# millecker/hadoop-1.0.3-gpu

Measured on AMD Instinct MI355X. Metric: K-Means job makespan + map-tasks/sec (whole node) at 1/2/4/8 MI355X, higher is better.
Workload: dtype fp32

## Files before the change

### hbmr/models/kmeans.py

```python
from __future__ import annotations

import base64
import logging
import math
import os
import threading
import time

import numpy as np
import torch

from ..gpu.splitjob import SplitJob, SplitSpec
from ..mapred import counters as C

log = logging.getLogger("hbmr.kmeans")

K_KEY = "hbmr.kmeans.k"
D_KEY = "hbmr.kmeans.dims"
INPUT_KEY = "hbmr.kmeans.input"
SPLIT_PTS_KEY = "hbmr.split.points"
CIN_KEY = "hbmr.kmeans.centroids.in"
COUT_KEY = "hbmr.kmeans.centroids.out"
INIT_KEY = "hbmr.kmeans.centroids.init"
NCENTERS_KEY = "hbmr.kmeans.synthetic.centers"
RETURN_KEY = "hbmr.kmeans.return.centroids"
CDIR_KEY = "hbmr.kmeans.centroids.dir"
EXACT_KEY = "hbmr.kmeans.exact"
EXACT_MFMA_KEY = "hbmr.kmeans.exact.mfma"
COMBINER_KEY = "hbmr.kmeans.combiner"
BOUNDS_KEY = "hbmr.kmeans.exact.bounds"

_M32 = 0xFFFFFFFF


def _mix32(x: torch.Tensor) -> torch.Tensor:
    x = x & _M32
    x = ((x ^ (x >> 16)) * 0x45D9F3B) & _M32
    x = ((x ^ (x >> 16)) * 0x45D9F3B) & _M32
    return x ^ (x >> 16)


def _uniform(c: torch.Tensor) -> torch.Tensor:
    return (_mix32(c).to(torch.float64) + 0.5) * (1.0 / 4294967296.0)


def _gauss(c1: torch.Tensor, c2: torch.Tensor) -> torch.Tensor:
    u1 = _uniform(c1)
    u2 = _uniform(c2)
    return torch.sqrt(-2.0 * torch.log(u1)) * torch.cos(2.0 * math.pi * u2)


def synthetic_points(seed: int, start: int, n: int, d: int, centers: int, device,
                     chunk: int = 1 << 18) -> torch.Tensor:
    dev = torch.device(device)
    out = torch.empty(n, d, dtype=torch.float32, device=dev)
    j = torch.arange(d, dtype=torch.int64, device=dev)
    cidx = torch.arange(centers, dtype=torch.int64, device=dev)
    s = (seed * 0x9E3779B1) & _M32
    cc = (cidx[:, None] * 131071 + j[None, :] + s * 7) & _M32
    cen = 10.0 * _gauss(cc * 2 + 1, cc * 2 + 2)
    for a in range(0, n, chunk):
        b = min(n, a + chunk)
        p = torch.arange(start + a, start + b, dtype=torch.int64, device=dev)
        lab = _mix32(p * 3 + s) % centers
        base = ((p[:, None] & 0xFFFFFF) * 1024 + j[None, :] + (s << 7)) & _M32
        noise = _gauss(base * 2 + 11, base * 2 + 12 + (p[:, None] >> 24))
        out[a:b] = (cen[lab] + noise).to(torch.float32)
    return out


def encode_centroids(c: torch.Tensor) -> str:
    a = c.detach().to("cpu", torch.float32).contiguous().numpy()
    return f"{a.shape[0]}x{a.shape[1]}:" + base64.b64encode(a.tobytes()).decode()


def decode_centroids(s: str) -> torch.Tensor:
    shp, b = s.split(":", 1)
    k, d = map(int, shp.split("x"))
    return torch.from_numpy(np.frombuffer(base64.b64decode(b), dtype=np.float32).copy()
                            ).reshape(k, d)


class CentroidStore:

    def __init__(self):
        self.lock = threading.Lock()
        self.host: dict[str, torch.Tensor] = {}
        self.images: dict[tuple, object] = {}
        self.order: list[str] = []
        self.keep = 4

    def put_host(self, key, cen):
        with self.lock:
            self.host[key] = cen
            for k in [k for k in self.images if k[0] == key]:
                self.images.pop(k)
            self._touch(key)

    def put_image(self, key, device, img):
        with self.lock:
            self.host.pop(key, None)
            self.images[(key, str(device))] = img
            self._touch(key)

    def _touch(self, key):
        if key in self.order:
            self.order.remove(key)
        self.order.append(key)
        while len(self.order) > self.keep:
            old = self.order.pop(0)
            self.host.pop(old, None)
            for k in [k for k in self.images if k[0] == old]:
                self.images.pop(k)

    def host_centroids(self, key):
        with self.lock:
            c = self.host.get(key)
            if c is not None:
                return c
            for (k, _dev), img in self.images.items():
                if k == key:
                    ready = getattr(img, "ready", None)
                    if ready is not None:
                        ready.synchronize()
                    c = img.cen.detach().to("cpu")
                    self.host[key] = c
                    return c
        return None

    def image(self, key, device):
        from ..ops import kmeans as km
        with self.lock:
            img = self.images.get((key, str(device)))
        if img is not None:
            return img
        cen = self.host_centroids(key)
        if cen is None:
            raise KeyError(f"centroids {key!r} not resident on this tracker")
        img = km.CentroidImage(cen, device)
        if img.cen.is_cuda:
            img.ready = torch.cuda.Event()
            img.ready.record()
        self.put_image(key, device, img)
        return img


STORE = CentroidStore()


def _centroid_file(cdir, key):
    return os.path.join(cdir, key.replace("/", "_").replace(":", "_") + ".npy")


def _save_centroids(cdir, key, cen):
    host = cen.detach().to("cpu", torch.float32).numpy()
    os.makedirs(cdir, exist_ok=True)
    path = _centroid_file(cdir, key)
    tmp = path + ".tmp.npy"
    np.save(tmp, host)
    os.replace(tmp, path)
    old = _SAVED.setdefault(cdir, [])
    old.append(path)
    while len(old) > 3:
        try:
            os.remove(old.pop(0))
        except OSError:
            pass


_SAVED: dict = {}
_PINNED_INFLIGHT: list = []


def _sum_slabs(outs):
    groups: dict = {}
    loose = []
    for s, c in outs:
        bs, bc = s._base, c._base
        if bs is not None and bc is not None and bs.dim() == 3 and bc.dim() == 2 and \
                tuple(s.shape) == tuple(bs.shape[1:]) and tuple(c.shape) == tuple(bc.shape[1:]):
            g = groups.setdefault(id(bs), [bs, bc, 0, []])
            g[2] += 1
            g[3].append((s, c))
        else:
            loose.append((s, c))
    parts_s, parts_c = [], []
    for bs, bc, n, members in groups.values():
        if n == bs.shape[0] and len({m[0].data_ptr() for m in members}) == n:
            parts_s.append(bs.sum(0))
            parts_c.append(bc.sum(0))
        else:
            loose.extend(members)
    if loose:
        parts_s.append(torch.stack([s for s, _ in loose]).sum(0))
        parts_c.append(torch.stack([c for _, c in loose]).sum(0))
    sums, counts = parts_s[0], parts_c[0]
    for s, c in zip(parts_s[1:], parts_c[1:]):
        sums = sums + s
        counts = counts + c
    return sums, counts


_EXACT_STATS: dict = {}
_EXACT_SKIPPED: dict = {}
_EXACT_LOCK = threading.Lock()

_BASELINES: "dict" = {}
_BASE_LOCK = threading.Lock()
_BASE_MAX = 4096


def _baseline_plan(ctxs, datas, k, dp, fx, exact, enabled):
    have, new, plain = [], [], []
    bases, keys = [], []
    seen = set()
    dev = str(ctxs[0].device)
    with _BASE_LOCK:
        for i, (c, d) in enumerate(zip(ctxs, datas)):
            sp = c.spec.split
            sk = sp.get("key") if enabled and isinstance(sp, dict) else None
            key = None if sk is None else (sk, dev, k, dp, fx, exact)
            keys.append(key)
            if key is None or key in seen:
                plain.append(i)
                bases.append(None)
                continue
            seen.add(key)
            b = _BASELINES.get(key)
            x = d.xb if exact else d
            if b is not None and b.data_ptr == x.data_ptr() and b.n == x.shape[0]:
                have.append(i)
                bases.append(b)
            else:
                new.append(i)
                bases.append(None)
    return have, new, plain, bases, keys


def _baseline_bytes(b) -> int:
    return sum(t.numel() * t.element_size() for t in (b.g, b.S0, b.N0, getattr(b, "gap", None))
               if t is not None)


def _drop_baselines(split_key, device):
    dev = f"cuda:{device}" if isinstance(device, int) else str(device)
    with _BASE_LOCK:
        for key in [kk for kk in _BASELINES if kk[0] == split_key and kk[1] == dev]:
            _BASELINES.pop(key)


def _install_baselines(entries, stream, cache=None, grown=None):
    ev = torch.cuda.Event()
    ev.record(stream)
    charge = []
    with _BASE_LOCK:
        for key, b in entries:
            b.event, b.stream = ev, stream
            old = _BASELINES.pop(key, None)
            _BASELINES[key] = b
            if old is not b:
                charge.append((key, b, _baseline_bytes(b)))
            elif grown and grown.get(id(b)):
                charge.append((key, b, grown[id(b)]))
        while len(_BASELINES) > _BASE_MAX:
            _BASELINES.pop(next(iter(_BASELINES)))
    if cache is not None and charge:
        cache.add_listener(_drop_baselines)
        idx = stream.device.index if stream is not None else 0
        for key, b, nbytes in charge:
            if not cache.charge(key[0], idx, nbytes):
                with _BASE_LOCK:
                    if _BASELINES.get(key) is b:
                        _BASELINES.pop(key)


def _exact_stats(cin, device):
    key = (cin, str(device))
    with _EXACT_LOCK:
        t = _EXACT_STATS.get(key)
        if t is None:
            t = _EXACT_STATS[key] = torch.zeros(3, dtype=torch.int64, device=device)
        return t


def _exact_skipped(cin, device):
    key = (cin, str(device))
    with _EXACT_LOCK:
        t = _EXACT_SKIPPED.get(key)
        if t is None:
            t = _EXACT_SKIPPED[key] = torch.zeros(1, dtype=torch.int64, device=device)
        return t


class KMeansSplitJob(SplitJob):
    collective_reduce = True
    needs_reduce = True

    def configure(self, conf):
        self.conf = conf
        self.k = conf.get_int(K_KEY, 64)
        self.d = conf.get_int(D_KEY, 128)
        self.input = conf.get(INPUT_KEY, "synthetic:100000:1")
        self.split_points = conf.get_int(SPLIT_PTS_KEY, 500_000)
        self.cin = conf.get(CIN_KEY)
        self.cout = conf.get(COUT_KEY)
        self.centers = conf.get_int(NCENTERS_KEY, self.k)
        self.fx_shift = conf.get_int("hbmr.kmeans.fx.shift", 24)
        self.cdir = conf.get(CDIR_KEY)
        self.exact = conf.get_boolean(EXACT_KEY, False)
        self.exact_dtype = torch.bfloat16 if (conf.get(EXACT_MFMA_KEY) or "f16").lower() in (
            "bf16", "bfloat16") else torch.float16
        self.bounds = conf.get_boolean(BOUNDS_KEY, True)
        self.combiner = (conf.get(COMBINER_KEY) or "delta").lower()
        if self.combiner not in ("delta", "sorted"):
            raise ValueError(f"{COMBINER_KEY} must be delta or sorted, not {self.combiner!r}")
        init = conf.get(INIT_KEY)
        if init and self.cin and STORE.host_centroids(self.cin) is None:
            STORE.put_host(self.cin, decode_centroids(init))
        if self.cin and self.cdir and STORE.host_centroids(self.cin) is None:
            path = _centroid_file(self.cdir, self.cin)
            if os.path.exists(path):
                STORE.put_host(self.cin, torch.from_numpy(np.load(path)))

    _split_memo: dict = {}

    def get_splits(self, conf, trackers):
        if self.input.startswith("synthetic:"):
            mk = (self.input, self.split_points, self.d, self.centers, tuple(trackers),
                  self.exact)
            got = KMeansSplitJob._split_memo.get(mk)
            if got is not None:
                return got
            if len(KMeansSplitJob._split_memo) > 16:
                KMeansSplitJob._split_memo.clear()
            out = KMeansSplitJob._split_memo[mk] = self._synthetic_splits(trackers)
            return out
        return self._file_splits(conf, trackers)

    def _synthetic_splits(self, trackers):
        _, n, seed = self.input.split(":")
        n, seed = int(n), int(seed)
        per = self.split_points
        nsplits = max(1, math.ceil(n / per))
        out = []
        for i in range(nsplits):
            a = i * per
            m = min(per, n - a)
            key = f"kmeans-syn:{seed}:{self.d}:{self.centers}:{a}:{m}" + \
                (":exact" if self.exact else "")
            loc = [trackers[i * len(trackers) // nsplits]] if trackers else []
            out.append(SplitSpec(i, key, "synthetic",
                                 {"seed": seed, "start": a, "n": m}, loc, m * self.d * 2))
        return out

    def _file_splits(self, conf, trackers):
        from ..mapred.formats import FileInputFormat, SequenceFileInputFormat
        from ..mapred.jobconf import JobConf
        jc = JobConf(conf)
        FileInputFormat.setInputPaths(jc, self.input)
        fmt = SequenceFileInputFormat()
        nmaps = max(1, conf.get_int("mapred.map.tasks", 1))
        if conf.get_long("mapred.min.split.size", 0) <= 1 and "://" not in self.input:
            total = sum(f.length for f in fmt.list_status(jc))
            jc.set_long("mapred.min.split.size", max(1, -(-total // nmaps)))
        splits = fmt.getSplits(jc, nmaps)
        out = []
        for i, s in enumerate(splits):
            key = f"kmeans-file:{s.path}:{s.start}:{s.length}" + (":exact" if self.exact else "")
            loc = [trackers[i % len(trackers)]] if trackers else []
            out.append(SplitSpec(i, key, "file", {"path": s.path, "start": s.start,
                                                  "length": s.length}, loc, s.length))
        return out

    def _load_raw(self, spec: SplitSpec, device):
        if spec.kind == "synthetic":
            p = spec.params
            return synthetic_points(p["seed"], p["start"], p["n"], self.d, self.centers, device)
        return self._load_file_split(spec.params, device)

    def _load_fp32(self, spec: SplitSpec, device):
        return self._load_raw(spec, device).to(torch.bfloat16)

    def split_nbytes(self, data) -> int:
        nb = getattr(data, "nbytes", None)
        if callable(nb):
            return int(nb())
        return super().split_nbytes(data)

    def load_split_host(self, spec: SplitSpec):
        if spec.kind != "file":
            return None
        from ..io import nativeio
        p = spec.params
        n = p["length"] // (20 + 4 * self.d) + 2
        host = torch.empty(n, self.d, dtype=torch.float32,
                           pin_memory=torch.cuda.is_available())
        got = nativeio.read_points_into(p["path"], p["start"], p["length"], host.data_ptr(),
                                        self.d, n)
        return host[:got]

    def load_split_from_host(self, spec: SplitSpec, host, device):
        from ..ops import kmeans as km
        x = host.to(device, non_blocking=True)
        ev = torch.cuda.Event()
        ev.record()
        _PINNED_INFLIGHT.append((ev, host))
        while _PINNED_INFLIGHT and _PINNED_INFLIGHT[0][0].query():
            _PINNED_INFLIGHT.pop(0)
        if self.exact:
            return km.ExactSplit(x, km.padded_dim(self.d), self.exact_dtype)
        xb = x.to(torch.bfloat16)
        dp = km.padded_dim(self.d)
        if dp == self.d:
            return xb.contiguous()
        out = torch.zeros(xb.shape[0], dp, dtype=torch.bfloat16, device=device)
        out[:, :self.d] = xb
        return out

    def _load_file_split(self, p, device):
        from ..io import nativeio
        n = p["length"] // (20 + 4 * self.d) + 2
        dev = torch.device(device)
        host = torch.empty(n, self.d, dtype=torch.float32, pin_memory=dev.type == "cuda")
        got = nativeio.read_points_into(p["path"], p["start"], p["length"], host.data_ptr(),
                                        self.d, n)
        host = host[:got]
        if dev.type != "cuda":
            return host
        x = host.to(dev, non_blocking=True)
        ev = torch.cuda.Event()
        ev.record()
        _PINNED_INFLIGHT.append((ev, host))
        while _PINNED_INFLIGHT and _PINNED_INFLIGHT[0][0].query():
            _PINNED_INFLIGHT.pop(0)
        return x

    def load_split_sample(self, spec: SplitSpec, device, fraction: float):
        if spec.kind == "synthetic":
            p = dict(spec.params)
            p["n"] = max(1, int(p["n"] * fraction))
            spec = SplitSpec(spec.index, spec.key + f":sample{fraction}", spec.kind, p,
                             spec.locations, spec.length)
            return self.load_split(spec, device)
        return super().load_split_sample(spec, device, fraction)

    def load_split(self, spec: SplitSpec, device):
        from ..ops import kmeans as km
        if self.exact:
            x = self._load_raw(spec, device)
            if str(device) == "cpu":
                return x.contiguous()
            return km.ExactSplit(x, km.padded_dim(self.d), self.exact_dtype)
        xb = self._load_fp32(spec, device)
        if str(device) == "cpu":
            return xb.to(torch.float32)
        dp = km.padded_dim(self.d)
        if dp == self.d:
            return xb.contiguous()
        out = torch.zeros(xb.shape[0], dp, dtype=torch.bfloat16, device=device)
        out[:, :self.d] = xb
        return out

    @staticmethod
    def _scratch(ctx, ns, k):
        from ..ops import kmeans as km
        key = ("kmeans-scratch", str(ctx.device), id(ctx.stream))
        store = ctx.tracker.__dict__.setdefault("_scratch", {})
        ws, labels = store.get(key, (None, None))
        need_lab, need_ws = km.batch_scratch_sizes(ns, k)
        need_ws = max(need_ws, km.delta_workspace_bytes(int(sum(ns)), len(ns), k))
        if ws is None or ws.numel() < need_ws:
            ws = torch.empty(max(need_ws, 1 << 20), dtype=torch.uint8, device=ctx.device)
        if labels is None or labels.numel() < need_lab:
            labels = torch.empty(max(need_lab, 1), dtype=torch.int32, device=ctx.device)
        store[key] = (ws, labels)
        return ws, labels

    def map_gpu(self, ctx, points):
        return self.map_gpu_batch([ctx], [points])[0]

    def map_gpu_batch(self, ctxs, datas):
        st = ctxs[0].stream
        if st is None:
            return self._map_gpu_batch(ctxs, datas)
        with torch.cuda.stream(st):
            return self._map_gpu_batch(ctxs, datas)

    def _map_gpu_batch(self, ctxs, datas):
        from ..ops import kmeans as km
        ctx = ctxs[0]
        img = STORE.image(self.cin, ctx.device)
        ready = getattr(img, "ready", None)
        if ready is not None:
            torch.cuda.current_stream().wait_event(ready)
        for t in (img.cbf, img.chalf):
            t.record_stream(torch.cuda.current_stream())
        B = len(datas)
        if self.exact:
            return self._map_exact(ctxs, datas, img)
        have, new, plain, bases, keys = _baseline_plan(
            ctxs, datas, self.k, img.dp, img.fx_shift, False, self.combiner == "delta")
        ws, labels = self._scratch(ctx, [d.shape[0] for d in datas], self.k)
        sums = torch.empty(B, self.k, img.dp, dtype=torch.int64, device=ctx.device)
        counts = torch.empty(B, self.k, dtype=torch.int64, device=ctx.device)
        order = have + new + plain
        H = len(have)
        S, N = sums.unbind(0), counts.unbind(0)
        out = [None] * B
        for j, i in enumerate(order):
            out[i] = (S[j], N[j])
        installed = []
        if have:
            hb = [bases[i] for i in have]
            km.map_batch_delta([datas[i] for i in have], img, sums[:H], counts[:H], labels, ws,
                               hb, stream=ctx.stream)
            for i, b in zip(have, hb):
                b.S0, b.N0 = out[i]
                installed.append((keys[i], b))
        rest = new + plain
        if rest:
            km.map_batch_gpu([datas[i] for i in rest], img, sums[H:], counts[H:], labels, ws,
                             stream=ctx.stream, zero_outputs=True)
            if new:
                total = sum(datas[i].shape[0] for i in rest)
                gall = labels[:total].clone()
                off = 0
                newset = set(new)
                for i in rest:
                    n = datas[i].shape[0]
                    if keys[i] is not None and i in newset:
                        installed.append((keys[i], km.Baseline(gall[off:off + n], *out[i],
                                                                datas[i].data_ptr(), n)))
                    off += n
        if installed:
            _install_baselines(installed, ctx.stream, getattr(ctx, "split_cache", None))
        for c, d in zip(ctxs, datas):
            c.reporter.incrCounter(C.TASK_GROUP, C.MAP_INPUT_RECORDS, d.shape[0])
        return out

    def _map_exact(self, ctxs, datas, img):
        from ..ops import kmeans as km
        from ..utils.trace import TRACE
        if TRACE.on:
            TRACE.instant("kmeans.map_exact", n=len(datas))
        ctx = ctxs[0]
        store = ctx.tracker.__dict__.setdefault("_scratch", {})
        scratch = store.setdefault(("kmeans-exact", str(ctx.device), id(ctx.stream)), {})
        stats = _exact_stats(self.cin, ctx.device)
        have, new, plain, bases, keys = _baseline_plan(
            ctxs, datas, self.k, img.dp, img.fx_shift, True, self.combiner == "delta")
        B = len(datas)
        sums = torch.empty(B, self.k, img.dp, dtype=torch.int64, device=ctx.device)
        counts = torch.empty(B, self.k, dtype=torch.int64, device=ctx.device)
        order = have + new + plain
        pos = {i: j for j, i in enumerate(order)}
        H = len(have)
        installed = []
        grown = None
        if have:
            ns = [datas[i].shape[0] for i in have]
            total = sum(ns)
            lab = scratch.get("labcat")
            if lab is None or lab.numel() < total:
                lab = scratch["labcat"] = torch.empty(total, dtype=torch.int32, device=ctx.device)
            need = km.delta_workspace_bytes(total, H, self.k)
            if scratch.get("dws") is None or scratch["dws"].numel() < need:
                scratch["dws"] = torch.empty(need, dtype=torch.uint8, device=ctx.device)
            hb = [bases[i] for i in have]
            bounded = self.bounds and self.combiner == "delta" and km.bounds_supported(img)
            if bounded:
                nogap = [b for b in hb if b.gap is None]
                km.assign_exact_batch([datas[i] for i in have], img, stats, lab, scratch,
                                      stream=ctx.stream, bounds=hb,
                                      skipped=_exact_skipped(self.cin, ctx.device))
                grown = {id(b): b.gap.numel() * b.gap.element_size() for b in nogap}
            else:
                km.assign_exact_batch([datas[i] for i in have], img, stats, lab, scratch,
                                      stream=ctx.stream)
            km.delta_combine([datas[i].x32 for i in have], lab, self.k, sums[:H], counts[:H],
                             scratch["dws"], hb, fx_shift=img.fx_shift, stream=ctx.stream,
                             keep_bounds=bounded)
            for i, b in zip(have, hb):
                b.S0, b.N0 = sums[pos[i]], counts[pos[i]]
                installed.append((keys[i], b))
        for i in new + plain:
            d = datas[i]
            s, c = sums[pos[i]], counts[pos[i]]
            s.zero_()
            c.zero_()
            lab = km.assign_exact(d, img, stats, scratch, stream=ctx.stream)
            need = km.workspace_bytes(d.shape[0], img.k)
            if scratch.get("ws") is None or scratch["ws"].numel() < need:
                scratch["ws"] = torch.empty(max(need, 1 << 20), dtype=torch.uint8,
                                            device=ctx.device)
            km.accumulate(d.x32, lab, img.k, s, c, fx_shift=img.fx_shift, stream=ctx.stream,
                          workspace=scratch["ws"])
            if keys[i] is not None and i in new:
                b = km.Baseline(lab.clone(), s, c, d.xb.data_ptr(), d.shape[0])
                installed.append((keys[i], b))
        if installed:
            _install_baselines(installed, ctx.stream, getattr(ctx, "split_cache", None), grown)
        for c, d in zip(ctxs, datas):
            c.reporter.incrCounter(C.TASK_GROUP, C.MAP_INPUT_RECORDS, d.shape[0])
        return [(sums[pos[i]], counts[pos[i]]) for i in range(B)]

    def map_cpu(self, ctx, points):
        from ..ops import kmeans as km
        cen = STORE.host_centroids(self.cin)
        if cen is None:
            raise KeyError(f"centroids {self.cin!r} not resident")
        sums, counts = km.new_partials(self.k, self.d, "cpu")
        st = [0]
        km.map_split_cpu(points, cen, sums, counts, nthreads=ctx.cpu_threads,
                         fx_shift=self.fx_shift, exact=self.exact, stats=st)
        if self.exact:
            ctx.reporter.incrCounter("KMEANS", "EXACT_FLAGGED_POINTS", st[0])
        ctx.reporter.incrCounter(C.TASK_GROUP, C.MAP_INPUT_RECORDS, points.shape[0])
        return sums, counts

    def map_sim(self, ctx, points):
        if points is None:
            ctx.reporter.incrCounter(C.TASK_GROUP, C.MAP_INPUT_RECORDS, 0)
            return None
        return self.map_cpu(ctx, points)

    def combine(self, ctx, outputs):
        from ..ops import kmeans as km
        dev = ctx.device if ctx.device is not None else torch.device("cpu")
        dp = km.padded_dim(self.d) if dev.type == "cuda" else self.d
        outputs = [o for o in outputs if o is not None]
        if dev.type == "cuda":
            cur = torch.cuda.current_stream()
            for s, c in outputs:
                if s.is_cuda:
                    s.record_stream(cur)
                    c.record_stream(cur)
        from ..utils.trace import TRACE
        if TRACE.on:
            TRACE.instant("kmeans.combine.recorded", n=len(outputs))
        same = [(s, c) for s, c in outputs if s.device == dev and s.shape[1] == dp]
        other = [(s, c) for s, c in outputs if not (s.device == dev and s.shape[1] == dp)]
        if same:
            sums, counts = _sum_slabs(same)
        else:
            sums = torch.zeros(self.k, dp, dtype=torch.int64, device=dev)
            counts = torch.zeros(self.k, dtype=torch.int64, device=dev)
        for s, c in other:
            sums[:, :s.shape[1]] += s.to(dev, non_blocking=True)
            counts += c.to(dev, non_blocking=True)
        return sums, counts

    def reduce(self, ctx, combined):
        from ..ops import kmeans as km
        from ..utils.trace import TRACE
        sums, counts = combined
        k, dp = sums.shape
        packed = torch.cat([sums.reshape(-1), counts])
        sim = getattr(ctx, "simulated_collective_s", None)
        with TRACE.span("kmeans.allreduce", nbytes=packed.numel() * 8):
            if sim is None:
                ctx.comm.all_reduce(packed)
            else:
                ctx.sim_ready = max(time.time(), getattr(ctx, "sim_base", 0.0)) + sim
        sums = packed[:k * dp].view(k, dp)
        counts = packed[k * dp:]
        est = _EXACT_STATS.pop((self.cin, str(sums.device)), None) \
            if self.exact and sums.device.type == "cuda" else None
        esk = _EXACT_SKIPPED.pop((self.cin, str(sums.device)), None) \
            if self.exact and sums.device.type == "cuda" else None
        killed = getattr(ctx, "killed", None)
        if killed is not None and killed():
            raise RuntimeError("reduce killed (collective restart): result not published")
        if sums.device.type == "cuda":
            old = STORE.image(self.cin, sums.device)
            ready = getattr(old, "ready", None)
            if ready is not None:
                torch.cuda.current_stream().wait_event(ready)
            img = km.CentroidImage.__new__(km.CentroidImage)
            img.__dict__.update(old.__dict__)
            img.cen = old.cen.clone()
            img.cbf = old.cbf.clone()
            img.chalf = old.chalf.clone()
            img.shift2 = torch.zeros_like(old.shift2)
            img.refresh(sums, counts)
            if self.exact:
                img.image16(self.exact_dtype)
                img.neighbors()
            img.ready = torch.cuda.Event()
            img.ready.record()
            host_cen = cen_ev = None
            if ctx.rank == 0 and (self.cdir or self.conf.get_boolean(RETURN_KEY, False)):
                host_cen = torch.empty(tuple(img.cen.shape), dtype=torch.float32,
                                       pin_memory=True)
                host_cen.copy_(img.cen, non_blocking=True)
                cen_ev = torch.cuda.Event()
                cen_ev.record()
            if TRACE.on:
                TRACE.instant("kmeans.refresh_launched")
            STORE.put_image(self.cout, sums.device, img)
            rel = getattr(ctx, "release_dependents", None)
            if rel is not None:
                rel()
            vals = [img.shift2.max().double().sqrt(), counts.sum().double()]
            if est is not None:
                vals += list(est.double().unbind(0))
            if esk is not None:
                vals.append(esk[0].double())
            got = torch.stack(vals).tolist()
            shift, npts = got[0], got[1]
            if esk is not None:
                ctx.reporter.incrCounter("KMEANS", "EXACT_BOUND_SKIPPED_POINTS", int(got[-1]))
            if est is not None:
                for name, v in zip(("EXACT_FLAGGED_POINTS", "EXACT_RELABELLED_POINTS",
                                    "EXACT_NEIGHBOUR_SCANS"), got[2:5]):
                    ctx.reporter.incrCounter("KMEANS", name, int(v))
            if TRACE.on:
                TRACE.instant("kmeans.shift_synced")
            new_cen = None
        else:
            host_cen = cen_ev = None
            old = STORE.host_centroids(self.cin)
            if sim is not None:
                new_cen, shift, npts = old, 0.0, 0
            else:
                cnt = counts.to(torch.float64)[:, None]
                s = sums[:, :self.d].to(torch.float64) / float(1 << self.fx_shift)
                new_cen = torch.where(cnt > 0, s / cnt.clamp(min=1),
                                      old.to(torch.float64)).to(torch.float32)
                shift = float((new_cen - old).norm(dim=1).max()) if self.k else 0.0
                npts = int(counts.sum().item())
            STORE.put_host(self.cout, new_cen)
            rel = getattr(ctx, "release_dependents", None)
            if rel is not None:
                rel()
            if sim is not None:
                delay = ctx.sim_ready - time.time()
                if delay > 0:
                    time.sleep(delay)
        self._write_output(ctx, counts, new_cen)
        if TRACE.on:
            TRACE.instant("kmeans.output_written")
        res = {"shift": shift, "points": int(npts), "centroids_key": self.cout}
        if host_cen is not None:
            cen_ev.synchronize()
        if ctx.rank == 0 and self.cdir:
            cen = new_cen if new_cen is not None else host_cen
            _save_centroids(self.cdir, self.cout, cen[:, :self.d])
        if ctx.rank == 0 and self.conf.get_boolean(RETURN_KEY, False):
            cen = new_cen if new_cen is not None else host_cen
            res["centroids"] = encode_centroids(cen[:, :self.d])
        if TRACE.on:
            TRACE.instant("kmeans.reduce_return")
        return res

    def poison_result(self, ctx):
        with STORE.lock:
            host = STORE.host.get(self.cout)
            if host is not None:
                STORE.host[self.cout] = host + 1.0
            for key, img in list(STORE.images.items()):
                if key[0] == self.cout:
                    STORE.images.pop(key)
                    STORE.host[self.cout] = img.cen.detach().to("cpu")[:, :self.d] + 1.0

    def _write_output(self, ctx, counts, new_cen):
        out = self.conf.get("mapred.output.dir")
        if not out:
            return
        import os

        from ..io import sequencefile as seqf
        from ..io.writable import FloatVectorWritable, IntWritable
        cen = new_cen if new_cen is not None else STORE.host_centroids(self.cout)
        W = ctx.world_size
        per = math.ceil(self.k / W)
        lo, hi = ctx.rank * per, min(self.k, (ctx.rank + 1) * per)
        os.makedirs(out, exist_ok=True)
        with seqf.Writer(os.path.join(out, f"part-{ctx.rank:05d}"), IntWritable,
                         FloatVectorWritable) as w:
            for j in range(lo, hi):
                w.append(IntWritable(j), FloatVectorWritable(cen[j].numpy()))


def make_iteration_conf(base, k, d, inp, split_points, cin, cout, init=None,
                        return_centroids=False):
    from ..mapred.jobconf import JobConf
    job = JobConf(base)
    job.set_job_name(f"kmeans {cin}->{cout}")
    job.set("hbmr.splitjob.class", "hbmr.models.kmeans:KMeansSplitJob")
    job.set("hbmr.gpu.mapper.class", "hbmr.models.kmeans:KMeansSplitJob")
    job.set_int(K_KEY, k)
    job.set_int(D_KEY, d)
    job.set(INPUT_KEY, inp)
    job.set_int(SPLIT_PTS_KEY, split_points)
    job.set(CIN_KEY, cin)
    job.set(COUT_KEY, cout)
    job.set("hbmr.job.signature", f"kmeans|{inp}|{k}|{d}|{split_points}")
    if init is not None:
        job.set(INIT_KEY, encode_centroids(init))
    if return_centroids:
        job.set_boolean(RETURN_KEY, True)
    return job


def initial_centroids(inp, k, d, centers=None, exact=False):
    def rnd(x):
        return x if exact else x.to(torch.bfloat16).to(torch.float32)
    if inp.startswith("synthetic:"):
        _, _n, seed = inp.split(":")
        x = synthetic_points(int(seed), 0, k, d, centers or k, "cpu")
        return rnd(x)
    from ..io import sequencefile as seqf
    import os
    path = inp
    if os.path.isdir(path):
        path = os.path.join(path, sorted(f for f in os.listdir(path) if not f.startswith(("_", ".")))[0])
    rows = []
    with seqf.Reader(path) as r:
        while len(rows) < k:
            raw = r.next_raw()
            if raw is None:
                break
            rows.append(np.frombuffer(raw[1][4:], dtype=">f4").astype(np.float32))
    return rnd(torch.from_numpy(np.stack(rows)))


class KMeansDriver:

    MANIFEST = "driver.json"

    def __init__(self, submit, result_of, conf=None, k=64, d=128, inp="synthetic:100000:1",
                 split_points=500_000, run_id=None, return_centroids=None, checkpoint_dir=None):
        self.submit = submit
        self.result_of = result_of
        self.base = conf
        self.k, self.d, self.inp, self.split_points = k, d, inp, split_points
        self.run_id = run_id or f"km{int(time.time() * 1e3) & 0xFFFFFF:x}"
        self.iteration = 0
        self.history = []
        self.return_centroids = (k * d <= 65536) if return_centroids is None else return_centroids
        base_dir = (conf.get("mapred.local.dir") if conf is not None else None) or "/tmp/hbmr-local"
        self.centroid_dir = checkpoint_dir or os.path.join(base_dir, "kmeans-centroids",
                                                           self.run_id)
        self._manifest_written = False
        self.prefetch_delay = 0.005
        self._ahead: list = []

    def _write_manifest(self):
        import json
        os.makedirs(self.centroid_dir, exist_ok=True)
        path = os.path.join(self.centroid_dir, self.MANIFEST)
        with open(path + ".tmp", "w") as f:
            json.dump({"run_id": self.run_id, "k": self.k, "d": self.d, "input": self.inp,
                       "split_points": self.split_points}, f)
        os.replace(path + ".tmp", path)
        self._manifest_written = True

    @classmethod
    def resume(cls, submit, result_of, checkpoint_dir, conf=None, **kw):
        import json
        import re
        with open(os.path.join(checkpoint_dir, cls.MANIFEST)) as f:
            m = json.load(f)
        drv = cls(submit, result_of, conf=conf, k=m["k"], d=m["d"], inp=m["input"],
# ... 119 lines not shown
```

### hbmr/ops/_lib.py

```python
from __future__ import annotations

import ctypes
import os
import threading
from pathlib import Path

import torch

_LIB_PATH = Path(__file__).resolve().parent.parent / "lib" / "libhbmr.so"
_lock = threading.Lock()
_lib = None

c_void_p = ctypes.c_void_p
c_long = ctypes.c_long
c_int = ctypes.c_int
c_uint = ctypes.c_uint
c_uint64 = ctypes.c_uint64
c_double_p = ctypes.POINTER(ctypes.c_double)

_SIGS = {
    "hbmr_kmeans_assign_bf16": (c_int, [c_void_p, c_long, c_int, c_void_p, c_void_p, c_int,
                                        c_void_p, c_void_p, c_void_p]),
    "hbmr_kmeans_accum_bf16": (c_int, [c_void_p, c_long, c_int, c_void_p, c_int, c_void_p,
                                       c_void_p, c_int, c_void_p, c_long, c_int, c_void_p]),
    "hbmr_kmeans_accum_f32": (c_int, [c_void_p, c_long, c_int, c_void_p, c_int, c_void_p,
                                      c_void_p, c_int, c_void_p, c_long, c_int, c_void_p]),
    "hbmr_kmeans_assign_top3_bf16": (c_int, [c_void_p, c_long, c_int, c_void_p, c_void_p, c_int,
                                             c_void_p, c_void_p, c_void_p, c_void_p, c_void_p]),
    "hbmr_kmeans_assign_top3_f16": (c_int, [c_void_p, c_long, c_int, c_void_p, c_void_p, c_int,
                                            c_void_p, c_void_p, c_void_p, c_void_p, c_void_p]),
    "hbmr_kmeans_exact_prep": (c_int, [c_void_p, c_long, c_int, c_int, c_int, c_int, c_void_p,
                                       c_void_p, c_void_p, c_void_p, c_void_p]),
    "hbmr_kmeans_assign_top3_q1_grouped": (c_int, [c_int, c_void_p, c_void_p, c_int, c_int,
                                                   c_void_p, c_void_p, c_void_p, c_int, c_void_p,
                                                   c_void_p, c_void_p, c_void_p, c_int, c_int,
                                                   c_void_p, c_void_p, c_void_p, c_void_p,
                                                   c_void_p, c_long, c_void_p, c_void_p]),
    "hbmr_kmeans_bound_workspace_bytes": (c_long, [c_long, c_int, c_int]),
    "hbmr_kmeans_assign_top3_q1_bounded": (c_int, [c_int, c_void_p, c_void_p, c_int, c_int,
                                                   c_void_p, c_void_p, c_int, c_void_p,
                                                   c_void_p, c_void_p, c_void_p, c_int, c_int,
                                                   c_void_p, c_void_p, c_void_p, c_void_p,
                                                   c_void_p, c_long, c_void_p,
                                                   c_void_p, c_void_p, c_void_p, c_void_p,
                                                   c_void_p, c_long, c_void_p, c_void_p]),
    "hbmr_kmeans_centroid_nbr": (c_int, [c_void_p, c_int, c_int, c_int, c_void_p, c_void_p,
                                         c_void_p, c_void_p]),
    "hbmr_kmeans_image16": (c_int, [c_void_p, c_int, c_int, c_int, c_int, c_int, c_void_p,
                                    c_void_p, c_void_p, c_void_p, c_void_p, c_void_p]),
    "hbmr_kmeans_image16_tiled": (c_int, [c_void_p, c_int, c_int, c_void_p, c_void_p]),
    "hbmr_kmeans_set_exact_kernel": (c_int, [c_int]),
    "hbmr_kmeans_get_exact_kernel": (c_int, []),
    "hbmr_kmeans_refine_f32": (c_int, [c_void_p, c_long, c_int, c_int, c_void_p, c_void_p,
                                       c_void_p, c_void_p, c_int, c_int, c_void_p, c_void_p,
                                       c_void_p, c_void_p, c_void_p, c_void_p, c_int, c_void_p,
                                       c_void_p, c_void_p, c_void_p, c_void_p, c_int,
                                       c_void_p]),
    "hbmr_kmeans_refine_batch_bytes": (c_long, [c_int, c_void_p]),
    "hbmr_kmeans_assign_top3_grouped": (c_int, [c_int, c_void_p, c_void_p, c_int, c_int,
                                                c_void_p, c_void_p, c_int, c_void_p, c_void_p,
                                                c_void_p, c_void_p, c_void_p]),
    "hbmr_kmeans_refine_batch_q1g": (c_int, [c_int, c_void_p, c_int, c_int, c_int, c_void_p,
                                             c_void_p, c_void_p, c_void_p, c_void_p, c_void_p,
                                             c_void_p, c_void_p, c_void_p, c_void_p, c_void_p,
                                             c_void_p, c_long, c_void_p, c_void_p]),
    "hbmr_kmeans_refine_batch_q1": (c_int, [c_int, c_void_p, c_int, c_int, c_int, c_int,
                                            c_void_p, c_void_p, c_void_p, c_void_p, c_void_p,
                                            c_void_p, c_void_p, c_void_p, c_void_p, c_void_p,
                                            c_void_p, c_void_p, c_void_p, c_long, c_int,
                                            c_void_p, c_void_p]),
    "hbmr_kmeans_refine_batch_finish": (c_int, [c_int, c_void_p, c_void_p, c_void_p, c_int,
                                                c_int, c_void_p, c_int, c_int, c_void_p,
                                                c_void_p, c_void_p, c_void_p, c_int, c_void_p,
                                                c_int, c_void_p, c_long, c_void_p]),
    "hbmr_kmeans_accum_workspace_bytes": (c_long, [c_long, c_int]),
    "hbmr_kmeans_batch_workspace_bytes": (c_long, [c_long, c_int, c_int]),
    "hbmr_kmeans_map_batch": (c_int, [c_int, c_void_p, c_void_p, c_int, c_void_p, c_void_p, c_int,
                                      c_int, c_void_p, c_void_p, c_long, c_void_p, c_void_p,
                                      c_int, c_int, c_void_p]),
    "hbmr_kmeans_delta_workspace_bytes": (c_long, [c_long, c_int, c_int]),
    "hbmr_kmeans_delta_combine": (c_int, [c_int, c_void_p, c_void_p, c_int, c_int, c_int,
                                          c_void_p, c_void_p, c_long, c_void_p, c_void_p, c_int,
                                          c_void_p, c_void_p, c_void_p, c_void_p]),
    "hbmr_kmeans_map_batch_delta": (c_int, [c_int, c_void_p, c_void_p, c_int, c_void_p, c_void_p,
                                            c_int, c_int, c_void_p, c_void_p, c_long, c_void_p,
                                            c_void_p, c_int, c_void_p, c_void_p, c_void_p,
                                            c_void_p]),
    "hbmr_kmeans_update": (c_int, [c_void_p, c_void_p, c_int, c_int, c_int, c_int, c_int,
                                   c_void_p, c_void_p, c_void_p, c_void_p, c_void_p]),
    "hbmr_kmeans_padded_k": (c_int, [c_int]),
    "hbmr_kmeans_map_cpu_f32": (c_int, [c_void_p, c_long, c_int, c_void_p, c_int, c_void_p,
                                        c_void_p, c_void_p, c_double_p, c_int, c_int]),
    "hbmr_kmeans_map_cpu_f32_ex": (c_int, [c_void_p, c_long, c_int, c_void_p, c_int, c_void_p,
                                           c_void_p, c_void_p, c_double_p, c_int, c_int, c_int,
                                           c_void_p]),
    "hbmr_kmeans_padded_dim": (c_int, [c_int]),
    "hbmr_f32_to_bf16_pad": (c_int, [c_void_p, c_long, c_int, c_int, c_void_p, c_void_p]),
    "hbmr_radix_sort_workspace_bytes": (c_long, [c_long]),
    "hbmr_radix_onesweep_workspace_bytes": (c_long, [c_long]),
    "hbmr_radix_onesweep_status_bytes": (c_long, [c_long]),
    "hbmr_radix_sort_keys_u64": (c_int, [c_void_p, c_void_p, c_long, c_int, c_int, c_void_p,
                                         c_long, c_void_p, c_long, c_void_p, c_void_p, c_int,
                                         c_void_p]),
    "hbmr_radix_sort_pairs_u64": (c_int, [c_void_p, c_void_p, c_void_p, c_void_p, c_long, c_int,
                                          c_int, c_void_p, c_long, c_void_p]),
    "hbmr_teragen": (c_int, [c_long, c_long, c_void_p, c_void_p]),
    "hbmr_tera_keys": (c_int, [c_void_p, c_long, c_int, c_void_p, c_void_p, c_void_p]),
    "hbmr_gather_u64": (c_int, [c_void_p, c_void_p, c_long, c_void_p, c_void_p]),
    "hbmr_gather_records": (c_int, [c_void_p, c_void_p, c_long, c_int, c_void_p, c_void_p]),
    "hbmr_split_offsets": (c_int, [c_void_p, c_void_p, c_long, c_void_p, c_void_p, c_int,
                                   c_void_p, c_void_p]),
    "hbmr_check_sorted": (c_int, [c_void_p, c_void_p, c_long, c_void_p, c_void_p]),
    "hbmr_tera_collect": (c_int, [c_void_p, c_void_p, c_void_p, c_void_p, c_void_p, c_int, c_long,
                                  c_void_p, c_void_p, c_void_p, c_void_p, c_void_p]),
    "hbmr_tera_collect_slots": (c_int, [c_void_p, c_void_p, c_void_p, c_int, c_int, c_long,
                                        c_void_p, c_void_p, c_void_p]),
    "hbmr_gather_records_multi": (c_int, [c_void_p, c_void_p, c_void_p, c_void_p, c_long, c_int,
                                          c_void_p, c_void_p]),
    "hbmr_tera_partition_workspace_bytes": (c_long, [c_long, c_int]),
    "hbmr_tera_collect_gid": (c_int, [c_void_p, c_void_p, c_void_p, c_void_p, c_int, c_long,
                                      c_int, c_uint64, c_uint, c_uint, c_int, c_void_p, c_void_p,
                                      c_void_p]),
    "hbmr_gather_records_gid": (c_int, [c_void_p, c_void_p, c_void_p, c_long, c_int, c_void_p,
                                        c_void_p, c_void_p, c_void_p, c_void_p]),
    "hbmr_tera_group_stats": (c_int, [c_void_p, c_void_p, c_long, c_void_p, c_void_p, c_void_p,
                                      c_void_p]),
    "hbmr_radix_set_onesweep_waves": (c_int, [c_int]),
    "hbmr_gather_set_unroll": (c_int, [c_int]),
    "hbmr_tera_tie_fix_scratch_bytes": (c_long, [c_long, c_int]),
    "hbmr_tera_tie_fix_records": (c_int, [c_void_p, c_void_p, c_void_p, c_long, c_int, c_uint64,
                                          c_uint, c_uint, c_int, c_void_p, c_void_p, c_void_p,
                                          c_long, c_void_p]),
    "hbmr_merge_path": (c_int, [c_void_p, c_void_p, c_void_p, c_long, c_void_p, c_void_p, c_void_p,
                                c_long, c_void_p, c_void_p, c_void_p, c_void_p]),
    "hbmr_tera_tie_fix": (c_int, [c_void_p, c_void_p, c_void_p, c_long, c_void_p, c_void_p]),
    "hbmr_tera_partition": (c_int, [c_void_p, c_long, c_int, c_void_p, c_void_p, c_int, c_void_p,
                                    c_void_p, c_void_p, c_void_p, c_void_p, c_void_p, c_long,
                                    c_void_p]),
    "hbmr_wc_tiles": (c_long, [c_long]),
    "hbmr_wc_tokenize_count": (c_int, [c_void_p, c_long, c_void_p, c_void_p]),
    "hbmr_wc_tokenize_write": (c_int, [c_void_p, c_long, c_void_p, c_void_p, c_void_p, c_void_p]),
    "hbmr_wc_insert": (c_int, [c_void_p, c_long, c_void_p, c_void_p, c_void_p, c_long, c_void_p,
                               c_void_p, c_long, c_void_p, c_void_p]),
    "hbmr_wc_compact": (c_int, [c_void_p, c_long, c_void_p, c_void_p, c_long, c_int, c_void_p,
                                c_void_p, c_void_p, c_void_p, c_void_p, c_void_p]),
    "hbmr_wc_pack": (c_int, [c_void_p, c_void_p, c_void_p, c_void_p, c_long, c_void_p, c_void_p,
                             c_void_p]),
    "hbmr_grep_cand_count": (c_int, [c_void_p, c_long, c_void_p, c_void_p, c_int, c_int, c_int,
                                     c_int, c_void_p, c_void_p, c_void_p]),
    "hbmr_grep_cand_write": (c_int, [c_void_p, c_long, c_void_p, c_void_p, c_int, c_int, c_int,
                                     c_int, c_void_p, c_void_p, c_void_p, c_void_p, c_void_p]),
    "hbmr_grep_select_blocks": (c_long, [c_long]),
    "hbmr_grep_block_max": (c_int, [c_void_p, c_long, c_void_p, c_void_p]),
    "hbmr_grep_prefix_max": (c_int, [c_void_p, c_long, c_void_p, c_void_p, c_void_p]),
    "hbmr_grep_select_count": (c_int, [c_void_p, c_void_p, c_void_p, c_long, c_void_p, c_void_p]),
    "hbmr_grep_select_write": (c_int, [c_void_p, c_void_p, c_void_p, c_long, c_void_p, c_void_p,
                                       c_void_p, c_void_p]),
    "hbmr_span_insert": (c_int, [c_void_p, c_long, c_void_p, c_void_p, c_void_p, c_long, c_void_p,
                                 c_void_p, c_long, c_void_p, c_void_p]),
    "hbmr_span_compact": (c_int, [c_void_p, c_void_p, c_void_p, c_void_p, c_void_p, c_long, c_int,
                                  c_void_p, c_void_p, c_void_p, c_void_p, c_void_p, c_void_p]),
    "hbmr_lines_count": (c_int, [c_void_p, c_long, c_void_p, c_void_p]),
    "hbmr_lines_write": (c_int, [c_void_p, c_long, c_void_p, c_void_p, c_void_p, c_void_p]),
    "hbmr_recsort_hash_partition": (c_int, [c_void_p, c_void_p, c_void_p, c_long, c_int, c_void_p,
                                            c_void_p]),
    "hbmr_recsort_round_keys": (c_int, [c_void_p, c_void_p, c_void_p, c_void_p, c_long, c_int,
                                        c_void_p, c_void_p, c_void_p]),
    "hbmr_recsort_round_workspace_bytes": (c_long, [c_long]),
    "hbmr_recsort_round": (c_int, [c_void_p, c_void_p, c_void_p, c_int, c_long, c_int, c_void_p,
                                   c_void_p, c_void_p, c_void_p, c_void_p, c_void_p, c_void_p,
                                   c_void_p, c_void_p, c_long, c_void_p]),
    "hbmr_recsort_cuts": (c_int, [c_void_p, c_void_p, c_void_p, c_void_p, c_long, c_void_p,
                                  c_void_p, c_void_p, c_int, c_void_p, c_void_p]),
    "hbmr_recsort_chunk_bytes": (c_int, []),
    "hbmr_recsort_set_chunk_lanes": (c_int, [c_int]),
    "hbmr_recsort_gather": (c_int, [c_void_p, c_void_p, c_void_p, c_void_p, c_void_p, c_void_p,
                                    c_void_p, c_long, c_long, c_void_p, c_void_p]),
    "hbmr_pi_halton": (c_int, [ctypes.c_longlong, ctypes.c_longlong, c_void_p, c_void_p]),
    "hbmr_gemm_bf16_tn": (c_int, [c_void_p, c_void_p, c_void_p, c_long, c_long, c_long,
                                  ctypes.c_float, c_int, c_void_p]),
    "hbmr_gemm_set_kernel": (c_int, [c_int]),
    "hbmr_gemm_bf16_tn_ex": (c_int, [c_void_p, c_void_p, c_void_p, c_long, c_long, c_long,
                                     ctypes.c_float, c_int, c_void_p, c_void_p]),
}


class NativeLibraryError(RuntimeError):
    pass


def lib_path() -> Path:
    return _LIB_PATH


def available() -> bool:
    try:
        load()
        return True
# ... 45 lines not shown
```

### hbmr/ops/kmeans.py

```python
from __future__ import annotations

import ctypes
import os
import threading

import torch

from . import _lib
from ..utils.trace import TRACE

SUPPORTED_DP = (64, 128, 256)


def _nullctx():
    import contextlib
    return contextlib.nullcontext()
FX_SHIFT = 24
NBR_L = 256


def padded_dim(d: int) -> int:
    for dp in SUPPORTED_DP:
        if d <= dp:
            return dp
# ... 172 lines not shown
    ws = max(int(lib.hbmr_kmeans_batch_workspace_bytes(total, len(ns), k)),
             int(lib.hbmr_kmeans_accum_workspace_bytes(max(ns), k)))
    return total, ws


def accum_workspace(n: int, k: int, device) -> torch.Tensor:
    lib = _lib.load()
    need = int(lib.hbmr_kmeans_accum_workspace_bytes(n, k))
    key = torch.device(device)
    ws = _workspaces.get(key)
    if ws is None or ws.numel() < need:
        ws = torch.empty(max(need, 1 << 20), dtype=torch.uint8, device=key)
        _workspaces[key] = ws
    return ws


def accumulate(points: torch.Tensor, labels: torch.Tensor, k: int, sums: torch.Tensor,
               counts: torch.Tensor, fx_shift: int = FX_SHIFT, stream=None,
               workspace: torch.Tensor | None = None, mode: int = ACCUM_AUTO) -> None:
    n, dp = points.shape
    if sums.shape != (k, dp) or sums.dtype != torch.int64:
        raise ValueError(f"sums must be int64 [{k}, {dp}]")
    if counts.shape != (k,) or counts.dtype != torch.int64:
        raise ValueError(f"counts must be int64 [{k}]")
    if points.dtype not in (torch.bfloat16, torch.float32) or not points.is_contiguous() or \
            dp not in SUPPORTED_DP or labels.numel() < n:
        raise ValueError("points must be contiguous bf16/fp32 [n, dp] with n labels")
    lib = _lib.load()
    if workspace is None and mode != ACCUM_LDS:
        workspace = accum_workspace(n, k, points.device)
    fn, name = ((lib.hbmr_kmeans_accum_f32, "hbmr_kmeans_accum_f32")
                if points.dtype == torch.float32 else
                (lib.hbmr_kmeans_accum_bf16, "hbmr_kmeans_accum_bf16"))
    rc = fn(_ptr(points), n, dp, _ptr(labels), k, _ptr(sums), _ptr(counts), fx_shift,
            _ptr(workspace), 0 if workspace is None else workspace.numel(), mode,
            _lib.stream_handle(stream))
    _lib.check(rc, name)


def _f32_up(v: torch.Tensor) -> torch.Tensor:
    f = v.float()
    return torch.where(f.double() < v, torch.nextafter(f, torch.full_like(f, float("inf"))), f)


class ExactSplit:
    __slots__ = ("xb", "x32", "xnorm", "xbn2", "xerr", "d")

    def __init__(self, x32: torch.Tensor, dp: int, dtype=torch.float16):
        n, d = x32.shape
        self.d = d
        dev = x32.device
        if dp == d:
            self.x32 = x32.contiguous()
        else:
            self.x32 = torch.zeros(n, dp, dtype=torch.float32, device=dev)
            self.x32[:, :d] = x32
        if dev.type == "cuda":
            self.xb = torch.empty(n, dp, dtype=dtype, device=dev)
            self.xnorm = torch.empty(n, dtype=torch.float32, device=dev)
            self.xbn2 = torch.empty(n, dtype=torch.float32, device=dev)
            self.xerr = torch.empty(n, dtype=torch.float32, device=dev)
            rc = _lib.load().hbmr_kmeans_exact_prep(
                _ptr(self.x32), n, dp, dp, dp, int(dtype == torch.float16), _ptr(self.xb),
                _ptr(self.xnorm), _ptr(self.xbn2), _ptr(self.xerr), _lib.stream_handle(None))
            _lib.check(rc, "hbmr_kmeans_exact_prep")
            return
        x64 = self.x32.double()
        self.xnorm = x64.norm(dim=1).float()
        lim = 65504.0 if dtype == torch.float16 else float("inf")
        xb = self.x32.clamp(-lim, lim).to(dtype)
        xb64 = xb.double()
        self.xbn2 = xb64.pow(2).sum(1).float()
        self.xerr = _f32_up((x64 - xb64).norm(dim=1))
        self.xb = xb.contiguous()

    @property
    def shape(self):
        return self.xb.shape

    def nbytes(self) -> int:
        return sum(t.numel() * t.element_size() for t in (self.xb, self.x32, self.xnorm,
                                                          self.xbn2, self.xerr))


def assign_top3(points: torch.Tensor, img: CentroidImage, labels, cand, scores, margin,
                stream=None) -> None:
    n, dp = points.shape
    if points.dtype not in (torch.bfloat16, torch.float16) or dp != img.dp or \
            not points.is_contiguous():
        raise ValueError("points must be contiguous bf16/fp16 [n, dp] matching the image")
    for t, dt, m in ((labels, torch.int32, 1), (cand, torch.int32, 2), (scores, torch.float32, 1),
                     (margin, torch.float32, 2)):
        if t.numel() != m * n or t.dtype != dt or not t.is_contiguous():
            raise ValueError("top-3 outputs: labels/scores [n], cand/margin [2n]")
    f16 = points.dtype == torch.float16
    with torch.cuda.stream(stream) if stream is not None else _nullctx():
        c16, ch = img.image16(points.dtype)[:2]
    fn = "hbmr_kmeans_assign_top3_f16" if f16 else "hbmr_kmeans_assign_top3_bf16"
    rc = getattr(_lib.load(), fn)(
        _ptr(points), n, dp, _ptr(c16), _ptr(ch), img.k_pad, _ptr(labels),
        _ptr(cand), _ptr(scores), _ptr(margin), _lib.stream_handle(stream))
    _lib.check(rc, fn)


REFINE_VERSION = int(os.environ.get("HBMR_REFINE", "3"))
MAX_REFINE_BATCH = 64


def _check_refine_dim(img: "CentroidImage") -> None:
    if REFINE_VERSION >= 3 and img.d % 8:
        raise ValueError(f"refine v3 needs d % 8 == 0 (d = {img.d}): HBMR_REFINE=2 takes any d")


def _refine_ws(ns: list, device, scratch: dict | None):
    arr = (ctypes.c_long * len(ns))(*ns)
    need = int(_lib.load().hbmr_kmeans_refine_batch_bytes(len(ns), arr))
    if need < 0:
        raise ValueError("refine batch of 1..64 splits expected")
    ws = None if scratch is None else scratch.get("refine_ws")
    if ws is None or ws.numel() < need:
        ws = torch.empty(need, dtype=torch.uint8, device=device)
        if scratch is not None:
            scratch["refine_ws"] = ws
    return arr, ws


class _RefineBatch:

    def __init__(self, splits: list, img: "CentroidImage", stats, scratch, stream):
        _check_refine_dim(img)
        self.splits, self.img, self.stats, self.stream = splits, img, stats, stream
        self.dt = splits[0].xb.dtype
        self.ns, self.ws = _refine_ws([sp.shape[0] for sp in splits], splits[0].x32.device,
                                      scratch)
        with torch.cuda.stream(stream) if stream is not None else _nullctx():
            self.norms = img.norms(self.dt)
            self.nbr = img.neighbors()
            self.pd = img.pair_dist()
        self.labels = [None] * len(splits)
        self.lib = _lib.load()
        self.st = _lib.stream_handle(stream)

    def q1(self, i, labels_ptr, cand, scores, margin):
        sp, img = self.splits[i], self.img
        cn, cmax, ce, cemax = self.norms
        self.labels[i] = labels_ptr
        rc = self.lib.hbmr_kmeans_refine_batch_q1(
            len(self.splits), self.ns, i, img.d, img.k, img.k_pad, _ptr(sp.xnorm),
            _ptr(sp.xbn2), _ptr(sp.xerr), _ptr(cn), _ptr(cmax), _ptr(ce), _ptr(cemax),
            labels_ptr, _ptr(cand), _ptr(scores), _ptr(margin), _ptr(self.stats),
            _ptr(self.ws), self.ws.numel(), int(i == 0), _ptr(self.pd), self.st)
        _lib.check(rc, "hbmr_kmeans_refine_batch_q1")

    def finish(self):
        B = len(self.splits)
        img = self.img
        _, cmax, _, cemax = self.norms
        ni, nd, L = self.nbr
        xs = (ctypes.c_void_p * B)(*[sp.x32.data_ptr() for sp in self.splits])
        ls = (ctypes.c_void_p * B)(*[(lp.value if isinstance(lp, ctypes.c_void_p) else lp)
                                     for lp in self.labels])
        rc = self.lib.hbmr_kmeans_refine_batch_finish(
            B, self.ns, xs, ls, img.d, self.splits[0].x32.shape[1], _ptr(img.cen), img.k,
            img.k_pad, _ptr(cmax), _ptr(cemax), _ptr(ni), _ptr(nd), L, _ptr(self.stats),
            self.stats.numel(), _ptr(self.ws), self.ws.numel(), self.st)
        _lib.check(rc, "hbmr_kmeans_refine_batch_finish")


def refine_f32(split: ExactSplit, img: CentroidImage, labels, cand, scores, margin,
               stats: torch.Tensor, stream=None, scratch: dict | None = None) -> None:
    n = split.shape[0]
    if stats.dtype != torch.int64 or stats.numel() < 3:
        raise ValueError("stats must be int64 [3]")
    if labels.numel() != n or cand.numel() != 2 * n or margin.numel() != 2 * n:
        raise ValueError("labels [n], cand/margin [2n] from assign_top3 expected")
    if REFINE_VERSION >= 3:
        rb = _RefineBatch([split], img, stats, scratch, stream)
        rb.q1(0, labels.data_ptr(), cand, scores, margin)
        rb.finish()
        return
    with torch.cuda.stream(stream) if stream is not None else _nullctx():
        cn, cmax, ce, cemax = img.norms(split.xb.dtype)
        ni, nd, L = img.neighbors()
    rc = _lib.load().hbmr_kmeans_refine_f32(
        _ptr(split.x32), n, img.d, split.x32.shape[1], _ptr(split.xnorm), _ptr(split.xbn2),
        _ptr(split.xerr), _ptr(img.cen), img.k, img.k_pad, _ptr(cn), _ptr(cmax), _ptr(ce),
        _ptr(cemax), _ptr(ni), _ptr(nd), L,
        _ptr(labels), _ptr(cand), _ptr(scores), _ptr(margin), _ptr(stats), stats.numel(),
        _lib.stream_handle(stream))
    _lib.check(rc, "hbmr_kmeans_refine_f32")


def assign_exact(split: ExactSplit, img: CentroidImage, stats: torch.Tensor,
                 scratch: dict | None = None, stream=None) -> torch.Tensor:
    _check_refine_dim(img)
    n = split.shape[0]
    dev = split.xb.device
    scratch = {} if scratch is None else scratch
    key = ("exact", n)
    bufs = scratch.get(key)
    if bufs is None:
        bufs = scratch[key] = (torch.empty(n, dtype=torch.int32, device=dev),
                               torch.empty(2 * n, dtype=torch.int32, device=dev),
                               torch.empty(n, dtype=torch.float32, device=dev),
                               torch.empty(2 * n, dtype=torch.float32, device=dev))
    lab, cand, sc, mg = bufs
    assign_top3(split.xb, img, lab, cand, sc, mg, stream=stream)
    refine_f32(split, img, lab, cand, sc, mg, stats, stream=stream, scratch=scratch)
    return lab


def bounds_supported(img: CentroidImage) -> bool:
    return REFINE_VERSION >= 3 and img.dp <= 128 and GROUPED_EXACT and FUSED_Q1 and \
        img.cen.is_cuda and _lib.load().hbmr_kmeans_get_exact_kernel() == 3


def assign_exact_batch(splits: list, img: CentroidImage, stats: torch.Tensor, out: torch.Tensor,
                       scratch: dict | None = None, stream=None, bounds: list | None = None,
                       skipped: torch.Tensor | None = None) -> None:
    if not splits:
        return
    _check_refine_dim(img)
    if bounds is not None and (len(bounds) != len(splits) or not bounds_supported(img)):
        raise ValueError("bounds: one baseline per split, grouped fused v3 assign (dp <= 128)")
    dev = splits[0].xb.device
    total = sum(sp.shape[0] for sp in splits)
    if out.dtype != torch.int32 or out.numel() < total or not out.is_contiguous():
        raise ValueError("out must be contiguous int32 with room for every split's labels")
    if stats.dtype != torch.int64 or stats.numel() < 3:
        raise ValueError("stats must be int64 [3]")
    dt = splits[0].xb.dtype
    for sp in splits:
        if sp.xb.dtype != dt or dt not in (torch.bfloat16, torch.float16) or \
                sp.xb.shape[1] != img.dp or not sp.xb.is_contiguous() or \
                not sp.x32.is_contiguous():
            raise ValueError("exact splits must hold contiguous [n, dp] rows of one 16-bit type")
    nmax = max(sp.shape[0] for sp in splits)
    scratch = {} if scratch is None else scratch
    key = ("exact-batch", nmax)
    bufs = scratch.get(key)
    if bufs is None:
        for kk in [kk for kk in scratch if isinstance(kk, tuple) and kk[0] == "exact-batch"]:
            del scratch[kk]
        bufs = scratch[key] = (torch.empty(2 * nmax, dtype=torch.int32, device=dev),
                               torch.empty(nmax, dtype=torch.float32, device=dev),
                               torch.empty(2 * nmax, dtype=torch.float32, device=dev))
    cand, sc, mg = bufs
    grouped = REFINE_VERSION >= 3 and img.dp <= 128 and GROUPED_EXACT
    with torch.cuda.stream(stream) if stream is not None else _nullctx():
        c16, ch, cn, cmax, ce, cemax = img.image16(dt)
        ni, nd, L = (None, None, 0) if grouped else img.neighbors()
        newref = None
        if bounds is not None:
            img.cen.record_stream(torch.cuda.current_stream())
            newref = img.cen.clone()
    lib = _lib.load()
    top3 = lib.hbmr_kmeans_assign_top3_f16 if dt == torch.float16 else \
        lib.hbmr_kmeans_assign_top3_bf16
    st = _lib.stream_handle(stream)
    pc, ps, pm, pst = _ptr(cand), _ptr(sc), _ptr(mg), _ptr(stats)
    pcn, pcmax, pce, pcemax, pni, pnd = (_ptr(t) for t in (cn, cmax, ce, cemax, ni, nd))
    base, off = out.data_ptr(), 0
    for g0 in range(0, len(splits), MAX_REFINE_BATCH):
        group = splits[g0:g0 + MAX_REFINE_BATCH]
        if grouped:
            off += _exact_group(group, img, stats, base + 4 * off, c16, ch, (cn, cmax, ce, cemax),
                                dt, scratch, stream, lib, st,
                                None if bounds is None else bounds[g0:g0 + MAX_REFINE_BATCH],
                                skipped, newref)
            continue
        rb = _RefineBatch(group, img, stats, scratch, stream) if REFINE_VERSION >= 3 else None
        for i, sp in enumerate(group):
            n = sp.shape[0]
            pl = ctypes.c_void_p(base + 4 * off)
            rc = top3(_ptr(sp.xb), n, img.dp, _ptr(c16), _ptr(ch), img.k_pad, pl, pc, ps, pm, st)
            _lib.check(rc, "hbmr_kmeans_assign_top3")
            if rb is not None:
                rb.q1(i, pl, cand, sc, mg)
            else:
                rc = lib.hbmr_kmeans_refine_f32(
                    _ptr(sp.x32), n, img.d, sp.x32.shape[1], _ptr(sp.xnorm), _ptr(sp.xbn2),
                    _ptr(sp.xerr), _ptr(img.cen), img.k, img.k_pad, pcn, pcmax, pce, pcemax,
                    pni, pnd, L, pl, pc, ps, pm, pst, stats.numel(), st)
                _lib.check(rc, "hbmr_kmeans_refine_f32")
            off += n
        if rb is not None:
            rb.finish()


PAIR_DIST_MAX_K = int(os.environ.get("HBMR_PAIR_DIST_MAX_K", "8192"))
NBR_NATIVE_MAX_K = int(os.environ.get("HBMR_NBR_NATIVE_MAX_K", "8192"))
GROUPED_EXACT = os.environ.get("HBMR_EXACT_GROUPED", "1") != "0"
FUSED_Q1 = os.environ.get("HBMR_EXACT_FUSED_Q1", "1") != "0"


def _bounded_group(group, bases, img, labels_ptr, ch, norms, dt, scratch, stream, lib, st, rb,
                   skipped, newref):
    B = len(group)
    ns = [sp.shape[0] for sp in group]
    N = sum(ns)
    dev = group[0].xb.device
    cur = torch.cuda.current_stream() if stream is None else stream
    with torch.cuda.stream(cur):
        events, blocks = {}, {}
        for b in bases:
            if b.event is not None and b.stream is not None and b.stream != cur:
                events[id(b.event)] = b.event
        for ev in events.values():
            cur.wait_event(ev)
        for b in bases:
            if b.gap is None:
                b.gap, b.ref = torch.empty(b.g.numel(), dtype=torch.float32, device=dev), None
        for b, n in zip(bases, ns):
            if b.g.numel() != n or b.gap.numel() != n or \
                    (b.ref is not None and (tuple(b.ref.shape) != tuple(img.cen.shape) or
                                            not b.ref.is_contiguous())):
                raise ValueError("bounds: baseline does not match its split / the centroids")
            for t in (b.g, b.gap, b.ref):
                if t is not None:
                    base = t._base if t._base is not None else t
                    blocks[id(base)] = base
        for t in blocks.values():
            t.record_stream(cur)
        need = int(lib.hbmr_kmeans_bound_workspace_bytes(N, B, img.k))
        bws = scratch.get("bound_ws")
        if bws is None or bws.numel() < need:
            bws = scratch["bound_ws"] = torch.empty(need, dtype=torch.uint8, device=dev)
    P = ctypes.c_void_p * B
    cn, cmax, ce, cemax = norms
    refs = [b.ref for b in bases]
    for b in bases:
        b.ref = b.pending = None
    rc = lib.hbmr_kmeans_assign_top3_q1_bounded(
        B, P(*[sp.xb.data_ptr() for sp in group]), (ctypes.c_long * B)(*ns), img.dp,
        int(dt == torch.float16), _ptr(img.image16_tiled(dt)), _ptr(ch), img.k_pad, labels_ptr,
        P(*[sp.xnorm.data_ptr() for sp in group]), P(*[sp.xbn2.data_ptr() for sp in group]),
        P(*[sp.xerr.data_ptr() for sp in group]), img.d, img.k, _ptr(cn), _ptr(cmax), _ptr(ce),
        _ptr(cemax), _ptr(rb.ws), rb.ws.numel(), _ptr(rb.pd),
        P(*[b.g.data_ptr() for b in bases]), P(*[b.gap.data_ptr() for b in bases]),
        P(*[None if r is None else r.data_ptr() for r in refs]), _ptr(img.cen),
        _ptr(bws), bws.numel(), _ptr(skipped), st)
    _lib.check(rc, "hbmr_kmeans_assign_top3_q1_bounded")
    for b in bases:
        b.pending = newref


def _exact_group(group, img, stats, labels_ptr, c16, ch, norms, dt, scratch, stream, lib, st,
                 bases=None, skipped=None, newref=None):
    B = len(group)
    ns = [sp.shape[0] for sp in group]
    N = sum(ns)
    dev = group[0].xb.device
    P = ctypes.c_void_p * B
    xs = P(*[sp.xb.data_ptr() for sp in group])
    nsa = (ctypes.c_long * B)(*ns)
    if bases is not None:
        rb = _RefineBatch(group, img, stats, scratch, stream)
        if TRACE.on:
            TRACE.instant("kmeans.top3_launch", n=B)
        _bounded_group(group, bases, img, labels_ptr, ch, norms, dt, scratch, stream, lib, st, rb,
                       skipped, newref)
        o = 0
        for i in range(B):
            rb.labels[i] = labels_ptr + 4 * o
            o += ns[i]
        rb.finish()
        return N
    if FUSED_Q1 and img.dp <= 128:
        rb = _RefineBatch(group, img, stats, scratch, stream)
        if TRACE.on:
            TRACE.instant("kmeans.top3_launch", n=B)
        cn, cmax, ce, cemax = norms
        rc = lib.hbmr_kmeans_assign_top3_q1_grouped(
            B, xs, nsa, img.dp, int(dt == torch.float16), _ptr(c16),
            _ptr(img.image16_tiled(dt)), _ptr(ch), img.k_pad,
            labels_ptr, P(*[sp.xnorm.data_ptr() for sp in group]),
            P(*[sp.xbn2.data_ptr() for sp in group]), P(*[sp.xerr.data_ptr() for sp in group]),
            img.d, img.k, _ptr(cn), _ptr(cmax), _ptr(ce), _ptr(cemax), _ptr(rb.ws),
            rb.ws.numel(), _ptr(rb.pd), st)
        _lib.check(rc, "hbmr_kmeans_assign_top3_q1_grouped")
        o = 0
        for i in range(B):
            rb.labels[i] = labels_ptr + 4 * o
            o += ns[i]
        rb.finish()
        return N
    key = ("exact-group", N)
    bufs = scratch.get(key)
    if bufs is None:
        for kk in [kk for kk in scratch if isinstance(kk, tuple) and kk[0] == "exact-group"]:
            del scratch[kk]
        bufs = scratch[key] = (torch.empty(2 * N, dtype=torch.int32, device=dev),
                               torch.empty(N, dtype=torch.float32, device=dev),
                               torch.empty(2 * N, dtype=torch.float32, device=dev))
    cand, sc, mg = bufs
    rc = lib.hbmr_kmeans_assign_top3_grouped(B, xs, nsa, img.dp, int(dt == torch.float16),
                                             _ptr(c16), _ptr(ch), img.k_pad, labels_ptr,
                                             _ptr(cand), _ptr(sc), _ptr(mg), st)
    _lib.check(rc, "hbmr_kmeans_assign_top3_grouped")
    rb = _RefineBatch(group, img, stats, scratch, stream)
    cn, cmax, ce, cemax = norms
    rc = lib.hbmr_kmeans_refine_batch_q1g(
        B, nsa, img.d, img.k, img.k_pad, P(*[sp.xnorm.data_ptr() for sp in group]),
        P(*[sp.xbn2.data_ptr() for sp in group]), P(*[sp.xerr.data_ptr() for sp in group]),
        _ptr(cn), _ptr(cmax), _ptr(ce), _ptr(cemax), labels_ptr, _ptr(cand), _ptr(sc), _ptr(mg),
        _ptr(rb.ws), rb.ws.numel(), _ptr(rb.pd), st)
    _lib.check(rc, "hbmr_kmeans_refine_batch_q1g")
    o = 0
    for i in range(B):
        rb.labels[i] = labels_ptr + 4 * o
        o += ns[i]
    rb.finish()
    return N


def map_split_exact(split: ExactSplit, img: CentroidImage, sums, counts, scratch: dict,
                    stats: torch.Tensor, stream=None) -> None:
    n = split.shape[0]
    lab = assign_exact(split, img, stats, scratch, stream=stream)
    need = workspace_bytes(n, img.k)
    if scratch.get("ws") is None or scratch["ws"].numel() < need:
        scratch["ws"] = torch.empty(max(need, 1 << 20), dtype=torch.uint8, device=split.xb.device)
    accumulate(split.x32, lab, img.k, sums, counts, fx_shift=img.fx_shift, stream=stream,
               workspace=scratch["ws"])


def map_batch_gpu(splits: list, img: CentroidImage, sums: torch.Tensor, counts: torch.Tensor,
                  labels: torch.Tensor, workspace: torch.Tensor, stream=None,
                  zero_outputs: bool = True) -> None:
    B = len(splits)
    if B == 0:
        return
    for s in splits:
        if s.dtype != torch.bfloat16 or s.shape[1] != img.dp or not s.is_contiguous():
            raise ValueError("splits must be contiguous bf16 [n, dp]")
    if sums.shape != (B, img.k, img.dp) or counts.shape != (B, img.k):
        raise ValueError("batch output shape mismatch")
    need_lab, need_ws = batch_scratch_sizes([s.shape[0] for s in splits], img.k)
    if labels.numel() < need_lab:
        raise ValueError("labels scratch too small")
    lib = _lib.load()
    if workspace.numel() < need_ws:
        raise ValueError("workspace too small")
    ptrs = (ctypes.c_void_p * B)(*[s.data_ptr() for s in splits])
    ns = (ctypes.c_long * B)(*[s.shape[0] for s in splits])
    rc = lib.hbmr_kmeans_map_batch(B, ptrs, ns, img.dp, _ptr(img.cbf), _ptr(img.chalf), img.k_pad,
                                   img.k, _ptr(labels), _ptr(workspace), workspace.numel(),
                                   _ptr(sums), _ptr(counts), img.fx_shift, int(zero_outputs),
                                   _lib.stream_handle(stream))
    _lib.check(rc, "hbmr_kmeans_map_batch")


class Baseline:
    __slots__ = ("g", "S0", "N0", "event", "stream", "data_ptr", "n", "gap", "ref", "pending")

    def __init__(self, g, S0, N0, data_ptr, n):
        self.g, self.S0, self.N0 = g, S0, N0
        self.gap = self.ref = self.pending = None
        self.event = None
        self.stream = None
        self.data_ptr, self.n = data_ptr, n

    def labels_advanced(self, bounded: bool = False) -> None:
        self.ref = self.pending if bounded else None
        self.pending = None


def delta_workspace_bytes(total: int, ntasks: int, k: int) -> int:
    return int(_lib.load().hbmr_kmeans_delta_workspace_bytes(total, ntasks, k))


def _delta_args(xs, bases, stream):
    B = len(xs)
    st = torch.cuda.current_stream() if stream is None else stream
    events, blocks = {}, {}
    for b in bases:
        if b.event is not None and b.stream is not None and b.stream != st:
            events[id(b.event)] = b.event
        for t in (b.g, b.S0, b.N0):
            base = t._base if t._base is not None else t
            blocks[id(base)] = base
    for ev in events.values():
        st.wait_event(ev)
    for t in blocks.values():
        t.record_stream(st)
    ptrs = (ctypes.c_void_p * B)(*[x.data_ptr() for x in xs])
    ns = (ctypes.c_long * B)(*[x.shape[0] for x in xs])
    gs = (ctypes.c_void_p * B)(*[b.g.data_ptr() for b in bases])
    s0 = (ctypes.c_void_p * B)(*[b.S0.data_ptr() for b in bases])
    n0 = (ctypes.c_void_p * B)(*[b.N0.data_ptr() for b in bases])
    return ptrs, ns, gs, s0, n0


def map_batch_delta(splits: list, img: CentroidImage, sums: torch.Tensor, counts: torch.Tensor,
                    labels: torch.Tensor, workspace: torch.Tensor, bases: list,
                    stream=None) -> None:
    B = len(splits)
    if B == 0:
        return
    if B > 64 or len(bases) != B:
        raise ValueError("at most 64 splits per delta batch, one baseline each")
    for s, b in zip(splits, bases):
        if s.dtype != torch.bfloat16 or s.shape[1] != img.dp or not s.is_contiguous():
            raise ValueError("splits must be contiguous bf16 [n, dp]")
        if b.g.numel() != s.shape[0] or tuple(b.S0.shape) != (img.k, img.dp) or \
                b.N0.numel() != img.k:
            raise ValueError("baseline does not match its split")
    if sums.shape != (B, img.k, img.dp) or counts.shape != (B, img.k) or \
            not sums.is_contiguous() or not counts.is_contiguous():
        raise ValueError("batch output shape mismatch")
    total = sum(s.shape[0] for s in splits)
    if labels.numel() < total:
        raise ValueError("labels scratch too small")
    need = delta_workspace_bytes(total, B, img.k)
    if workspace.numel() < need:
        raise ValueError("workspace too small")
    ptrs, ns, gs, s0, n0 = _delta_args(splits, bases, stream)
    for b in bases:
        b.labels_advanced()
    rc = _lib.load().hbmr_kmeans_map_batch_delta(
        B, ptrs, ns, img.dp, _ptr(img.cbf), _ptr(img.chalf), img.k_pad, img.k, _ptr(labels),
        _ptr(workspace), workspace.numel(), _ptr(sums), _ptr(counts), img.fx_shift, gs, s0, n0,
        _lib.stream_handle(stream))
    _lib.check(rc, "hbmr_kmeans_map_batch_delta")


def delta_combine(xs: list, labels: torch.Tensor, k: int, sums: torch.Tensor,
                  counts: torch.Tensor, workspace: torch.Tensor, bases: list,
                  fx_shift: int = FX_SHIFT, stream=None, keep_bounds: bool = False) -> None:
    B = len(xs)
    if B == 0:
        return
    pend = [b.pending for b in bases]
    for b in bases:
        b.labels_advanced()
    dp = xs[0].shape[1]
    f32 = xs[0].dtype == torch.float32
    for x, b in zip(xs, bases):
        if x.dtype != xs[0].dtype or x.shape[1] != dp or not x.is_contiguous() or \
                b.g.numel() != x.shape[0]:
            raise ValueError("delta_combine: rows/baselines mismatch")
    if B > 64 or dp not in SUPPORTED_DP or sums.shape != (B, k, dp) or counts.shape != (B, k):
        raise ValueError("delta_combine: shape mismatch")
    total = sum(x.shape[0] for x in xs)
    need = delta_workspace_bytes(total, B, k)
    if workspace.numel() < need or labels.numel() < total:
        raise ValueError("delta_combine: scratch too small")
    ptrs, ns, gs, s0, n0 = _delta_args(xs, bases, stream)
    rc = _lib.load().hbmr_kmeans_delta_combine(
        B, ptrs, ns, dp, int(f32), k, _ptr(labels), _ptr(workspace), workspace.numel(),
        _ptr(sums), _ptr(counts), fx_shift, gs, s0, n0, _lib.stream_handle(stream))
    _lib.check(rc, "hbmr_kmeans_delta_combine")
    if keep_bounds:
        for b, p in zip(bases, pend):
            b.ref = p


def map_split_gpu(points, img: CentroidImage, sums, counts, labels=None, stream=None):
    labels = assign(points, img, labels=labels, stream=stream)
    accumulate(points, labels, img.k, sums, counts, fx_shift=img.fx_shift, stream=stream)
    return labels


def map_split_cpu(points: torch.Tensor, centroids: torch.Tensor, sums: torch.Tensor,
                  counts: torch.Tensor, nthreads: int = 1, labels: torch.Tensor | None = None,
                  fx_shift: int = FX_SHIFT, exact: bool = False, stats: list | None = None):
    x = points.detach().to(torch.float32).contiguous()
    c = centroids.detach().to(torch.float32).contiguous()
    n, d = x.shape
    k = c.shape[0]
    if counts.shape != (k,) or counts.dtype != torch.int64 or sums.dtype != torch.int64:
        raise ValueError("sums/counts must be int64")
    target = sums
    if sums.shape != (k, d):
        target = torch.zeros(k, d, dtype=torch.int64)
    cost = ctypes.c_double(0.0)
    lib = _lib.load()
    res = ctypes.c_long(0)
    rc = lib.hbmr_kmeans_map_cpu_f32_ex(_ptr(x), n, d, _ptr(c), k, _ptr(labels), _ptr(target),
                                        _ptr(counts), ctypes.byref(cost), fx_shift, int(nthreads),
                                        int(exact), ctypes.byref(res))
    _lib.check(rc, "hbmr_kmeans_map_cpu_f32_ex")
    if stats is not None:
        stats[0] += res.value
    if target is not sums:
        sums[:, :d] += target
    return cost.value
```

### native/include/hbmr/hbmr.h

```cpp
#pragma once
#include <stddef.h>
#include <stdint.h>

#ifdef __cplusplus
extern "C" {
#endif

typedef struct ihipStream_t* hbmr_stream_t;

#ifndef HBMR_NO_HIP_DECLS
#include <hip/hip_runtime_api.h>
int hbmr_kmeans_assign_bf16(const void* X, long n, int dp, const void* C, const float* chalf,
                            int k_pad, int32_t* labels, float* scores, hipStream_t st);
int hbmr_kmeans_accum_bf16(const void* X, long n, int dp, const int32_t* labels, int k,
                           long long* sums, long long* counts, int fx_shift, void* ws,
                           long ws_bytes, int mode, hipStream_t st);
int hbmr_kmeans_accum_f32(const float* X, long n, int dp, const int32_t* labels, int k,
                          long long* sums, long long* counts, int fx_shift, void* ws,
                          long ws_bytes, int mode, hipStream_t st);
int hbmr_kmeans_assign_top3_bf16(const void* X, long n, int dp, const void* C, const float* chalf,
                                 int k_pad, int32_t* labels, int32_t* cand, float* scores,
                                 float* margin, hipStream_t st);
int hbmr_kmeans_assign_top3_f16(const void* X, long n, int dp, const void* C, const float* chalf,
                                int k_pad, int32_t* labels, int32_t* cand, float* scores,
                                float* margin, hipStream_t st);
int hbmr_kmeans_exact_prep(const float* x, long n, int d, int ldx, int dp, int f16, void* x16,
                           float* xnorm, float* xn2, float* xerr, hipStream_t st);
int hbmr_kmeans_centroid_nbr(const float* cen, int k, int d, int L, int32_t* di, float* dv,
                             float* pd, hipStream_t st);
int hbmr_kmeans_image16(const float* cen, int k, int d, int dp, int k_pad, int f16, void* c16,
                        float* chalf, float* cnorm, float* cerr, float* maxima, hipStream_t st);
int hbmr_kmeans_image16_tiled(const void* c16, int k_pad, int dp, void* c16t, hipStream_t st);
int hbmr_kmeans_set_stamps(void* p);
int hbmr_kmeans_refine_f32(const float* X32, long n, int d, int ldx, const float* xnorm,
                           const float* xbn2, const float* xerr, const float* C32, int k,
                           int k_pad, const float* cnorm, const float* cmax, const float* cerr,
                           const float* cerrmax, const int32_t* nbr_idx,
                           const float* nbr_dist, int L, int32_t* labels, const int32_t* cand,
                           const float* scores, const float* margin, unsigned long long* stats,
                           int nstats, hipStream_t st);
int hbmr_kmeans_assign_top3_q1_grouped(int nsplit, const void* const* X, const long* n, int dp,
                                       int f16, const void* C, const void* Ct,
                                       const float* chalf, int k_pad,
                                       int32_t* labels, const float* const* xnorm,
                                       const float* const* xbn2, const float* const* xerr,
                                       int d, int k, const float* cnorm, const float* cmax,
                                       const float* cerr, const float* cerrmax, void* ws,
                                       long ws_bytes, const float* dcc, hipStream_t st);
long hbmr_kmeans_bound_workspace_bytes(long total, int nsplit, int k);
int hbmr_kmeans_assign_top3_q1_bounded(int nsplit, const void* const* X, const long* n, int dp,
                                       int f16, const void* Ct, const float* chalf, int k_pad,
                                       int32_t* labels, const float* const* xnorm,
                                       const float* const* xbn2, const float* const* xerr,
                                       int d, int k, const float* cnorm, const float* cmax,
                                       const float* cerr, const float* cerrmax, void* ws,
                                       long ws_bytes, const float* dcc,
                                       const int32_t* const* g, float* const* gap,
                                       const float* const* ref, const float* cen, void* bws,
                                       long bws_bytes, unsigned long long* skipped,
                                       hipStream_t st);
int hbmr_kmeans_assign_top3_grouped(int nsplit, const void* const* X, const long* n, int dp,
                                    int f16, const void* C, const float* chalf, int k_pad,
                                    int32_t* labels, int32_t* cand, float* scores, float* margin,
                                    hipStream_t st);
int hbmr_kmeans_refine_batch_q1g(int nsplit, const long* ns, int d, int k, int k_pad,
                                 const float* const* xnorm, const float* const* xbn2,
                                 const float* const* xerr, const float* cnorm, const float* cmax,
                                 const float* cerr, const float* cerrmax, const int32_t* labels,
                                 const int32_t* cand, const float* scores, const float* margin,
                                 void* ws, long ws_bytes, const float* dcc, hipStream_t st);
long hbmr_kmeans_refine_batch_bytes(int nsplit, const long* ns);
int hbmr_kmeans_refine_batch_q1(int nsplit, const long* ns, int s, int d, int k, int k_pad,
                                const float* xnorm, const float* xbn2, const float* xerr,
                                const float* cnorm, const float* cmax, const float* cerr,
                                const float* cerrmax, const int32_t* labels, const int32_t* cand,
                                const float* scores, const float* margin,
                                unsigned long long* stats, void* ws, long ws_bytes, int reset,
                                const float* dcc, hipStream_t st);
int hbmr_kmeans_refine_batch_finish(int nsplit, const long* ns, const float* const* x32,
                                    int32_t* const* labels, int d, int ldx, const float* C32,
                                    int k, int k_pad, const float* cmax, const float* cerrmax,
                                    const int32_t* nbr_idx, const float* nbr_dist, int L,
                                    unsigned long long* stats, int nstats, void* ws,
                                    long ws_bytes, hipStream_t st);
int hbmr_kmeans_update(const long long* sums, const long long* counts, int fx_shift, int k, int d,
                       int dp, int k_pad, float* cen, void* cbf, float* chalf, float* shift2,
                       hipStream_t st);
int hbmr_kmeans_map_batch(int ntasks, const void* const* X, const long* n, int dp,
                          const void* C, const float* chalf, int k_pad, int k, int32_t* labels,
                          void* ws, long ws_bytes, long long* sums, long long* counts,
                          int fx_shift, int zero_outputs, hipStream_t st);
int hbmr_f32_to_bf16_pad(const float* src, long n, int d, int dp, void* dst, hipStream_t st);
#endif
int hbmr_kmeans_padded_dim(int d);

#ifndef HBMR_NO_HIP_DECLS
int hbmr_radix_sort_pairs_u64(uint64_t* keys, uint32_t* vals, uint64_t* tkeys, uint32_t* tvals,
                              long n, int begin_bit, int end_bit, void* ws, long ws_bytes,
                              hipStream_t st);
int hbmr_teragen(long first_row, long nrows, void* out, hipStream_t st);
int hbmr_tera_keys(const void* records, long n, int stride, uint64_t* hi, uint64_t* lo,
                   hipStream_t st);
int hbmr_gather_u64(const uint64_t* src, const uint32_t* perm, long n, uint64_t* dst,
                    hipStream_t st);
int hbmr_gather_records(const void* src, const uint32_t* perm, long n, int record_bytes, void* dst,
                        hipStream_t st);
int hbmr_split_offsets(const uint64_t* hi, const uint64_t* lo, long n, const uint64_t* shi,
                       const uint64_t* slo, int nparts, long* offsets, hipStream_t st);
int hbmr_check_sorted(const uint64_t* hi, const uint64_t* lo, long n, unsigned long long* bad,
                      hipStream_t st);
int hbmr_tera_collect(const uint64_t* const* his, const uint64_t* const* los,
                      const uint32_t* const* rows, const long* starts, const long* prefix, int S,
                      long n, uint64_t* ohi, uint64_t* olo, uint32_t* osplit, uint32_t* orow,
                      hipStream_t st);
int hbmr_tera_collect_slots(const uint32_t* const* rows, const long* starts, const long* pre,
                            int S, int W, long C, uint32_t* osplit, uint32_t* orow,
                            hipStream_t st);
int hbmr_gather_records_multi(const void* const* bases, const uint32_t* split, const uint32_t* row,
                              const uint32_t* perm, long n, int record_bytes, void* dst,
                              hipStream_t st);
int hbmr_tera_collect_gid(const uint64_t* const* his, const uint32_t* const* rows,
                          const long* starts, const long* prefix, int S, long n, int pack,
                          uint64_t vlo, unsigned int m, unsigned int R, int sh, uint64_t* ohi,
                          uint32_t* ogid, hipStream_t st);
int hbmr_gather_records_gid(const void* const* bases, const uint32_t* gid, const uint64_t* packed,
                            long n, int record_bytes, void* dst, uint64_t* hi, uint64_t* lo,
                            uint32_t* win, hipStream_t st);
long hbmr_radix_onesweep_workspace_bytes(long n);
long hbmr_radix_onesweep_status_bytes(long n);
int hbmr_radix_sort_keys_u64(uint64_t* keys, uint64_t* tkeys, long n, int begin_bit, int end_bit,
                             void* ws, long ws_bytes, void* status, long status_bytes,
                             unsigned int* epoch, uint32_t* err, int copy_back, hipStream_t st);
long hbmr_tera_tie_fix_scratch_bytes(long cap, int record_bytes);
int hbmr_tera_group_stats(const uint64_t* hi, const uint64_t* lo, long n, const uint64_t* ph,
                          const uint64_t* pl, unsigned long long* acc, hipStream_t st);
int hbmr_tera_tie_fix_records(uint64_t* hi, uint64_t* lo, void* rec, long n, int record_bytes,
                              uint64_t vlo, unsigned int m, unsigned int R, int sh,
                              const uint32_t* win, unsigned int* flag, void* scratch, long cap,
                              hipStream_t st);
int hbmr_merge_path(const uint64_t* ahi, const uint64_t* alo, const uint32_t* av, long na,
                    const uint64_t* bhi, const uint64_t* blo, const uint32_t* bv, long nb,
                    uint64_t* ohi, uint64_t* olo, uint32_t* ov, hipStream_t st);
int hbmr_tera_tie_fix(const uint64_t* hi, uint64_t* lo, uint32_t* perm, long n,
                      unsigned int* flag, hipStream_t st);
int hbmr_tera_partition(const void* records, long n, int stride, const uint64_t* shi,
                        const uint64_t* slo, int nsplit, uint64_t* ohi, uint64_t* olo,
                        uint32_t* orow, long* offsets, unsigned long long* kmm, void* ws,
                        long ws_bytes, hipStream_t st);
#endif
long hbmr_radix_sort_workspace_bytes(long n);
long hbmr_tera_partition_workspace_bytes(long n, int nparts);

#ifndef HBMR_NO_HIP_DECLS
int hbmr_gemm_bf16_tn(const void* A, const void* Bt, void* C, long M, long N, long K, float alpha,
                      int out_bf16, hipStream_t st);
int hbmr_gemm_bf16_tn_ex(const void* A, const void* Bt, void* C, long M, long N, long K,
                         float alpha, int out_bf16, double* partials, hipStream_t st);
#endif
#ifndef HBMR_NO_HIP_DECLS
long hbmr_wc_tiles(long n);
int hbmr_wc_tokenize_count(const uint8_t* buf, long n, uint32_t* tile_counts, hipStream_t st);
int hbmr_wc_tokenize_write(const uint8_t* buf, long n, const long* tile_base, uint32_t* starts,
                           uint32_t* lens, hipStream_t st);
int hbmr_wc_insert(const uint8_t* buf, long n, const uint32_t* starts, const uint32_t* lens,
                   const int64_t* weights, long nwords, uint64_t* tkeys, uint64_t* tcounts,
                   long cap, int* overflow, hipStream_t st);
int hbmr_wc_compact(const uint8_t* buf, long n, const uint64_t* tkeys, const uint64_t* tcounts,
                    long cap, int R, uint32_t* ustart, uint32_t* ulen, int64_t* ucount,
                    int32_t* upart, unsigned int* counter, hipStream_t st);
int hbmr_wc_pack(const uint8_t* buf, const uint32_t* ustart, const uint32_t* ulen,
                 const int64_t* order, long nu, const int64_t* out_off, uint8_t* out,
                 hipStream_t st);
#endif
#ifndef HBMR_NO_HIP_DECLS
int hbmr_grep_cand_count(const uint8_t* buf, long n, const uint16_t* table,
                         const uint8_t* byteclass, int nstates, int nclasses, int start_bol,
                         int start_mid, uint32_t* tile_counts, int* non_ascii, hipStream_t st);
int hbmr_grep_cand_write(const uint8_t* buf, long n, const uint16_t* table,
                         const uint8_t* byteclass, int nstates, int nclasses, int start_bol,
                         int start_mid, const long* tile_base, uint32_t* pos, uint32_t* len,
                         int64_t* end, hipStream_t st);
long hbmr_grep_select_blocks(long nc);
int hbmr_grep_block_max(const int64_t* end, long nc, int64_t* block_max, hipStream_t st);
int hbmr_grep_prefix_max(const int64_t* end, long nc, const int64_t* block_prefix, int64_t* pmax,
                         hipStream_t st);
int hbmr_grep_select_count(const uint32_t* pos, const uint32_t* len, const int64_t* pmax, long nc,
                           uint32_t* block_counts, hipStream_t st);
int hbmr_grep_select_write(const uint32_t* pos, const uint32_t* len, const int64_t* pmax, long nc,
                           const long* block_base, uint32_t* spos, uint32_t* slen,
                           hipStream_t st);
int hbmr_span_insert(const uint8_t* buf, long n, const uint32_t* starts, const uint32_t* lens,
                     const int64_t* weights, long nspans, uint64_t* tkeys, uint64_t* tcounts,
                     long cap, int* overflow, hipStream_t st);
int hbmr_span_compact(const uint8_t* buf, const uint32_t* starts, const uint32_t* lens,
                      const uint64_t* tkeys, const uint64_t* tcounts, long cap, int R,
                      uint32_t* ustart, uint32_t* ulen, int64_t* ucount, int32_t* upart,
                      unsigned int* counter, hipStream_t st);
int hbmr_lines_count(const uint8_t* buf, long n, uint32_t* tile_counts, hipStream_t st);
int hbmr_lines_write(const uint8_t* buf, long n, const long* tile_base, uint32_t* starts,
                     uint32_t* lens, hipStream_t st);
int hbmr_recsort_hash_partition(const uint8_t* data, const int64_t* koff, const int64_t* klen,
                                long n, int nparts, uint32_t* part, hipStream_t st);
int hbmr_recsort_round_keys(const uint8_t* data, const int64_t* koff, const int64_t* klen,
                            const uint32_t* rec, long m, int d, uint64_t* keys, uint32_t* vals,
                            hipStream_t st);
long hbmr_recsort_round_workspace_bytes(long m);
int hbmr_recsort_round(const uint8_t* data, const int64_t* koff, const int64_t* klen, int d,
                       long m, int seg_bits, const uint32_t* act_pos, const uint32_t* act_rec,
                       const uint32_t* act_seg, uint32_t* perm, uint32_t* new_pos,
                       uint32_t* new_rec, uint32_t* new_seg, uint32_t* count, void* ws,
                       long ws_bytes, hipStream_t st);
int hbmr_recsort_cuts(const uint8_t* data, const int64_t* koff, const int64_t* klen,
                      const uint32_t* perm, long n, const uint8_t* sp, const int64_t* sp_off,
                      const int64_t* sp_len, int nsplit, int64_t* cuts, hipStream_t st);
int hbmr_recsort_chunk_bytes(void);
int hbmr_recsort_set_chunk_lanes(int lanes);
int hbmr_recsort_gather(const uint8_t* src, const uint32_t* perm, const int64_t* foff,
                        const int64_t* flen, const int64_t* dst_off, const int64_t* chunk_base,
                        const uint32_t* chunk_entry, long n, long nchunks, uint8_t* dst,
                        hipStream_t st);
#endif
int hbmr_kmeans_padded_k(int k);
long hbmr_kmeans_accum_workspace_bytes(long n, int k);
long hbmr_kmeans_batch_workspace_bytes(long total_n, int ntasks, int k);

int hbmr_kmeans_map_cpu_f32(const float* X, long n, int d, const float* C, int k,
                            int32_t* labels, long long* sums, long long* counts, double* cost,
                            int fx_shift, int nthreads);
int hbmr_kmeans_map_cpu_f32_ex(const float* X, long n, int d, const float* C, int k,
                               int32_t* labels, long long* sums, long long* counts, double* cost,
                               int fx_shift, int nthreads, int exact, long* rescored);

#ifdef __cplusplus
}
#endif
```

### native/kernels/kmeans.hip

```cpp
#include "common.h"
#include "../include/hbmr/hbmr.h"
#include <algorithm>
#include <cstdlib>
#include <cstring>
#include <type_traits>
#include "kmeans/assign.h"
#include "kmeans/grouped.h"
#include "kmeans/combine.h"
#include "kmeans/refine.h"
#include "kmeans/image.h"
#include "kmeans/refine_queue.h"
#include "kmeans/fused.h"
#include "kmeans/bounded.h"
#include "kmeans/launch.h"

extern "C" {

int hbmr_kmeans_assign_bf16(const void* X, long n, int dp, const void* C, const float* chalf,
                            int k_pad, int32_t* labels, float* scores, hipStream_t st) {
  return dispatch_dp(dp, [&](auto D) {
    return launch_assign<D()>(X, n, C, chalf, k_pad, labels, scores, st);
  });
}

// ... 55 lines not shown
  if (ntasks <= 0) return 0;
  if (zero_outputs) {
    HBMR_RETURN_IF_ERROR(hipMemsetAsync(sums, 0, (size_t)ntasks * k * dp * 8, st));
    HBMR_RETURN_IF_ERROR(hipMemsetAsync(counts, 0, (size_t)ntasks * k * 8, st));
  }
  long total = 0;
  for (int t = 0; t < ntasks; ++t) total += n[t];
  const bool small = ((size_t)k * AccCfg<128>::RS * 8 + (size_t)k * 4) <= 76 * 1024 && dp <= 128;
  if (!small && ntasks <= kMaxGroup && k <= 8192 &&
      ws_bytes >= hbmr_kmeans_batch_workspace_bytes(total, ntasks, k)) {
    set_lds_limits();
    return map_batch_grouped(ntasks, X, n, dp, C, chalf, k_pad, k, labels, ws, sums, counts,
                             fx_shift, st, cu_count());
  }
  long off = 0;
  for (int t = 0; t < ntasks; ++t) {
    int rc = hbmr_kmeans_assign_bf16(X[t], n[t], dp, C, chalf, k_pad, labels + off, nullptr, st);
    if (rc) return rc;
    rc = hbmr_kmeans_accum_bf16(X[t], n[t], dp, labels + off, k, sums + (size_t)t * k * dp,
                                counts + (size_t)t * k, fx_shift, ws, ws_bytes, 0, st);
    if (rc) return rc;
    off += n[t];
  }
  return 0;
}

long hbmr_kmeans_delta_workspace_bytes(long total_n, int ntasks, int k) {
  return (long)(2 * ws_align((size_t)ntasks * k * 4) + ws_align((size_t)ntasks * (k + 1) * 4) +
                ws_align((size_t)ntasks * 4) + 2 * ws_align((size_t)total_n * 8));
}

int hbmr_kmeans_delta_combine(int ntasks, const void* const* X, const long* n, int dp, int x_f32,
                              int k, const int32_t* labels, void* ws, long ws_bytes,
                              long long* sums, long long* counts, int fx_shift,
                              int32_t* const* g, const long long* const* S0,
                              const long long* const* N0, hipStream_t st) {
  if (ntasks <= 0) return 0;
  if (ntasks > kMaxGroup || k <= 0 || k > 8192 || (dp != 64 && dp != 128 && dp != 256))
    return (int)hipErrorInvalidValue;
  long total = 0;
  for (int i = 0; i < ntasks; ++i) {
    if (n[i] < 0 || n[i] >= (1L << 31)) return (int)hipErrorInvalidValue;
    total += n[i];
  }
  if (ws == nullptr || ws_bytes < hbmr_kmeans_delta_workspace_bytes(total, ntasks, k))
    return (int)hipErrorInvalidValue;
  set_lds_limits();
  return x_f32 ? delta_combine_impl<float>(ntasks, X, n, dp, k, labels, ws, sums, counts,
                                           fx_shift, g, S0, N0, st)
               : delta_combine_impl<__bf16>(ntasks, X, n, dp, k, labels, ws, sums, counts,
                                            fx_shift, g, S0, N0, st);
}

int hbmr_kmeans_map_batch_delta(int ntasks, const void* const* X, const long* n, int dp,
                                const void* C, const float* chalf, int k_pad, int k,
                                int32_t* labels, void* ws, long ws_bytes, long long* sums,
                                long long* counts, int fx_shift, int32_t* const* g,
                                const long long* const* S0, const long long* const* N0,
                                hipStream_t st) {
  if (ntasks <= 0) return 0;
  if (ntasks > kMaxGroup || k_pad % kCK) return (int)hipErrorInvalidValue;
  const int pts = assign_pts_of(dp);
  if (!pts) return (int)hipErrorInvalidValue;
  SplitTable t;
  make_split_table(t, ntasks, k, X, n);
  const long nb = split_blocks(t, [&](long m) { return (m + pts - 1) / pts; });
  if (nb > 0x7fffffffL) return (int)hipErrorInvalidValue;
  if (nb > 0) {
    launch_grouped_assign(dp, nb, t, C, chalf, k_pad, labels, st);
    HBMR_RETURN_IF_ERROR(hipGetLastError());
  }
  return hbmr_kmeans_delta_combine(ntasks, X, n, dp, 0, k, labels, ws, ws_bytes, sums, counts,
                                   fx_shift, g, S0, N0, st);
}

int hbmr_kmeans_assign_top3_bf16(const void* X, long n, int dp, const void* C, const float* chalf,
                                 int k_pad, int32_t* labels, int32_t* cand, float* scores,
                                 float* margin, hipStream_t st) {
  if (!labels || !cand || !scores || !margin) return (int)hipErrorInvalidValue;
  return dispatch_dp(dp, [&](auto D) {
    return launch_assign_top3<D(), false>(X, n, C, chalf, k_pad, labels, cand, scores, margin, st);
  });
}

int hbmr_kmeans_assign_top3_f16(const void* X, long n, int dp, const void* C, const float* chalf,
                                int k_pad, int32_t* labels, int32_t* cand, float* scores,
                                float* margin, hipStream_t st) {
  if (!labels || !cand || !scores || !margin) return (int)hipErrorInvalidValue;
  return dispatch_dp(dp, [&](auto D) {
    return launch_assign_top3<D(), true>(X, n, C, chalf, k_pad, labels, cand, scores, margin, st);
  });
}

int hbmr_kmeans_assign_top3_grouped(int nsplit, const void* const* X, const long* n, int dp,
                                    int f16, const void* C, const float* chalf, int k_pad,
                                    int32_t* labels, int32_t* cand, float* scores, float* margin,
                                    hipStream_t st) {
  if (!labels || !cand || !scores || !margin) return (int)hipErrorInvalidValue;
  return dispatch_dp(dp, [&](auto D) {
    return f16 ? launch_assign_top3_grouped<D(), true>(nsplit, X, n, C, chalf, k_pad, labels,
                                                       cand, scores, margin, st)
               : launch_assign_top3_grouped<D(), false>(nsplit, X, n, C, chalf, k_pad, labels,
                                                        cand, scores, margin, st);
  });
}

int hbmr_kmeans_assign_top3_q1_grouped(int nsplit, const void* const* X, const long* n, int dp,
                                       int f16, const void* C, const void* Ct,
                                       const float* chalf, int k_pad,
                                       int32_t* labels, const float* const* xnorm,
                                       const float* const* xbn2, const float* const* xerr,
                                       int d, int k, const float* cnorm, const float* cmax,
                                       const float* cerr, const float* cerrmax, void* ws,
                                       long ws_bytes, const float* dcc, hipStream_t st) {
  if (nsplit <= 0 || nsplit > kMaxGroup || k_pad % 32 || k <= 0 || k_pad < k ||
      d > kRefineMaxDp || !labels || ((uintptr_t)ws & 255) || (dp != 64 && dp != 128))
    return (int)hipErrorInvalidValue;
  TopQ1Table t;
  memset(&t, 0, sizeof(t));
  t.nsplit = nsplit;
  long total = 0, nb = 0;
  for (int i = 0; i < nsplit; ++i) {
    if (n[i] < 0 || n[i] > 0x7fffffffL) return (int)hipErrorInvalidValue;
    fill_topq1(t, i, X, xnorm, xbn2, xerr, total, nb);
    total += n[i];
    nb += ceil_div(n[i], kFusedPts);
  }
  t.off[nsplit] = total;
  t.blk[nsplit] = nb;
  const RefineLayout Ly = refine_layout(nsplit, n);
  if (ws_bytes < (long)Ly.bytes) return (int)hipErrorInvalidValue;
  char* w = static_cast<char*>(ws);
  HBMR_RETURN_IF_ERROR(hipMemsetAsync(w, 0, kHdrClear, st));
  if (nb == 0) return 0;
  if (nb > 0x7fffffffL) return (int)hipErrorInvalidValue;
  const FusedQ1Fin fin = make_fused_fin(k, d, k_pad, cnorm, cerr, dcc, cmax, cerrmax, w, Ly);
  if (exact_kernel() == 3) {
    if (!Ct) return (int)hipErrorInvalidValue;
    const auto [kern, lds] = fused_kernel(dp, f16, [](auto D, auto F) {
      return &kmeans_assign_top3_q1_v3_kernel<D(), F()>;
    });
    hipLaunchKernelGGL(kern, dim3((unsigned)nb), dim3(256), lds, st, t,
                       reinterpret_cast<const __bf16*>(Ct), chalf, k_pad / 32, labels, fin);
    return (int)hipGetLastError();
  }
  const auto [kern, lds] = fused_kernel(dp, f16, [](auto D, auto F) {
    return &kmeans_assign_top3_q1_grouped_kernel<D(), F()>;
  });
  hipLaunchKernelGGL(kern, dim3((unsigned)nb), dim3(AssignV2<64>::THREADS), lds, st, t,
                     reinterpret_cast<const __bf16*>(C), chalf, k_pad / 32, labels, fin);
  return (int)hipGetLastError();
}

long hbmr_kmeans_bound_workspace_bytes(long total, int nsplit, int k) {
  if (total < 0 || nsplit <= 0 || nsplit > kMaxGroup || k <= 0) return -1;
  const size_t sh = ((size_t)nsplit * k * sizeof(float) + 255) & ~(size_t)255;
  return (long)(kBoundHdr + sh + (size_t)total * sizeof(uint32_t));
}

int hbmr_kmeans_assign_top3_q1_bounded(int nsplit, const void* const* X, const long* n, int dp,
                                       int f16, const void* Ct, const float* chalf, int k_pad,
                                       int32_t* labels, const float* const* xnorm,
                                       const float* const* xbn2, const float* const* xerr,
                                       int d, int k, const float* cnorm, const float* cmax,
                                       const float* cerr, const float* cerrmax, void* ws,
                                       long ws_bytes, const float* dcc,
                                       const int32_t* const* g, float* const* gap,
                                       const float* const* ref, const float* cen, void* bws,
                                       long bws_bytes, unsigned long long* skipped,
                                       hipStream_t st) {
  if (nsplit <= 0 || nsplit > kMaxGroup || k_pad % 32 || k <= 0 || k_pad < k || d <= 0 ||
      d > kRefineMaxDp || !labels || ((uintptr_t)ws & 255) || (dp != 64 && dp != 128) || !Ct ||
      !g || !gap || !ref || !cen || !bws || ((uintptr_t)bws & 255))
    return (int)hipErrorInvalidValue;
  TopQ1Table t;
  SweepTable sw;
  GapTable gt;
  ShiftTable sh;
  memset(&t, 0, sizeof(t));
  memset(&sw, 0, sizeof(sw));
  memset(&gt, 0, sizeof(gt));
  memset(&sh, 0, sizeof(sh));
  t.nsplit = sw.nsplit = nsplit;
  long total = 0, nb = 0, nsb = 0;
  int nref = 0;
  for (int i = 0; i < nsplit; ++i) {
    if (n[i] < 0 || n[i] > 0x7fffffffL || (n[i] > 0 && (!gap[i] || (ref[i] && !g[i]))))
      return (int)hipErrorInvalidValue;
    fill_topq1(t, i, X, xnorm, xbn2, xerr, total, nb);
    sw.off[i] = total;
    sw.blk[i] = nsb;
    sw.n[i] = n[i];
    sw.g[i] = g[i];
    gt.gap[i] = gap[i];
    if (ref[i]) {
      int r = 0;
      while (r < nref && sh.ref[r] != ref[i]) ++r;
      if (r == nref) sh.ref[nref++] = ref[i];
      sw.rid[i] = r;
      sw.gap[i] = gap[i];
    }
    total += n[i];
    nb += ceil_div(n[i], kFusedPts);
    nsb += ceil_div(n[i], 256 * kSweepPer);
  }
  t.off[nsplit] = total;
  t.blk[nsplit] = nb;
  sw.blk[nsplit] = nsb;
  const RefineLayout Ly = refine_layout(nsplit, n);
  if (ws_bytes < (long)Ly.bytes ||
      bws_bytes < hbmr_kmeans_bound_workspace_bytes(total, nsplit, k))
    return (int)hipErrorInvalidValue;
  char* w = static_cast<char*>(ws);
  char* bw = static_cast<char*>(bws);
  HBMR_RETURN_IF_ERROR(hipMemsetAsync(w, 0, kHdrClear, st));
  if (nb == 0) return 0;
  if (nb > 0x7fffffffL) return (int)hipErrorInvalidValue;
  HBMR_RETURN_IF_ERROR(hipMemsetAsync(bw, 0, kBoundHdr, st));
  uint32_t* cnt = reinterpret_cast<uint32_t*>(bw);
  uint32_t* smax = cnt + kMaxGroup;
  float* shift = reinterpret_cast<float*>(bw + kBoundHdr);
  uint32_t* idx = reinterpret_cast<uint32_t*>(
      bw + kBoundHdr + (((size_t)nsplit * k * sizeof(float) + 255) & ~(size_t)255));
  if (nref > 0) {
    hipLaunchKernelGGL(kmeans_bound_shift_kernel, dim3((unsigned)k, (unsigned)nref), dim3(64), 0,
                       st, sh, cen, k, d, shift, smax);
    HBMR_RETURN_IF_ERROR(hipGetLastError());
  }
  hipLaunchKernelGGL(kmeans_bound_sweep_kernel, dim3((unsigned)nsb), dim3(256), 0, st, sw, k,
                     shift, reinterpret_cast<const float*>(smax), labels, cnt, idx);
  HBMR_RETURN_IF_ERROR(hipGetLastError());
  const FusedQ1Fin fin = make_fused_fin(k, d, k_pad, cnorm, cerr, dcc, cmax, cerrmax, w, Ly);
  const auto [kern, lds] = fused_kernel(dp, f16, [](auto D, auto F) {
    return &kmeans_assign_top3_q1_bounded_kernel<D(), F()>;
  });
  hipLaunchKernelGGL(kern, dim3((unsigned)nb), dim3(256), lds, st, t, gt,
                     reinterpret_cast<const __bf16*>(Ct), chalf, k_pad / 32, labels, fin,
                     (const uint32_t*)cnt, (const uint32_t*)idx, skipped);
  return (int)hipGetLastError();
}

int hbmr_kmeans_refine_f32(const float* X32, long n, int d, int ldx, const float* xnorm,
                           const float* xbn2, const float* xerr, const float* C32, int k,
                           int k_pad, const float* cnorm, const float* cmax, const float* cerr,
                           const float* cerrmax, const int32_t* nbr_idx,
                           const float* nbr_dist, int L, int32_t* labels, const int32_t* cand,
                           const float* scores, const float* margin, unsigned long long* stats,
                           int nstats, hipStream_t st) {
  if (n <= 0) return 0;
  if (d > ldx || d > kRefineMaxDp || k <= 0 || k_pad < k || L < 1 || L > k)
    return (int)hipErrorInvalidValue;
  const double pack_rel = pack_rel_of(k_pad);
  const long blocks = (n + 255) / 256;
  const bool v2_ok = d % 8 == 0 && ldx % 4 == 0 && ((uintptr_t)X32 & 15) == 0 &&
                     ((uintptr_t)C32 & 15) == 0;
  if (v2_ok) {
    auto kern = d <= 128 ? kmeans_refine_v2_kernel<1> : kmeans_refine_v2_kernel<2>;
    hipLaunchKernelGGL(kern, dim3((unsigned)blocks), dim3(256), 0, st, X32, n, d, ldx, xnorm,
                       xbn2, xerr, C32, k, cnorm, cmax, cerr, cerrmax, pack_rel, nbr_idx,
                       nbr_dist, L, labels, cand, scores, margin, stats, nstats);
    return (int)hipGetLastError();
  }
  hipLaunchKernelGGL(kmeans_refine_kernel, dim3((unsigned)blocks), dim3(256), 0, st, X32, n, d,
                     ldx, xnorm, xbn2, xerr, C32, k, cnorm, cmax, cerr, cerrmax, pack_rel,
                     nbr_idx, nbr_dist, L,
                     labels, cand, scores, margin, stats, nstats);
  return (int)hipGetLastError();
}


int hbmr_kmeans_exact_prep(const float* x, long n, int d, int ldx, int dp, int f16, void* x16,
                           float* xnorm, float* xn2, float* xerr, hipStream_t st) {
  if (n <= 0) return 0;
  if (d > ldx || d > dp || dp % 8 || !x16 || !xnorm || !xn2 || !xerr)
    return (int)hipErrorInvalidValue;
  const long blocks = (n + 15) / 16;
  if (blocks > 0x7fffffffL) return (int)hipErrorInvalidValue;
  hipLaunchKernelGGL(kmeans_exact_prep_kernel, dim3((unsigned)blocks), dim3(256), 0, st, x, n, d,
                     ldx, dp, f16, reinterpret_cast<uint16_t*>(x16), xnorm, xn2, xerr);
  return (int)hipGetLastError();
}

int hbmr_kmeans_set_exact_kernel(int v) {
  const int old = g_exact_kernel;
  g_exact_kernel = v == 2 || v == 3 ? v : -1;
  return old;
}

int hbmr_kmeans_get_exact_kernel(void) { return exact_kernel(); }

int hbmr_kmeans_image16_tiled(const void* c16, int k_pad, int dp, void* c16t, hipStream_t st) {
  if (k_pad <= 0 || k_pad % 32 || (dp != 64 && dp != 128) || !c16 || !c16t)
    return (int)hipErrorInvalidValue;
  const long pieces = (long)k_pad * dp / 8;
  hipLaunchKernelGGL(kmeans_image16_tiled_kernel, dim3((unsigned)((pieces + 255) / 256)),
                     dim3(256), 0, st, reinterpret_cast<const uint4*>(c16), k_pad, dp,
                     reinterpret_cast<uint4*>(c16t));
  return (int)hipGetLastError();
}

int hbmr_kmeans_image16(const float* cen, int k, int d, int dp, int k_pad, int f16, void* c16,
                        float* chalf, float* cnorm, float* cerr, float* maxima, hipStream_t st) {
  if (k <= 0 || k_pad < k || d > dp) return (int)hipErrorInvalidValue;
  HBMR_RETURN_IF_ERROR(hipMemsetAsync(maxima, 0, 2 * sizeof(float), st));
  hipLaunchKernelGGL(kmeans_image16_kernel, dim3((unsigned)k_pad), dim3(128), 0, st, cen, k, d,
                     dp, f16, reinterpret_cast<uint16_t*>(c16), chalf, cnorm, cerr,
                     reinterpret_cast<unsigned*>(maxima));
  return (int)hipGetLastError();
}

int hbmr_kmeans_centroid_nbr(const float* cen, int k, int d, int L, int32_t* di, float* dv,
                             float* pd, hipStream_t st) {
  if (k <= 0 || k > kNbrMaxK || d <= 0 || d > kNbrMaxD || L <= 0 || L > k)
    return (int)hipErrorInvalidValue;
  if (((uintptr_t)cen & 15) != 0) return (int)hipErrorInvalidValue;
  int kp2 = 1;
  while (kp2 < k) kp2 <<= 1;
  const size_t lds = (size_t)kp2 * sizeof(unsigned long long);
  static bool lds_set = false;
  if (!lds_set) {
    HBMR_RETURN_IF_ERROR(hipFuncSetAttribute((const void*)kmeans_centroid_nbr_kernel,
                                             hipFuncAttributeMaxDynamicSharedMemorySize,
                                             (int)(kNbrMaxK * sizeof(unsigned long long))));
    lds_set = true;
  }
  const double rel = (double)(d + 4) * 0x1p-53 * 1.01;
  hipLaunchKernelGGL(kmeans_centroid_nbr_kernel, dim3((unsigned)k), dim3(kNbrThreads), lds, st,
                     cen, k, d, L, kp2, rel, di, dv, pd);
  return (int)hipGetLastError();
}


long hbmr_kmeans_refine_batch_bytes(int nsplit, const long* ns) {
  if (nsplit <= 0 || nsplit > kMaxGroup) return -1;
  return (long)refine_layout(nsplit, ns).bytes;
}

int hbmr_kmeans_refine_batch_q1(int nsplit, const long* ns, int s, int d, int k, int k_pad,
                                const float* xnorm, const float* xbn2, const float* xerr,
                                const float* cnorm, const float* cmax, const float* cerr,
                                const float* cerrmax, const int32_t* labels, const int32_t* cand,
                                const float* scores, const float* margin,
                                unsigned long long* stats, void* ws, long ws_bytes, int reset,
                                const float* dcc, hipStream_t st) {
  if (nsplit <= 0 || nsplit > kMaxGroup || s < 0 || s >= nsplit || k <= 0 || k_pad < k ||
      d > kRefineMaxDp || ((uintptr_t)ws & 255))
    return (int)hipErrorInvalidValue;
  for (int i = 0; i < nsplit; ++i)
    if (ns[i] < 0 || ns[i] > 0x7fffffffL) return (int)hipErrorInvalidValue;
  const RefineLayout Ly = refine_layout(nsplit, ns);
  if (ws_bytes < (long)Ly.bytes) return (int)hipErrorInvalidValue;
  char* w = static_cast<char*>(ws);
  uint32_t* c1 = reinterpret_cast<uint32_t*>(w);
  if (reset) HBMR_RETURN_IF_ERROR(hipMemsetAsync(c1, 0, kHdrClear, st));
  const long n = ns[s];
  if (n == 0) return 0;
  const double pack_rel = pack_rel_of(k_pad);
  const long b1 = ceil_div(n, 256 * kQ1Per);
  hipLaunchKernelGGL(kmeans_refine_q1_kernel, dim3((unsigned)b1), dim3(256), 0, st, n, s, d, k,
                     xnorm, xbn2, xerr, cnorm, cmax, cerr, cerrmax, pack_rel, labels, cand,
                     scores, margin, c1, reinterpret_cast<ExactQ1*>(w + Ly.off1), Ly.cap1,
                     reinterpret_cast<unsigned long long*>(w + kStatsOff), dcc);
  return (int)hipGetLastError();
}

int hbmr_kmeans_refine_batch_q1g(int nsplit, const long* ns, int d, int k, int k_pad,
                                 const float* const* xnorm, const float* const* xbn2,
                                 const float* const* xerr, const float* cnorm, const float* cmax,
                                 const float* cerr, const float* cerrmax, const int32_t* labels,
                                 const int32_t* cand, const float* scores, const float* margin,
                                 void* ws, long ws_bytes, const float* dcc, hipStream_t st) {
  if (nsplit <= 0 || nsplit > kMaxGroup || k <= 0 || k_pad < k || d > kRefineMaxDp ||
      ((uintptr_t)ws & 255))
    return (int)hipErrorInvalidValue;
  Q1Table t;
  memset(&t, 0, sizeof(t));
  t.nsplit = nsplit;
  long total = 0, nb = 0;
  for (int i = 0; i < nsplit; ++i) {
    if (ns[i] < 0 || ns[i] > 0x7fffffffL) return (int)hipErrorInvalidValue;
    t.n[i] = ns[i];
    fill_topq1(t, i, nullptr, xnorm, xbn2, xerr, total, nb);
    total += ns[i];
    nb += ceil_div(ns[i], 256 * kQ1Per);
  }
  t.blk[nsplit] = nb;
  t.total = total;
  const RefineLayout Ly = refine_layout(nsplit, ns);
  if (ws_bytes < (long)Ly.bytes) return (int)hipErrorInvalidValue;
  char* w = static_cast<char*>(ws);
  uint32_t* c1 = reinterpret_cast<uint32_t*>(w);
  HBMR_RETURN_IF_ERROR(hipMemsetAsync(c1, 0, kHdrClear, st));
  if (nb == 0) return 0;
  const double pack_rel = pack_rel_of(k_pad);
  hipLaunchKernelGGL(kmeans_refine_q1_grouped_kernel, dim3((unsigned)nb), dim3(256), 0, st, t, d,
                     k, cnorm, cmax, cerr, cerrmax, pack_rel, labels, cand, scores, margin, c1,
                     reinterpret_cast<ExactQ1*>(w + Ly.off1), Ly.cap1,
                     reinterpret_cast<unsigned long long*>(w + kStatsOff), dcc);
  return (int)hipGetLastError();
}

int hbmr_kmeans_refine_batch_finish(int nsplit, const long* ns, const float* const* x32,
                                    int32_t* const* labels, int d, int ldx, const float* C32,
                                    int k, int k_pad, const float* cmax, const float* cerrmax,
                                    const int32_t* nbr_idx, const float* nbr_dist, int L,
                                    unsigned long long* stats, int nstats, void* ws,
                                    long ws_bytes, hipStream_t st) {
  if (nsplit <= 0 || nsplit > kMaxGroup || d > ldx || d > kRefineMaxDp || d % 8 || ldx % 4 ||
      k <= 0 || k_pad < k || L < 1 || L > k || nstats < 3 || ((uintptr_t)C32 & 15) ||
      ((uintptr_t)ws & 255))
    return (int)hipErrorInvalidValue;
  const RefineLayout Ly = refine_layout(nsplit, ns);
  if (ws_bytes < (long)Ly.bytes) return (int)hipErrorInvalidValue;
  RefineTable tbl;
  std::memset(&tbl, 0, sizeof(tbl));
  tbl.nsplit = nsplit;
  for (int i = 0; i < nsplit; ++i) {
    if ((uintptr_t)x32[i] & 15) return (int)hipErrorInvalidValue;
    tbl.x32[i] = x32[i];
    tbl.labels[i] = labels[i];
  }
  const double pack_rel = pack_rel_of(k_pad);
  char* w = static_cast<char*>(ws);
  uint32_t* c1 = reinterpret_cast<uint32_t*>(w);
  uint32_t* c2 = c1 + kQShards;
  const ExactQ1* q1 = reinterpret_cast<const ExactQ1*>(w + Ly.off1);
  ExactQ2* q2 = reinterpret_cast<ExactQ2*>(w + Ly.off2);
  unsigned long long* ss = reinterpret_cast<unsigned long long*>(w + kStatsOff);
  const unsigned g3 = std::max(1u, Ly.g2);
  if (d <= 128) {
    hipLaunchKernelGGL(kmeans_refine_q2_kernel<1>, dim3(Ly.g2), dim3(256), 0, st, tbl, d, ldx,
                       C32, k, cmax, cerrmax, pack_rel, c1, q1, Ly.cap1, c2, q2, Ly.cap2, ss);
    HBMR_RETURN_IF_ERROR(hipGetLastError());
    hipLaunchKernelGGL(kmeans_refine_q3_kernel<1>, dim3(g3), dim3(256), 0, st, tbl, d, ldx, C32,
                       k, nbr_idx, nbr_dist, L, c2, q2, Ly.cap2, ss, nstats);
  } else {
    hipLaunchKernelGGL(kmeans_refine_q2_kernel<2>, dim3(Ly.g2), dim3(256), 0, st, tbl, d, ldx,
                       C32, k, cmax, cerrmax, pack_rel, c1, q1, Ly.cap1, c2, q2, Ly.cap2, ss);
    HBMR_RETURN_IF_ERROR(hipGetLastError());
    hipLaunchKernelGGL(kmeans_refine_q3_kernel<2>, dim3(g3), dim3(256), 0, st, tbl, d, ldx, C32,
                       k, nbr_idx, nbr_dist, L, c2, q2, Ly.cap2, ss, nstats);
  }
  HBMR_RETURN_IF_ERROR(hipGetLastError());
  hipLaunchKernelGGL(kmeans_refine_stats_kernel, dim3(1), dim3(64), 0, st, ss, stats, nstats);
  return (int)hipGetLastError();
}

}
```

### native/kernels/kmeans/bounded.h

```cpp
#pragma once
#include "../common.h"
#include "fused.h"

namespace {

constexpr int kSweepPer = 8;
constexpr int kBoundHdr = 512;

struct ShiftTable {
  const float* ref[kMaxGroup];
};

__global__ __launch_bounds__(64) void kmeans_bound_shift_kernel(
    const ShiftTable tbl, const float* __restrict__ cen, int k, int d, float* __restrict__ shift,
    uint32_t* __restrict__ smax) {
  const int j = blockIdx.x, r = blockIdx.y;
  const float* a = cen + (size_t)j * d;
  const float* b = tbl.ref[r] + (size_t)j * d;
  double acc = 0.0;
  for (int i = threadIdx.x; i < d; i += 64) {
    const double e = (double)a[i] - (double)b[i];
    acc = fma(e, e, acc);
  }
#pragma unroll
  for (int off = 1; off < 64; off <<= 1) acc += __shfl_xor(acc, off);
  if (threadIdx.x == 0) {
    const float s = __double2float_ru(sqrt(acc) * (1.0 + 0x1p-40));
    shift[(size_t)r * k + j] = s;
    atomicMax(smax + r, __float_as_uint(s));
  }
}

__device__ __forceinline__ float sub_rd_pos(float a, float b) {
  const float t = a - b;
  if (!(t > 0x1p-100f)) return 0.f;
  const float bb = t - a;
  const float err = (a - (t - bb)) - (b + bb);
  return err < 0.f ? __uint_as_float(__float_as_uint(t) - 1u) : t;
}

struct SweepTable {
  int nsplit;
  const int32_t* g[kMaxGroup];
  float* gap[kMaxGroup];
  int rid[kMaxGroup];
  long n[kMaxGroup];
  long off[kMaxGroup];
  long blk[kMaxGroup + 1];
};

__global__ __launch_bounds__(256) void kmeans_bound_sweep_kernel(
    const SweepTable tbl, int k, const float* __restrict__ shift,
    const float* __restrict__ smax, int32_t* __restrict__ labels, uint32_t* __restrict__ cnt,
    uint32_t* __restrict__ idx) {
  const long b = blockIdx.x;
  int lo = 0, hi = tbl.nsplit;
  while (hi - lo > 1) {
    const int mid = (lo + hi) >> 1;
    if (tbl.blk[mid] <= b) lo = mid; else hi = mid;
  }
  const int s = __builtin_amdgcn_readfirstlane(lo);
  const int tid = threadIdx.x, lane = tid & 63, wave = tid >> 6;
  const long n = tbl.n[s], o = tbl.off[s];
  const int32_t* __restrict__ g = tbl.g[s];
  float* __restrict__ gap = tbl.gap[s];
  const float* __restrict__ sh = shift + (size_t)tbl.rid[s] * k;
  const float sm = gap ? smax[tbl.rid[s]] : 0.f;
  const long p0 = (b - tbl.blk[s]) * (256 * kSweepPer);
  __shared__ uint32_t wcnt[4][kSweepPer];
  __shared__ uint32_t base_s;
  bool list[kSweepPer];
  uint32_t rank[kSweepPer];
#pragma unroll
  for (int i = 0; i < kSweepPer; ++i) {
    const long p = p0 + i * 256 + tid;
    list[i] = false;
    if (p < n) {
      list[i] = true;
      if (gap) {
        const int32_t c = g[p];
        const float v =
            (uint32_t)c < (uint32_t)k ? sub_rd_pos(sub_rd_pos(gap[p], sh[c]), sm) : 0.f;
        if (v > 0.f) {
          list[i] = false;
          labels[o + p] = c;
          gap[p] = v;
        }
      }
    }
    const unsigned long long m = __ballot(list[i]);
    rank[i] = lane_rank(m);
    if (lane == 0) wcnt[wave][i] = (uint32_t)__popcll(m);
  }
  __syncthreads();
  if (tid == 0) {
    uint32_t tot = 0;
#pragma unroll
    for (int w = 0; w < 4; ++w)
#pragma unroll
      for (int i = 0; i < kSweepPer; ++i) {
        const uint32_t c = wcnt[w][i];
        wcnt[w][i] = tot;
        tot += c;
      }
    base_s = tot ? atomicAdd(cnt + s, tot) : 0u;
  }
  __syncthreads();
  uint32_t* out = idx + o + base_s;
#pragma unroll
  for (int i = 0; i < kSweepPer; ++i)
    if (list[i]) out[wcnt[wave][i] + rank[i]] = (uint32_t)(p0 + i * 256 + tid);
}

struct GapTable {
  float* gap[kMaxGroup];
};

template <int D, bool F16>
__global__ __launch_bounds__(256, kExactMinB) void kmeans_assign_top3_q1_bounded_kernel(
    const TopQ1Table tbl, const GapTable gt, const __bf16* __restrict__ Ct,
    const float* __restrict__ chalf, int ntiles, int32_t* __restrict__ labels, FusedQ1Fin fin,
    const uint32_t* __restrict__ cnt, const uint32_t* __restrict__ idx,
    unsigned long long* __restrict__ skipped) {
  extern __shared__ __attribute__((aligned(16))) char smem[];
  if (blockIdx.x == 0 && threadIdx.x == 0 && skipped != nullptr) {
    unsigned long long sk = 0;
    for (int i = 0; i < tbl.nsplit; ++i)
      sk += (unsigned long long)(tbl.off[i + 1] - tbl.off[i]) - cnt[i];
    if (sk) atomicAdd(skipped, sk);
  }
  const long b = hbmr_xcd_remap(blockIdx.x, gridDim.x);
  int lo = 0, hi = tbl.nsplit;
  while (hi - lo > 1) {
    const int mid = (lo + hi) >> 1;
    if (tbl.blk[mid] <= b) lo = mid; else hi = mid;
  }
  const int s = __builtin_amdgcn_readfirstlane(lo);
  const long nl = (long)__builtin_amdgcn_readfirstlane(cnt[s]);
  const long lb = b - tbl.blk[s];
  if (lb * 256 >= nl) return;
  const long o = tbl.off[s];
  fin.xnorm = tbl.xnorm[s];
  fin.xbn2 = tbl.xbn2[s];
  fin.xerr = tbl.xerr[s];
  fin.sidx = s;
  fin.idx = idx + o;
  fin.gap = gt.gap[s];
  assign_tile_v3<D, F16, true>(tbl.X[s], nl, Ct, chalf, ntiles, labels + o, lb, smem, fin);
}


}
```

### native/kernels/kmeans/fused.h

```cpp
#pragma once
#include "../common.h"
#include "assign.h"
#include "grouped.h"
#include "refine_queue.h"

namespace {

struct FusedQ1Fin {
  const float* xnorm;
  const float* xbn2;
  const float* xerr;
  int sidx;
  int k;
  double gam, pack_rel;
  const float* cmax_p;
  const float* cerrmax_p;
  const float* cnorm;
  const float* cerr;
  const float* dcc;
  uint32_t* qcount;
  ExactQ1* q1;
  long cap1;
  unsigned long long* stats;
  const uint32_t* idx;
  float* gap;

  template <class AM, int PB, bool BND = false>
  __device__ __forceinline__ void operator()(const AM (&am)[PB], int h, long p0, int col, long n,
                                             int32_t* __restrict__ labels) const {
    const int tid = threadIdx.x, lane = tid & 63, wave = tid >> 6;
    __shared__ uint32_t fq_cnt[4 * PB];
    __shared__ uint32_t fq_base;
    const int shard = blockIdx.x % kQShards;
    const double inflate = 1.0 + 0x1p-20;
    const double cem = (double)cerrmax_p[0] * inflate;
    const double cm = (double)cmax_p[0] * inflate + cem;
    ExactQ1 e[PB];
    bool flag[PB];
    uint32_t rank[PB];
#pragma unroll
    for (int pb = 0; pb < PB; ++pb) {
      float v[3];
      int c[3];
      am[pb].top3(v[0], v[1], v[2]);
#pragma unroll
      for (int i = 0; i < 3; ++i) c[i] = am[pb].cluster(v[i], h);
      float ov[3];
      int oc[3];
#pragma unroll
      for (int i = 0; i < 3; ++i) {
        ov[i] = __shfl_xor(v[i], 32);
        oc[i] = __shfl_xor(c[i], 32);
      }
#pragma unroll
      for (int i = 0; i < 3; ++i) insert3(v, c, ov[i], oc[i]);
      if (((c[0] ^ c[1]) & AM::TMASK) == 0) {
        v[2] = v[0];
        c[2] = c[0];
      }
      const long p = p0 + pb * 32 + col;
      flag[pb] = false;
      if (h == 0 && p < n) {
        long row = p;
        if constexpr (BND) row = idx[p];
        labels[row] = c[0];
        const float bs = am[pb].score(v[0]);
        const float m2 = bs - am[pb].score(v[1]);
        ExactQ1& q = e[pb];
        q.row = (uint32_t)row;
        q.split = (uint32_t)sidx;
        q.b = c[0];
        q.s = c[1];
        q.t = c[2];
        q.sb = bs;
        q.m3 = bs - am[pb].score(v[2]);
        q.x2 = xbn2[row];
        q.xn = xnorm[row];
        q.xe = xerr[row];
        q.pad0 = q.pad1 = 0.f;
        if constexpr (BND) {
          float gp = 0.f;
          flag[pb] = q.s < k && q1_certify<true>(q, m2, cnorm[q.b], cerr[q.b], k, gam, cm, cem,
                                                 pack_rel, cnorm, cerr, dcc, gp);
          gap[row] = gp;
        } else {
          flag[pb] = q.s < k && q1_flagged(q, m2, cnorm[q.b], cerr[q.b], k, gam, cm, cem,
                                           pack_rel, cnorm, cerr, dcc);
        }
      }
      const unsigned long long m = __ballot(flag[pb]);
      rank[pb] = lane_rank(m);
      if (lane == 0) fq_cnt[wave * PB + pb] = (uint32_t)__popcll(m);
    }
    __syncthreads();
    if (tid == 0) {
      uint32_t tot = 0;
#pragma unroll
      for (int i = 0; i < 4 * PB; ++i) {
        const uint32_t c = fq_cnt[i];
        fq_cnt[i] = tot;
        tot += c;
      }
      fq_base = tot ? atomicAdd(qcount + shard, tot) : 0u;
      if (tot) atomicAdd(stats + 4 * shard, (unsigned long long)tot);
    }
    __syncthreads();
    ExactQ1* out = q1 + (long)shard * cap1 + fq_base;
#pragma unroll
    for (int pb = 0; pb < PB; ++pb)
      if (flag[pb]) out[fq_cnt[wave * PB + pb] + rank[pb]] = e[pb];
  }
};

template <int D>
__device__ __forceinline__ void stage_tile32t(char* buf, const __bf16* __restrict__ Ct,
                                              const float* __restrict__ chalf, int tile, int wave,
                                              int lane) {
  using V = AssignV2<D>;
  const uint32_t loff = (uint32_t)lane * 16u;
#pragma unroll
  for (int i = 0; i < V::P; ++i) {
    const int base = (i * V::WAVES + wave) * HBMR_WAVE;
    const char* g = reinterpret_cast<const char*>(Ct) + (size_t)tile * V::TILE_BYTES +
                    (size_t)base * 16;
    __builtin_amdgcn_global_load_lds((const void*)(g + loff), (void*)(buf + base * 16), 16, 0, 0);
  }
  if (wave == 0 && lane < 32) {
    const char* g = reinterpret_cast<const char*>(chalf + (size_t)tile * 32);
    __builtin_amdgcn_global_load_lds((const void*)(g + loff / 4u), (void*)(buf + V::TILE_BYTES),
                                     4, 0, 0);
  }
}

__device__ __forceinline__ void tile_codes(uint32_t top, int t, uint32_t (&code)[16]) {
  const uint32_t base = top - ((uint32_t)t << 4);
#pragma unroll
  for (int r = 0; r < 16; ++r) {
    code[r] = base | (15u - r);
    asm("" : "+s"(code[r]));
  }
}

__device__ __forceinline__ void top2_insert(PackedTop2x8& am, const f32x16& acc,
                                            const uint32_t (&code)[16], uint32_t vmask) {
  constexpr int NT = PackedTop2x8::NT;
#pragma unroll
  for (int r = 0; r < 16; ++r) {
    if ((r / NT) % 2) continue;
    const float u = __uint_as_float((__float_as_uint(acc[r]) & vmask) | code[r]);
    const float v = __uint_as_float((__float_as_uint(acc[r + NT]) & vmask) | code[r + NT]);
    const float m = vmed3(am.tb[r % NT], u, v);
    am.ts[r % NT] = vmax3(m, am.ts[r % NT], am.ts[r % NT]);
    am.tb[r % NT] = vmax3(am.tb[r % NT], u, v);
  }
}

template <int D, bool F16, bool BND = false>
__device__ __forceinline__ void assign_tile_v3(const __bf16* __restrict__ X, long n,
                                               const __bf16* __restrict__ Ct,
                                               const float* __restrict__ chalf, int ntiles,
                                               int32_t* __restrict__ labels, long blk, char* smem,
                                               const FusedQ1Fin& fin) {
  static_assert(D <= 128, "v3 keeps two 32-point blocks of D <= 128 in registers");
  constexpr int PB = 2, NS = 4;
  using V = AssignV2<D, NS>;
  static_assert(V::WAVES == 4, "v3: 4 waves per workgroup");
  constexpr int KS = V::KS;
  static_assert(V::TILE_BYTES == 32 * D * 2, "tile layout");
  const int tid = threadIdx.x;
  const int wave = __builtin_amdgcn_readfirstlane(tid / HBMR_WAVE);
  const int lane = tid & (HBMR_WAVE - 1);
  const int h = lane >> 5;
  const int col = lane & 31;
  const long p0 = blk * (V::WAVES * PB * 32) + (long)wave * PB * 32;
  const int rowoff = h * 512 + col * 16;
  auto frag = [&](const char* row, int s) __attribute__((always_inline)) {
    return *reinterpret_cast<const bf16x8*>(row + s * 1024);
  };
  auto bias = [&](const char* buf, f32x16& acc) __attribute__((always_inline)) {
    const float* ch = reinterpret_cast<const float*>(buf + V::TILE_BYTES);
#pragma unroll
    for (int g = 0; g < 4; ++g) {
      const f32x4 v = *reinterpret_cast<const f32x4*>(ch + 8 * g + 4 * h);
      acc[4 * g + 0] = v[0];
      acc[4 * g + 1] = v[1];
      acc[4 * g + 2] = v[2];
      acc[4 * g + 3] = v[3];
    }
  };

#pragma unroll
  for (int i = 0; i < NS; ++i)
    if (i < ntiles) stage_tile32t<D>(smem + i * V::BUF, Ct, chalf, i, wave, lane);

  bf16x8 bfrag[PB][KS];
#pragma unroll
  for (int pb = 0; pb < PB; ++pb) {
    long p = p0 + pb * 32 + col;
    if (p >= n) p = n - 1;
    if constexpr (BND) p = fin.idx[p];
    const uint4* row = reinterpret_cast<const uint4*>(X + p * D);
#pragma unroll
    for (int s = 0; s < KS; ++s) bfrag[pb][s] = __builtin_bit_cast(bf16x8, row[2 * s + h]);
  }
  PackedTop2x8 am[PB];
#pragma unroll
  for (int pb = 0; pb < PB; ++pb) am[pb].init(ntiles);
  asm volatile("s_waitcnt vmcnt(0)" ::: "memory");
#pragma unroll
  for (int pb = 0; pb < PB; ++pb)
#pragma unroll
    for (int s = 0; s < KS; ++s) asm volatile("" : "+v"(bfrag[pb][s]));
  __syncthreads();
  const bool w0 = wave == 0;
  const uint32_t top = am[0].top;
  const uint32_t vmask = am[0].vmask;

  bf16x8 a[KS];
  f32x16 bz;
  {
    const char* row = smem + rowoff;
#pragma unroll
    for (int s = 0; s < KS; ++s) a[s] = frag(row, s);
    bias(smem, bz);
  }
  int slot = 0;
  for (int t = 0; t < ntiles; ++t) {
    wait_tile_dmas<V::P, NS - 2>(max(0, min(NS - 2, ntiles - 2 - t)), w0);
    asm volatile("s_waitcnt lgkmcnt(0)" ::: "memory");
    __syncthreads();
    char* rbuf = smem + slot * V::BUF;
    if (t + NS < ntiles) stage_tile32t<D>(rbuf, Ct, chalf, t + NS, wave, lane);
    slot = slot + 1 == NS ? 0 : slot + 1;
    const char* nbuf = smem + slot * V::BUF;
    const char* nrow = nbuf + rowoff;
    f32x16 acc[PB];
#pragma unroll
// ... 71 lines not shown
```

### native/kernels/kmeans/refine_queue.h

```cpp
#pragma once
#include "../common.h"
#include <algorithm>
#include "grouped.h"
#include "refine.h"

namespace {

struct ExactQ1 {
  uint32_t row, split;
  int32_t b, s, t;
  float sb, m3, x2, xn, xe, pad0, pad1;
};
struct ExactQ2 {
  uint32_t row, split;
  int32_t w, pad;
  double dw;
};
static_assert(sizeof(ExactQ1) == 48 && sizeof(ExactQ2) == 24, "queue entry layout");

constexpr int kQShards = 8;
constexpr int kQ1Per = 4;
constexpr int kQ2Lanes = 8;
constexpr int kQ2Per = HBMR_WAVE / kQ2Lanes;
constexpr int kRefineGrid = 2048;
constexpr int kStatsOff = 64;
constexpr int kRefineHdr = 512;
constexpr int kHdrClear = kStatsOff + kQShards * 4 * 8;

struct RefineTable {
  int nsplit;
  const float* x32[kMaxGroup];
  int32_t* labels[kMaxGroup];
};

__host__ __device__ inline long ceil_div(long a, long b) { return (a + b - 1) / b; }

struct RefineLayout {
  long cap1, cap2;
  unsigned g2;
  size_t off1, off2, bytes;
};
inline RefineLayout refine_layout(int nsplit, const long* ns) {
  RefineLayout L;
  long total = 0, cap1 = 0, nb_fused = 0;
  for (int i = 0; i < nsplit; ++i) {
    total += ns[i];
    cap1 += ceil_div(ceil_div(ns[i], 256 * kQ1Per), kQShards) * 256 * kQ1Per;
    nb_fused += ceil_div(ns[i], 256);
  }
  L.cap1 = std::max<long>(cap1, ceil_div(nb_fused, kQShards) * 256);
  L.g2 = (unsigned)std::max<long>(1, std::min<long>(kRefineGrid, ceil_div(total, 4 * kQ2Per)));
  const long per_iter = (long)L.g2 * 4 * kQ2Per;
  L.cap2 = ceil_div(L.g2, kQShards) * 4 * kQ2Per * std::max<long>(1, ceil_div(total, per_iter));
  L.off1 = kRefineHdr;
  L.off2 = L.off1 + ((kQShards * (size_t)L.cap1 * sizeof(ExactQ1) + 255) & ~(size_t)255);
  L.bytes = L.off2 + kQShards * (size_t)L.cap2 * sizeof(ExactQ2);
  return L;
}

__device__ __forceinline__ long shard_slot(const uint32_t (&c)[kQShards], long cap, uint32_t i) {
  uint32_t acc = 0;
  long slot = 0;
#pragma unroll
  for (int j = 0; j < kQShards; ++j) {
    if (i >= acc && i < acc + c[j]) slot = (long)j * cap + (i - acc);
    acc += c[j];
  }
  return slot;
}

__device__ __forceinline__ uint32_t lane_rank(unsigned long long m) {
  return __builtin_amdgcn_mbcnt_hi((uint32_t)(m >> 32), __builtin_amdgcn_mbcnt_lo((uint32_t)m, 0u));
}

template <bool GAP>
__device__ __forceinline__ bool q1_certify(const ExactQ1& e, float m2, float cnb, float ceb, int k,
                                           double gam, double cm, double cem, double pack_rel,
                                           const float* __restrict__ cnorm,
                                           const float* __restrict__ cerr,
                                           const float* __restrict__ dcc, float& gap) {
  const double inflate = 1.0 + 0x1p-20;
  const double xn = ((double)e.xn + (double)e.xe) * inflate;
  const double x2 = (double)e.x2;
  const double sb = e.sb;
  const double mm = m2;
  const double amax = ((double)e.xe + cem) * inflate;
  double eb, es, dl_b, dl_s;
  exact_bound(sb, ((double)cnb + (double)ceb) * inflate, xn, x2,
              ((double)e.xe + (double)ceb) * inflate, gam, pack_rel, eb, dl_b);
  exact_bound(sb - mm, cm, xn, x2, amax, gam, pack_rel, es, dl_s);
  bool flag = !(mm > eb + es && dl_s >= 2.0 * amax);
  double marg = mm - (eb + es);
  const int b = e.b, sc = e.s, t = e.t;
  if (flag && dcc != nullptr && t < k && t != b) {
    const double ex = (double)e.xe * inflate;
    const double ebb = (double)ceb * inflate;
    const double ess = (double)cerr[sc] * inflate;
    const double dbs = ((double)dcc[(size_t)b * k + sc] + (double)ceb + (double)cerr[sc]) *
                       inflate;
    double eap_b, rb, eap_s, rs;
    score_err(sb, ((double)cnb + (double)ceb) * inflate, xn, x2, gam, pack_rel, eap_b, rb);
    score_err(sb - mm, ((double)cnorm[sc] + (double)cerr[sc]) * inflate, xn, x2, gam,
              pack_rel, eap_s, rs);
    const double ep = dbs * ex + rs * ess + rb * ebb + 0.5 * (ex + ebb) * (ex + ebb) +
                      eap_b + eap_s;
    double et, dl_t;
    const double m3 = e.m3;
    exact_bound(sb - m3, cm, xn, x2, amax, gam, pack_rel, et, dl_t);
    if (mm > ep && m3 > eb + et && dl_t >= 2.0 * amax) {
      flag = false;
      if constexpr (GAP) marg = fmin(mm - ep, m3 - (eb + et));
    }
  }
  if constexpr (GAP) {
    gap = 0.f;
    if (!flag && marg > 0.0) {
      const double ctb = ((double)cnb + (double)ceb) * inflate;
      const double eacc = gam * (xn * ctb + 0.5 * ctb * ctb);
      const double slack = 2.0 * (eacc + fabs(sb) * pack_rel) + x2 * 0x1p-22;
      const double r = sqrt(fmax(0.0, x2 - 2.0 * sb) + slack) * (1.0 + 0x1p-40) +
                       ((double)e.xe + (double)ceb) * inflate;
      const double delta = 2.0 * marg * (1.0 - 0x1p-30);
      const double g = delta / (sqrt(r * r + delta) * (1.0 + 0x1p-40) + r) * (1.0 - 0x1p-30);
      gap = fmaxf(0.f, __double2float_rd(g));
    }
  }
  return flag;
}

__device__ __forceinline__ bool q1_flagged(const ExactQ1& e, float m2, float cnb, float ceb, int k,
                                           double gam, double cm, double cem, double pack_rel,
                                           const float* __restrict__ cnorm,
                                           const float* __restrict__ cerr,
                                           const float* __restrict__ dcc) {
  float unused;
  return q1_certify<false>(e, m2, cnb, ceb, k, gam, cm, cem, pack_rel, cnorm, cerr, dcc, unused);
}

__device__ __forceinline__ void refine_q1_block(
    long n, int sidx, long blk, int d, int k, const float* __restrict__ xnorm,
    const float* __restrict__ xbn2, const float* __restrict__ xerr,
    const float* __restrict__ cnorm, const float* __restrict__ cmax,
    const float* __restrict__ cerr, const float* __restrict__ cerrmax, double pack_rel,
    const int32_t* __restrict__ labels, const int32_t* __restrict__ cand,
    const float* __restrict__ score, const float* __restrict__ margin, long cs,
    uint32_t* __restrict__ qcount, ExactQ1* __restrict__ q1, long cap1,
    unsigned long long* __restrict__ stats, const float* __restrict__ dcc) {
  const int tid = threadIdx.x, lane = tid & 63, wave = tid >> 6;
  const int shard = blockIdx.x % kQShards;
  __shared__ uint32_t wcnt[4][kQ1Per];
  __shared__ uint32_t base_s;
  const double inflate = 1.0 + 0x1p-20;
  const double gam = (double)(d + 2) * 0x1p-23 * 1.01;
  const double cem = (double)cerrmax[0] * inflate;
  const double cm = (double)cmax[0] * inflate + cem;
  ExactQ1 e[kQ1Per];
  bool in[kQ1Per];
  float m2[kQ1Per];
#pragma unroll
  for (int i = 0; i < kQ1Per; ++i) {
    const long p = blk * (256 * kQ1Per) + i * 256 + tid;
    in[i] = p < n;
    const long q = in[i] ? p : n - 1;
    e[i].row = (uint32_t)q;
    e[i].split = (uint32_t)sidx;
    e[i].b = labels[q];
    e[i].s = cand[q];
    e[i].t = cand[cs + q];
    e[i].sb = score[q];
    m2[i] = margin[q];
    e[i].m3 = margin[cs + q];
    e[i].x2 = xbn2[q];
    e[i].xn = xnorm[q];
    e[i].xe = xerr[q];
  }
  float cnb[kQ1Per], ceb[kQ1Per];
#pragma unroll
  for (int i = 0; i < kQ1Per; ++i) {
    cnb[i] = cnorm[e[i].b];
    ceb[i] = cerr[e[i].b];
  }
  bool flag[kQ1Per];
  uint32_t rank[kQ1Per];
#pragma unroll
  for (int i = 0; i < kQ1Per; ++i) {
    flag[i] = in[i] && e[i].s < k &&
              q1_flagged(e[i], m2[i], cnb[i], ceb[i], k, gam, cm, cem, pack_rel, cnorm, cerr, dcc);
    const unsigned long long m = __ballot(flag[i]);
    rank[i] = lane_rank(m);
    if (lane == 0) wcnt[wave][i] = (uint32_t)__popcll(m);
  }
  __syncthreads();
  if (tid == 0) {
    uint32_t tot = 0;
#pragma unroll
    for (int w = 0; w < 4; ++w)
#pragma unroll
      for (int i = 0; i < kQ1Per; ++i) {
        const uint32_t c = wcnt[w][i];
        wcnt[w][i] = tot;
        tot += c;
      }
    base_s = tot ? atomicAdd(qcount + shard, tot) : 0u;
    if (tot) atomicAdd(stats + 4 * shard, (unsigned long long)tot);
  }
  __syncthreads();
  ExactQ1* out = q1 + (long)shard * cap1 + base_s;
#pragma unroll
  for (int i = 0; i < kQ1Per; ++i)
    if (flag[i]) out[wcnt[wave][i] + rank[i]] = e[i];
}

__global__ __launch_bounds__(256) void kmeans_refine_q1_kernel(
    long n, int sidx, int d, int k, const float* __restrict__ xnorm,
    const float* __restrict__ xbn2, const float* __restrict__ xerr,
    const float* __restrict__ cnorm, const float* __restrict__ cmax,
    const float* __restrict__ cerr, const float* __restrict__ cerrmax, double pack_rel,
    const int32_t* __restrict__ labels, const int32_t* __restrict__ cand,
    const float* __restrict__ score, const float* __restrict__ margin,
    uint32_t* __restrict__ qcount, ExactQ1* __restrict__ q1, long cap1,
    unsigned long long* __restrict__ stats, const float* __restrict__ dcc) {
  refine_q1_block(n, sidx, blockIdx.x, d, k, xnorm, xbn2, xerr, cnorm, cmax, cerr, cerrmax,
                  pack_rel, labels, cand, score, margin, n, qcount, q1, cap1, stats, dcc);
}

struct Q1Table {
  int nsplit;
  long total;
  long n[kMaxGroup];
  long off[kMaxGroup];
  long blk[kMaxGroup + 1];
  const float* xnorm[kMaxGroup];
  const float* xbn2[kMaxGroup];
  const float* xerr[kMaxGroup];
};

__global__ __launch_bounds__(256) void kmeans_refine_q1_grouped_kernel(
    const Q1Table tbl, int d, int k, const float* __restrict__ cnorm,
    const float* __restrict__ cmax, const float* __restrict__ cerr,
    const float* __restrict__ cerrmax, double pack_rel, const int32_t* __restrict__ labels,
    const int32_t* __restrict__ cand, const float* __restrict__ score,
    const float* __restrict__ margin, uint32_t* __restrict__ qcount, ExactQ1* __restrict__ q1,
    long cap1, unsigned long long* __restrict__ stats, const float* __restrict__ dcc) {
  const long b = blockIdx.x;
  int lo = 0, hi = tbl.nsplit;
  while (hi - lo > 1) {
    const int mid = (lo + hi) >> 1;
    if (tbl.blk[mid] <= b) lo = mid; else hi = mid;
  }
  const int s = __builtin_amdgcn_readfirstlane(lo);
  const long o = tbl.off[s];
  refine_q1_block(tbl.n[s], s, b - tbl.blk[s], d, k, tbl.xnorm[s], tbl.xbn2[s], tbl.xerr[s],
                  cnorm, cmax, cerr, cerrmax, pack_rel, labels + o, cand + o, score + o,
                  margin + o, tbl.total, qcount, q1, cap1, stats, dcc);
}

template <int NM>
__device__ __forceinline__ void load_row16(const float* __restrict__ r, int d, int sub,
                                           float (&v)[16 * NM]) {
#pragma unroll
  for (int m = 0; m < NM; ++m) {
#pragma unroll
    for (int h = 0; h < 4; ++h) {
      const int b = 128 * m + 32 * h + 4 * sub;
      const bool ok = b < d;
      const float4 a = *reinterpret_cast<const float4*>(r + (ok ? b : 0));
      float* o = v + 16 * m + 4 * h;
      o[0] = ok ? a.x : 0.f; o[1] = ok ? a.y : 0.f; o[2] = ok ? a.z : 0.f; o[3] = ok ? a.w : 0.f;
    }
  }
}

__device__ __forceinline__ float row_sum8f(float v) {
  v += __shfl_xor(v, 1);
  v += __shfl_xor(v, 2);
  v += __shfl_xor(v, 4);
  return v;
}

__device__ __forceinline__ double row_sum8(double v) {
  v += dpp_f64<0xB1>(v);
  v += dpp_f64<0x4E>(v);
  v += dpp_f64<0x141>(v);
  return v;
}

template <int NM>
__global__ __launch_bounds__(256) void kmeans_refine_q2_kernel(
    const RefineTable tbl, int d, int ldx, const float* __restrict__ C32, int k,
    const float* __restrict__ cmax, const float* __restrict__ cerrmax, double pack_rel,
    const uint32_t* __restrict__ qcount, const ExactQ1* __restrict__ q1, long cap1,
    uint32_t* __restrict__ q2count, ExactQ2* __restrict__ q2, long cap2,
    unsigned long long* __restrict__ sstats) {
  constexpr uint32_t kPerBlk = 4 * kQ2Per;
  constexpr uint32_t kBuf = 256;
  const int tid = threadIdx.x, lane = tid & 63, wave = tid >> 6;
  const int grp = lane / kQ2Lanes, sub = lane % kQ2Lanes;
  __shared__ ExactQ2 sbuf[kBuf];
  __shared__ uint32_t sn, sbase;
  __shared__ unsigned long long cnt[2];
  if (tid < 2) cnt[tid] = 0;
  if (tid == 0) sn = 0;
  __syncthreads();
  const double inflate = 1.0 + 0x1p-20;
  const double gam = (double)(d + 2) * 0x1p-23 * 1.01;
  const double cem = (double)cerrmax[0] * inflate;
  const double cm = (double)cmax[0] * inflate + cem;
  uint32_t c1[kQShards];
  uint32_t total = 0;
#pragma unroll
  for (int j = 0; j < kQShards; ++j) {
    c1[j] = qcount[j];
    total += c1[j];
  }
  const int shard = blockIdx.x % kQShards;
  const uint32_t stride = gridDim.x * kPerBlk;
  const uint32_t off = wave * kQ2Per + grp;
  auto flush = [&]() {
    if (tid == 0) {
      sbase = atomicAdd(q2count + shard, sn);
      cnt[1] += sn;
    }
    __syncthreads();
    const uint32_t m = sn;
    for (uint32_t i = tid; i < m; i += 256) q2[(long)shard * cap2 + sbase + i] = sbuf[i];
    __syncthreads();
    if (tid == 0) sn = 0;
    __syncthreads();
  };
  uint32_t bb = blockIdx.x * kPerBlk;
  ExactQ1 e;
  if (bb < total) e = q1[shard_slot(c1, cap1, min(bb + off, total - 1))];
  for (; bb < total; bb += stride) {
    const ExactQ1 q = e;
    const bool have = bb + off < total;
    const uint32_t nb = bb + stride;
    if (nb < total) e = q1[shard_slot(c1, cap1, min(nb + off, total - 1))];
    const bool t_real = q.t < k;
    const float* xr = tbl.x32[q.split] + (size_t)q.row * ldx;
    float xf[16 * NM], c0[16 * NM], c1r[16 * NM], c2[16 * NM];
    load_row16<NM>(xr, d, sub, xf);
    load_row16<NM>(C32 + (size_t)q.b * d, d, sub, c0);
    load_row16<NM>(C32 + (size_t)q.s * d, d, sub, c1r);
    load_row16<NM>(C32 + (size_t)(t_real ? q.t : q.b) * d, d, sub, c2);
    float f0 = 0.f, f1 = 0.f, f2 = 0.f;
#pragma unroll
    for (int i = 0; i < 16 * NM; ++i) {
      const float e0 = xf[i] - c0[i], e1 = xf[i] - c1r[i], e2 = xf[i] - c2[i];
      f0 = fmaf(e0, e0, f0);
      f1 = fmaf(e1, e1, f1);
      f2 = fmaf(e2, e2, f2);
    }
    f0 = row_sum8f(f0);
    f1 = row_sum8f(f1);
    f2 = row_sum8f(f2);
    const double rel = (double)(16 * NM + 8) * 0x1p-24 * 1.01, aeps = 0x1p-120;
    int w = q.b;
    double dw = f0;
    if ((double)f1 < dw || ((double)f1 == dw && q.s < w)) { w = q.s; dw = f1; }
    if (t_real && ((double)f2 < dw || ((double)f2 == dw && q.t < w))) { w = q.t; dw = f2; }
    const double whi = dw * (1.0 + rel) + aeps;
    auto beats = [&](double dj) { return dj * (1.0 - rel) - aeps > whi; };
    bool separated = isfinite(whi) &&
                     (w == q.b || beats(f0)) && (w == q.s || beats(f1)) &&
                     (!t_real || w == q.t || beats(f2));
    dw = whi;
    bool certified = !t_real && separated;
    if (t_real && separated) {
      const double xn = ((double)q.xn + (double)q.xe) * inflate;
      const double x2 = (double)q.x2;
      const double amax = ((double)q.xe + cem) * inflate;
      const double st = (double)q.sb - (double)q.m3;
      double et, dl_t;
      exact_bound(st, cm, xn, x2, amax, gam, pack_rel, et, dl_t);
      certified = 0.5 * (x2 - dw) - x2 * 0x1p-23 > st + et && dl_t >= 2.0 * amax;
    }
    if (have && sub == 0 && certified && w != q.b) {
      tbl.labels[q.split][q.row] = w;
      atomicAdd(&cnt[0], 1ull);
    }
    const bool spill = have && sub == 0 && !certified;
    const unsigned long long m = __ballot(spill);
    if (m) {
      uint32_t b2 = 0;
      if (lane == 0) b2 = atomicAdd(&sn, (uint32_t)__popcll(m));
      b2 = __shfl(b2, 0);
      if (spill) {
        ExactQ2 o;
        o.row = q.row;
        o.split = q.split;
        o.w = w;
        o.pad = 0;
        o.dw = dw;
        sbuf[b2 + lane_rank(m)] = o;
      }
    }
    __syncthreads();
    if (sn > kBuf - kPerBlk) flush();
  }
  __syncthreads();
  if (sn) flush();
  if (tid < 2 && cnt[tid]) atomicAdd(sstats + 4 * shard + 1 + tid, cnt[tid]);
}

template <int NM>
__global__ __launch_bounds__(256) void kmeans_refine_q3_kernel(
    const RefineTable tbl, int d, int ldx, const float* __restrict__ C32, int k,
    const int32_t* __restrict__ nbr_idx, const float* __restrict__ nbr_dist, int L,
    const uint32_t* __restrict__ q2count, const ExactQ2* __restrict__ q2, long cap2,
    unsigned long long* __restrict__ sstats, int nstats) {
  const int tid = threadIdx.x, lane = tid & 63;
  const int grp = lane / kRefineGroup, sub = lane % kRefineGroup;
  __shared__ unsigned long long cnt[3];
  if (tid < 3) cnt[tid] = 0;
  __syncthreads();
  uint32_t c2[kQShards];
  uint32_t total = 0;
#pragma unroll
  for (int j = 0; j < kQShards; ++j) {
    c2[j] = q2count[j];
    total += c2[j];
  }
  const uint32_t nwaves = gridDim.x * 4;
  const uint32_t gw = blockIdx.x * 4 + (tid >> 6);
  for (uint32_t base = gw * 4; base < total; base += nwaves * 4) {
    const uint32_t idx = base + grp;
    const bool have = idx < total;
    const ExactQ2 q = q2[shard_slot(c2, cap2, have ? idx : base)];
    int32_t* lab = tbl.labels[q.split];
    const int b0 = lab[q.row];
    double xv[8 * NM];
    {
      float xf[8 * NM];
      load_row8<NM>(tbl.x32[q.split] + (size_t)q.row * ldx, d, sub, xf);
#pragma unroll
      for (int i = 0; i < 8 * NM; ++i) xv[i] = (double)xf[i];
    }
    const int w0 = q.w;
    int w = w0;
    double dw;
    {
      const float* c0p[1] = {C32 + (size_t)w0 * d};
      double d0[1];
      rows_dist2<NM, 1>(xv, c0p, d, sub, d0);
      dw = d0[0];
    }
    const double r0 = sqrt(dw);
    bool done = false;
    const int32_t* ni = nbr_idx + (size_t)w0 * L;
    const float* nd = nbr_dist + (size_t)w0 * L;
    const float* cw0 = C32 + (size_t)w0 * d;
    int evals = 0;
    for (int jj = 0; jj < L; jj += kElkanStep) {
      const double lim = (r0 + sqrt(dw)) * (1.0 + 0x1p-40);
      if ((double)nd[jj] > lim) {
        done = true;
        break;
      }
      int jv[kElkanStep];
      const float* cp[kElkanStep];
#pragma unroll
      for (int v = 0; v < kElkanStep; ++v) {
        const bool ok = jj + v < L && (double)nd[jj + v] <= lim;
        jv[v] = ok ? ni[jj + v] : -1;
        cp[v] = ok ? C32 + (size_t)jv[v] * d : cw0;
      }
      double dj[kElkanStep];
      rows_dist2<NM, kElkanStep>(xv, cp, d, sub, dj);
      evals += kElkanStep;
#pragma unroll
      for (int v = 0; v < kElkanStep; ++v)
        if (jv[v] >= 0 && (dj[v] < dw || (dj[v] == dw && jv[v] < w))) { w = jv[v]; dw = dj[v]; }
    }
    const bool full = !done && L < k;
    if (full) {
      for (int j = 0; j < k; j += 4) {
        const float* cp[4];
#pragma unroll
        for (int v = 0; v < 4; ++v) cp[v] = C32 + (size_t)(j + v < k ? j + v : j) * d;
        double dj[4];
        rows_dist2<NM, 4>(xv, cp, d, sub, dj);
#pragma unroll
        for (int v = 0; v < 4; ++v)
          if (j + v < k && (dj[v] < dw || (dj[v] == dw && j + v < w))) { w = j + v; dw = dj[v]; }
      }
    }
    if (have && sub == 0) {
      atomicAdd(&cnt[1], (unsigned long long)evals);
      if (full) atomicAdd(&cnt[2], 1ull);
      if (w != b0) atomicAdd(&cnt[0], 1ull);
      lab[q.row] = w;
    }
  }
  __syncthreads();
  const int sh = blockIdx.x % (kQShards / 2);
  if (tid == 0 && cnt[0]) atomicAdd(sstats + 4 * sh + 1, cnt[0]);
  if (tid == 1 && cnt[1]) atomicAdd(sstats + 4 * sh + 3, cnt[1]);
  if (tid == 2 && cnt[2]) atomicAdd(sstats + 4 * (sh + kQShards / 2) + 3, cnt[2]);
}

__global__ void kmeans_refine_stats_kernel(const unsigned long long* __restrict__ ss,
                                           unsigned long long* __restrict__ stats, int nstats) {
  const int t = threadIdx.x;
  if (t >= 5 || (t >= 3 && nstats < 5)) return;
  unsigned long long v = 0;
  if (t < 3) {
    for (int j = 0; j < kQShards; ++j) v += ss[4 * j + t];
  } else {
    for (int j = 0; j < kQShards / 2; ++j) v += ss[4 * (j + (t - 3) * (kQShards / 2)) + 3];
  }
  if (v) stats[t] += v;
}

}
```

Before: 10150.

## Stash top-3 candidates and radius bound to skip re-scoring stable points

When exact bounded assignment certifies a point, it now stores that point's three candidate centroids and a lower radius bound in each baseline. On later iterations, points whose bounds still hold but whose stash is valid are re-checked only against the stashed three centroids inside the q2 refine kernel, avoiding the full top-3 scan. Stashes that fail the radius test are invalidated. This adds per-point memory (4 int16 plus 1 float), a larger workspace queue, and extra counters, and it is on by default.

```diff
diff --git a/hbmr/models/kmeans.py b/hbmr/models/kmeans.py
--- a/hbmr/models/kmeans.py
+++ b/hbmr/models/kmeans.py
@@ -29,6 +29,7 @@
 EXACT_MFMA_KEY = "hbmr.kmeans.exact.mfma"
 COMBINER_KEY = "hbmr.kmeans.combiner"
 BOUNDS_KEY = "hbmr.kmeans.exact.bounds"
+STASH_KEY = "hbmr.kmeans.exact.bounds.stash"
 
 _M32 = 0xFFFFFFFF
 
@@ -238,8 +239,8 @@
 
 
 def _baseline_bytes(b) -> int:
-    return sum(t.numel() * t.element_size() for t in (b.g, b.S0, b.N0, getattr(b, "gap", None))
-               if t is not None)
+    return sum(t.numel() * t.element_size()
+               for t in (b.g, b.S0, b.N0, b.gap, b.cand, b.rlow) if t is not None)
 
 
 def _drop_baselines(split_key, device):
@@ -288,7 +289,7 @@
     with _EXACT_LOCK:
         t = _EXACT_SKIPPED.get(key)
         if t is None:
-            t = _EXACT_SKIPPED[key] = torch.zeros(1, dtype=torch.int64, device=device)
+            t = _EXACT_SKIPPED[key] = torch.zeros(3, dtype=torch.int64, device=device)
         return t
 
 
@@ -311,6 +312,7 @@
         self.exact_dtype = torch.bfloat16 if (conf.get(EXACT_MFMA_KEY) or "f16").lower() in (
             "bf16", "bfloat16") else torch.float16
         self.bounds = conf.get_boolean(BOUNDS_KEY, True)
+        self.stash = conf.get_boolean(STASH_KEY, True)
         self.combiner = (conf.get(COMBINER_KEY) or "delta").lower()
         if self.combiner not in ("delta", "sorted"):
             raise ValueError(f"{COMBINER_KEY} must be delta or sorted, not {self.combiner!r}")
@@ -569,11 +571,15 @@
             hb = [bases[i] for i in have]
             bounded = self.bounds and self.combiner == "delta" and km.bounds_supported(img)
             if bounded:
-                nogap = [b for b in hb if b.gap is None]
+                def bound_bytes(b):
+                    return sum(t.numel() * t.element_size() for t in (b.gap, b.cand, b.rlow)
+                               if t is not None)
+                before = {id(b): bound_bytes(b) for b in hb}
                 km.assign_exact_batch([datas[i] for i in have], img, stats, lab, scratch,
                                       stream=ctx.stream, bounds=hb,
-                                      skipped=_exact_skipped(self.cin, ctx.device))
-                grown = {id(b): b.gap.numel() * b.gap.element_size() for b in nogap}
+                                      skipped=_exact_skipped(self.cin, ctx.device),
+                                      stash=self.stash)
+                grown = {id(b): max(0, bound_bytes(b) - before[id(b)]) for b in hb}
             else:
                 km.assign_exact_batch([datas[i] for i in have], img, stats, lab, scratch,
                                       stream=ctx.stream)
@@ -705,11 +711,13 @@
             if est is not None:
                 vals += list(est.double().unbind(0))
             if esk is not None:
-                vals.append(esk[0].double())
+                vals += list(esk.double().unbind(0))
             got = torch.stack(vals).tolist()
             shift, npts = got[0], got[1]
             if esk is not None:
-                ctx.reporter.incrCounter("KMEANS", "EXACT_BOUND_SKIPPED_POINTS", int(got[-1]))
+                for name, v in zip(("EXACT_BOUND_SKIPPED_POINTS", "EXACT_STASH_POINTS",
+                                    "EXACT_STASH_INVALIDATED"), got[-3:]):
+                    ctx.reporter.incrCounter("KMEANS", name, int(v))
             if est is not None:
                 for name, v in zip(("EXACT_FLAGGED_POINTS", "EXACT_RELABELLED_POINTS",
                                     "EXACT_NEIGHBOUR_SCANS"), got[2:5]):
diff --git a/hbmr/ops/_lib.py b/hbmr/ops/_lib.py
--- a/hbmr/ops/_lib.py
+++ b/hbmr/ops/_lib.py
@@ -44,6 +44,19 @@
                                                    c_void_p, c_long, c_void_p,
                                                    c_void_p, c_void_p, c_void_p, c_void_p,
                                                    c_void_p, c_long, c_void_p, c_void_p]),
+    "hbmr_kmeans_assign_top3_q1_bounded_stash": (c_int, [c_int, c_void_p, c_void_p, c_int, c_int,
+                                                         c_void_p, c_void_p, c_int, c_void_p,
+                                                         c_void_p, c_void_p, c_void_p, c_int,
+                                                         c_int, c_void_p, c_void_p, c_void_p,
+                                                         c_void_p, c_void_p, c_long, c_void_p,
+                                                         c_void_p, c_void_p, c_void_p, c_void_p,
+                                                         c_void_p, c_long, c_void_p, c_void_p,
+                                                         c_void_p, c_void_p, c_void_p]),
+    "hbmr_kmeans_refine_batch_finish_stash": (c_int, [c_int, c_void_p, c_void_p, c_void_p, c_int,
+                                                      c_int, c_void_p, c_int, c_int, c_void_p,
+                                                      c_void_p, c_void_p, c_void_p, c_int,
+                                                      c_void_p, c_int, c_void_p, c_long, c_void_p,
+                                                      c_long, c_void_p, c_void_p, c_void_p]),
     "hbmr_kmeans_centroid_nbr": (c_int, [c_void_p, c_int, c_int, c_int, c_void_p, c_void_p,
                                          c_void_p, c_void_p]),
     "hbmr_kmeans_image16": (c_int, [c_void_p, c_int, c_int, c_int, c_int, c_int, c_void_p,
diff --git a/hbmr/ops/kmeans.py b/hbmr/ops/kmeans.py
--- a/hbmr/ops/kmeans.py
+++ b/hbmr/ops/kmeans.py
@@ -348,7 +348,7 @@
             _ptr(self.ws), self.ws.numel(), int(i == 0), _ptr(self.pd), self.st)
         _lib.check(rc, "hbmr_kmeans_refine_batch_q1")
 
-    def finish(self):
+    def finish(self, stash=None):
         B = len(self.splits)
         img = self.img
         _, cmax, _, cemax = self.norms
@@ -356,6 +356,15 @@
         xs = (ctypes.c_void_p * B)(*[sp.x32.data_ptr() for sp in self.splits])
         ls = (ctypes.c_void_p * B)(*[(lp.value if isinstance(lp, ctypes.c_void_p) else lp)
                                      for lp in self.labels])
+        if stash is not None:
+            bws, rlows, inval = stash
+            rc = self.lib.hbmr_kmeans_refine_batch_finish_stash(
+                B, self.ns, xs, ls, img.d, self.splits[0].x32.shape[1], _ptr(img.cen), img.k,
+                img.k_pad, _ptr(cmax), _ptr(cemax), _ptr(ni), _ptr(nd), L, _ptr(self.stats),
+                self.stats.numel(), _ptr(self.ws), self.ws.numel(), _ptr(bws), bws.numel(),
+                rlows, inval, self.st)
+            _lib.check(rc, "hbmr_kmeans_refine_batch_finish_stash")
+            return
         rc = self.lib.hbmr_kmeans_refine_batch_finish(
             B, self.ns, xs, ls, img.d, self.splits[0].x32.shape[1], _ptr(img.cen), img.k,
             img.k_pad, _ptr(cmax), _ptr(cemax), _ptr(ni), _ptr(nd), L, _ptr(self.stats),
@@ -411,9 +420,12 @@
         img.cen.is_cuda and _lib.load().hbmr_kmeans_get_exact_kernel() == 3
 
 
+STASH_MAX_K = 0xffff
+
+
 def assign_exact_batch(splits: list, img: CentroidImage, stats: torch.Tensor, out: torch.Tensor,
                        scratch: dict | None = None, stream=None, bounds: list | None = None,
-                       skipped: torch.Tensor | None = None) -> None:
+                       skipped: torch.Tensor | None = None, stash: bool = False) -> None:
     if not splits:
         return
     _check_refine_dim(img)
@@ -463,7 +475,7 @@
             off += _exact_group(group, img, stats, base + 4 * off, c16, ch, (cn, cmax, ce, cemax),
                                 dt, scratch, stream, lib, st,
                                 None if bounds is None else bounds[g0:g0 + MAX_REFINE_BATCH],
-                                skipped, newref)
+                                skipped, newref, stash and img.k <= STASH_MAX_K)
             continue
         rb = _RefineBatch(group, img, stats, scratch, stream) if REFINE_VERSION >= 3 else None
         for i, sp in enumerate(group):
@@ -491,7 +503,7 @@
 
 
 def _bounded_group(group, bases, img, labels_ptr, ch, norms, dt, scratch, stream, lib, st, rb,
-                   skipped, newref):
+                   skipped, newref, stash=False):
     B = len(group)
     ns = [sp.shape[0] for sp in group]
     N = sum(ns)
@@ -507,12 +519,20 @@
         for b in bases:
             if b.gap is None:
                 b.gap, b.ref = torch.empty(b.g.numel(), dtype=torch.float32, device=dev), None
+            if not stash:
+                b.cand = b.rlow = None
+            elif b.cand is None or b.rlow is None:
+                b.cand = torch.zeros(b.g.numel(), 4, dtype=torch.int16, device=dev)
+                b.rlow = torch.zeros(b.g.numel(), dtype=torch.float32, device=dev)
         for b, n in zip(bases, ns):
             if b.g.numel() != n or b.gap.numel() != n or \
+                    (stash and (b.rlow.numel() != n or b.cand.numel() != 4 * n or
+                                b.cand.dtype != torch.int16 or b.rlow.dtype != torch.float32 or
+                                not b.cand.is_contiguous())) or \
                     (b.ref is not None and (tuple(b.ref.shape) != tuple(img.cen.shape) or
                                             not b.ref.is_contiguous())):
                 raise ValueError("bounds: baseline does not match its split / the centroids")
-            for t in (b.g, b.gap, b.ref):
+            for t in (b.g, b.gap, b.ref, b.cand, b.rlow):
                 if t is not None:
                     base = t._base if t._base is not None else t
                     blocks[id(base)] = base
@@ -527,7 +547,12 @@
     refs = [b.ref for b in bases]
     for b in bases:
         b.ref = b.pending = None
-    rc = lib.hbmr_kmeans_assign_top3_q1_bounded(
+    cands = rlows = None
+    if stash:
+        cands = P(*[b.cand.data_ptr() for b in bases])
+        rlows = P(*[b.rlow.data_ptr() for b in bases])
+    more = skipped is not None and skipped.numel() >= 3
+    rc = lib.hbmr_kmeans_assign_top3_q1_bounded_stash(
         B, P(*[sp.xb.data_ptr() for sp in group]), (ctypes.c_long * B)(*ns), img.dp,
         int(dt == torch.float16), _ptr(img.image16_tiled(dt)), _ptr(ch), img.k_pad, labels_ptr,
         P(*[sp.xnorm.data_ptr() for sp in group]), P(*[sp.xbn2.data_ptr() for sp in group]),
@@ -535,14 +560,18 @@
         _ptr(cemax), _ptr(rb.ws), rb.ws.numel(), _ptr(rb.pd),
         P(*[b.g.data_ptr() for b in bases]), P(*[b.gap.data_ptr() for b in bases]),
         P(*[None if r is None else r.data_ptr() for r in refs]), _ptr(img.cen),
-        _ptr(bws), bws.numel(), _ptr(skipped), st)
-    _lib.check(rc, "hbmr_kmeans_assign_top3_q1_bounded")
+        _ptr(bws), bws.numel(), _ptr(skipped), cands, rlows,
+        ctypes.c_void_p(skipped.data_ptr() + 8) if more else None, st)
+    _lib.check(rc, "hbmr_kmeans_assign_top3_q1_bounded_stash")
     for b in bases:
         b.pending = newref
+    if not stash:
+        return None
+    return bws, rlows, ctypes.c_void_p(skipped.data_ptr() + 16) if more else None
 
 
 def _exact_group(group, img, stats, labels_ptr, c16, ch, norms, dt, scratch, stream, lib, st,
-                 bases=None, skipped=None, newref=None):
+                 bases=None, skipped=None, newref=None, stash=False):
     B = len(group)
     ns = [sp.shape[0] for sp in group]
     N = sum(ns)
@@ -554,13 +583,13 @@
         rb = _RefineBatch(group, img, stats, scratch, stream)
         if TRACE.on:
             TRACE.instant("kmeans.top3_launch", n=B)
-        _bounded_group(group, bases, img, labels_ptr, ch, norms, dt, scratch, stream, lib, st, rb,
-                       skipped, newref)
+        sq = _bounded_group(group, bases, img, labels_ptr, ch, norms, dt, scratch, stream, lib, st,
+                            rb, skipped, newref, stash)
         o = 0
         for i in range(B):
             rb.labels[i] = labels_ptr + 4 * o
             o += ns[i]
-        rb.finish()
+        rb.finish(sq)
         return N
     if FUSED_Q1 and img.dp <= 128:
         rb = _RefineBatch(group, img, stats, scratch, stream)
@@ -648,11 +677,13 @@
 
 
 class Baseline:
-    __slots__ = ("g", "S0", "N0", "event", "stream", "data_ptr", "n", "gap", "ref", "pending")
+    __slots__ = ("g", "S0", "N0", "event", "stream", "data_ptr", "n", "gap", "ref", "pending",
+                 "cand", "rlow")
 
     def __init__(self, g, S0, N0, data_ptr, n):
         self.g, self.S0, self.N0 = g, S0, N0
         self.gap = self.ref = self.pending = None
+        self.cand = self.rlow = None
         self.event = None
         self.stream = None
         self.data_ptr, self.n = data_ptr, n
diff --git a/native/include/hbmr/hbmr.h b/native/include/hbmr/hbmr.h
--- a/native/include/hbmr/hbmr.h
+++ b/native/include/hbmr/hbmr.h
@@ -59,6 +59,14 @@
                                        const float* const* ref, const float* cen, void* bws,
                                        long bws_bytes, unsigned long long* skipped,
                                        hipStream_t st);
+int hbmr_kmeans_assign_top3_q1_bounded_stash(
+    int nsplit, const void* const* X, const long* n, int dp, int f16, const void* Ct,
+    const float* chalf, int k_pad, int32_t* labels, const float* const* xnorm,
+    const float* const* xbn2, const float* const* xerr, int d, int k, const float* cnorm,
+    const float* cmax, const float* cerr, const float* cerrmax, void* ws, long ws_bytes,
+    const float* dcc, const int32_t* const* g, float* const* gap, const float* const* ref,
+    const float* cen, void* bws, long bws_bytes, unsigned long long* skipped,
+    void* const* cand, float* const* rlow, unsigned long long* stashed, hipStream_t st);
 int hbmr_kmeans_assign_top3_grouped(int nsplit, const void* const* X, const long* n, int dp,
                                     int f16, const void* C, const float* chalf, int k_pad,
                                     int32_t* labels, int32_t* cand, float* scores, float* margin,
@@ -83,6 +91,12 @@
                                     const int32_t* nbr_idx, const float* nbr_dist, int L,
                                     unsigned long long* stats, int nstats, void* ws,
                                     long ws_bytes, hipStream_t st);
+int hbmr_kmeans_refine_batch_finish_stash(
+    int nsplit, const long* ns, const float* const* x32, int32_t* const* labels, int d, int ldx,
+    const float* C32, int k, int k_pad, const float* cmax, const float* cerrmax,
+    const int32_t* nbr_idx, const float* nbr_dist, int L, unsigned long long* stats, int nstats,
+    void* ws, long ws_bytes, const void* bws, long bws_bytes, float* const* rlow,
+    unsigned long long* invalidated, hipStream_t st);
 int hbmr_kmeans_update(const long long* sums, const long long* counts, int fx_shift, int k, int d,
                        int dp, int k_pad, float* cen, void* cbf, float* chalf, float* shift2,
                        hipStream_t st);
diff --git a/native/kernels/kmeans.hip b/native/kernels/kmeans.hip
--- a/native/kernels/kmeans.hip
+++ b/native/kernels/kmeans.hip
@@ -231,10 +231,21 @@
   return (int)hipGetLastError();
 }
 
+struct BoundLayout {
+  size_t shift, idx, sq, bytes;
+};
+static BoundLayout bound_layout(long total, int nsplit, int k) {
+  BoundLayout L;
+  L.shift = kBoundHdr;
+  L.idx = L.shift + (((size_t)nsplit * k * sizeof(float) + 255) & ~(size_t)255);
+  L.sq = L.idx + (((size_t)total * sizeof(uint32_t) + 255) & ~(size_t)255);
+  L.bytes = L.sq + (size_t)total * sizeof(StashEnt);
+  return L;
+}
+
 long hbmr_kmeans_bound_workspace_bytes(long total, int nsplit, int k) {
   if (total < 0 || nsplit <= 0 || nsplit > kMaxGroup || k <= 0) return -1;
-  const size_t sh = ((size_t)nsplit * k * sizeof(float) + 255) & ~(size_t)255;
-  return (long)(kBoundHdr + sh + (size_t)total * sizeof(uint32_t));
+  return (long)bound_layout(total, nsplit, k).bytes;
 }
 
 int hbmr_kmeans_assign_top3_q1_bounded(int nsplit, const void* const* X, const long* n, int dp,
@@ -248,10 +259,26 @@
                                        const float* const* ref, const float* cen, void* bws,
                                        long bws_bytes, unsigned long long* skipped,
                                        hipStream_t st) {
+  return hbmr_kmeans_assign_top3_q1_bounded_stash(
+      nsplit, X, n, dp, f16, Ct, chalf, k_pad, labels, xnorm, xbn2, xerr, d, k, cnorm, cmax, cerr,
+      cerrmax, ws, ws_bytes, dcc, g, gap, ref, cen, bws, bws_bytes, skipped, nullptr, nullptr,
+      nullptr, st);
+}
+
+int hbmr_kmeans_assign_top3_q1_bounded_stash(
+    int nsplit, const void* const* X, const long* n, int dp, int f16, const void* Ct,
+    const float* chalf, int k_pad, int32_t* labels, const float* const* xnorm,
+    const float* const* xbn2, const float* const* xerr, int d, int k, const float* cnorm,
+    const float* cmax, const float* cerr, const float* cerrmax, void* ws, long ws_bytes,
+    const float* dcc, const int32_t* const* g, float* const* gap, const float* const* ref,
+    const float* cen, void* bws, long bws_bytes, unsigned long long* skipped,
+    void* const* cand, float* const* rlow, unsigned long long* stashed, hipStream_t st) {
   if (nsplit <= 0 || nsplit > kMaxGroup || k_pad % 32 || k <= 0 || k_pad < k || d <= 0 ||
       d > kRefineMaxDp || !labels || ((uintptr_t)ws & 255) || (dp != 64 && dp != 128) || !Ct ||
-      !g || !gap || !ref || !cen || !bws || ((uintptr_t)bws & 255))
-    return (int)hipErrorInvalidValue;
+      !g || !gap || !ref || !cen || !bws || ((uintptr_t)bws & 255) || (cand == nullptr) !=
+      (rlow == nullptr) || (cand != nullptr && k > 0xffff))
+    return (int)hipErrorInvalidValue;
+  const bool stash = cand != nullptr;
   TopQ1Table t;
   SweepTable sw;
   GapTable gt;
@@ -266,12 +293,17 @@
   for (int i = 0; i < nsplit; ++i) {
     if (n[i] < 0 || n[i] > 0x7fffffffL || (n[i] > 0 && (!gap[i] || (ref[i] && !g[i]))))
       return (int)hipErrorInvalidValue;
+    if (stash && n[i] > 0 && (!cand[i] || !rlow[i] || ((uintptr_t)cand[i] & 7)))
+      return (int)hipErrorInvalidValue;
     fill_topq1(t, i, X, xnorm, xbn2, xerr, total, nb);
     sw.off[i] = total;
     sw.blk[i] = nsb;
-    sw.n[i] = n[i];
     sw.g[i] = g[i];
     gt.gap[i] = gap[i];
+    if (stash) {
+      sw.cand[i] = static_cast<ushort4*>(cand[i]);
+      sw.rlow[i] = rlow[i];
+    }
     if (ref[i]) {
       int r = 0;
       while (r < nref && sh.ref[r] != ref[i]) ++r;
@@ -285,29 +317,32 @@
   }
   t.off[nsplit] = total;
   t.blk[nsplit] = nb;
+  sw.off[nsplit] = total;
   sw.blk[nsplit] = nsb;
   const RefineLayout Ly = refine_layout(nsplit, n);
-  if (ws_bytes < (long)Ly.bytes ||
-      bws_bytes < hbmr_kmeans_bound_workspace_bytes(total, nsplit, k))
-    return (int)hipErrorInvalidValue;
+  const BoundLayout Bl = bound_layout(total, nsplit, k);
+  if (ws_bytes < (long)Ly.bytes || bws_bytes < (long)Bl.bytes) return (int)hipErrorInvalidValue;
   char* w = static_cast<char*>(ws);
   char* bw = static_cast<char*>(bws);
   HBMR_RETURN_IF_ERROR(hipMemsetAsync(w, 0, kHdrClear, st));
+  HBMR_RETURN_IF_ERROR(hipMemsetAsync(bw, 0, kBoundHdr, st));
   if (nb == 0) return 0;
   if (nb > 0x7fffffffL) return (int)hipErrorInvalidValue;
-  HBMR_RETURN_IF_ERROR(hipMemsetAsync(bw, 0, kBoundHdr, st));
   uint32_t* cnt = reinterpret_cast<uint32_t*>(bw);
   uint32_t* smax = cnt + kMaxGroup;
-  float* shift = reinterpret_cast<float*>(bw + kBoundHdr);
-  uint32_t* idx = reinterpret_cast<uint32_t*>(
-      bw + kBoundHdr + (((size_t)nsplit * k * sizeof(float) + 255) & ~(size_t)255));
+  uint32_t* scnt = smax + kMaxGroup;
+  StashPub* pub = reinterpret_cast<StashPub*>(bw + kBoundCnt);
+  float* shift = reinterpret_cast<float*>(bw + Bl.shift);
+  uint32_t* idx = reinterpret_cast<uint32_t*>(bw + Bl.idx);
+  StashEnt* sq = reinterpret_cast<StashEnt*>(bw + Bl.sq);
   if (nref > 0) {
     hipLaunchKernelGGL(kmeans_bound_shift_kernel, dim3((unsigned)k, (unsigned)nref), dim3(64), 0,
                        st, sh, cen, k, d, shift, smax);
     HBMR_RETURN_IF_ERROR(hipGetLastError());
   }
-  hipLaunchKernelGGL(kmeans_bound_sweep_kernel, dim3((unsigned)nsb), dim3(256), 0, st, sw, k,
-                     shift, reinterpret_cast<const float*>(smax), labels, cnt, idx);
+  auto sweep = stash ? kmeans_bound_sweep_kernel<true> : kmeans_bound_sweep_kernel<false>;
+  hipLaunchKernelGGL(sweep, dim3((unsigned)nsb), dim3(256), 0, st, sw, k, shift,
+                     reinterpret_cast<const float*>(smax), labels, cnt, idx, scnt, sq, pub);
   HBMR_RETURN_IF_ERROR(hipGetLastError());
   const FusedQ1Fin fin = make_fused_fin(k, d, k_pad, cnorm, cerr, dcc, cmax, cerrmax, w, Ly);
   const auto [kern, lds] = fused_kernel(dp, f16, [](auto D, auto F) {
@@ -315,7 +350,8 @@
   });
   hipLaunchKernelGGL(kern, dim3((unsigned)nb), dim3(256), lds, st, t, gt,
                      reinterpret_cast<const __bf16*>(Ct), chalf, k_pad / 32, labels, fin,
-                     (const uint32_t*)cnt, (const uint32_t*)idx, skipped);
+                     (const uint32_t*)cnt, (const uint32_t*)idx, skipped, (const uint32_t*)scnt,
+                     stash ? (const StashPub*)pub : nullptr, stashed);
   return (int)hipGetLastError();
 }
 
@@ -485,19 +521,51 @@
                                     const int32_t* nbr_idx, const float* nbr_dist, int L,
                                     unsigned long long* stats, int nstats, void* ws,
                                     long ws_bytes, hipStream_t st) {
+  return hbmr_kmeans_refine_batch_finish_stash(nsplit, ns, x32, labels, d, ldx, C32, k, k_pad,
+                                               cmax, cerrmax, nbr_idx, nbr_dist, L, stats, nstats,
+                                               ws, ws_bytes, nullptr, 0, nullptr, nullptr, st);
+}
+
+int hbmr_kmeans_refine_batch_finish_stash(
+    int nsplit, const long* ns, const float* const* x32, int32_t* const* labels, int d, int ldx,
+    const float* C32, int k, int k_pad, const float* cmax, const float* cerrmax,
+    const int32_t* nbr_idx, const float* nbr_dist, int L, unsigned long long* stats, int nstats,
+    void* ws, long ws_bytes, const void* bws, long bws_bytes, float* const* rlow,
+    unsigned long long* invalidated, hipStream_t st) {
   if (nsplit <= 0 || nsplit > kMaxGroup || d > ldx || d > kRefineMaxDp || d % 8 || ldx % 4 ||
       k <= 0 || k_pad < k || L < 1 || L > k || nstats < 3 || ((uintptr_t)C32 & 15) ||
       ((uintptr_t)ws & 255))
+    return (int)hipErrorInvalidValue;
+  const bool stash = bws != nullptr;
+  if (stash && (!rlow || ((uintptr_t)bws & 255) || d > 128))
     return (int)hipErrorInvalidValue;
   const RefineLayout Ly = refine_layout(nsplit, ns);
   if (ws_bytes < (long)Ly.bytes) return (int)hipErrorInvalidValue;
   RefineTable tbl;
   std::memset(&tbl, 0, sizeof(tbl));
   tbl.nsplit = nsplit;
+  StashQueue sq;
+  std::memset(&sq, 0, sizeof(sq));
+  long total = 0;
   for (int i = 0; i < nsplit; ++i) {
     if ((uintptr_t)x32[i] & 15) return (int)hipErrorInvalidValue;
     tbl.x32[i] = x32[i];
     tbl.labels[i] = labels[i];
+    if (stash) {
+      if (ns[i] > 0 && !rlow[i]) return (int)hipErrorInvalidValue;
+      sq.off[i] = total;
+      sq.rlow[i] = rlow[i];
+    }
+    total += ns[i];
+  }
+  if (stash) {
+    const BoundLayout Bl = bound_layout(total, nsplit, k);
+    if (bws_bytes < (long)Bl.bytes) return (int)hipErrorInvalidValue;
+    const char* bw = static_cast<const char*>(bws);
+    sq.nsplit = nsplit;
+    sq.cnt = reinterpret_cast<const uint32_t*>(bw) + 2 * kMaxGroup;
+    sq.ents = reinterpret_cast<const StashEnt*>(bw + Bl.sq);
+    sq.inval = invalidated;
   }
   const double pack_rel = pack_rel_of(k_pad);
   char* w = static_cast<char*>(ws);
@@ -507,19 +575,14 @@
   ExactQ2* q2 = reinterpret_cast<ExactQ2*>(w + Ly.off2);
   unsigned long long* ss = reinterpret_cast<unsigned long long*>(w + kStatsOff);
   const unsigned g3 = std::max(1u, Ly.g2);
-  if (d <= 128) {
-    hipLaunchKernelGGL(kmeans_refine_q2_kernel<1>, dim3(Ly.g2), dim3(256), 0, st, tbl, d, ldx,
-                       C32, k, cmax, cerrmax, pack_rel, c1, q1, Ly.cap1, c2, q2, Ly.cap2, ss);
-    HBMR_RETURN_IF_ERROR(hipGetLastError());
-    hipLaunchKernelGGL(kmeans_refine_q3_kernel<1>, dim3(g3), dim3(256), 0, st, tbl, d, ldx, C32,
-                       k, nbr_idx, nbr_dist, L, c2, q2, Ly.cap2, ss, nstats);
-  } else {
-    hipLaunchKernelGGL(kmeans_refine_q2_kernel<2>, dim3(Ly.g2), dim3(256), 0, st, tbl, d, ldx,
-                       C32, k, cmax, cerrmax, pack_rel, c1, q1, Ly.cap1, c2, q2, Ly.cap2, ss);
-    HBMR_RETURN_IF_ERROR(hipGetLastError());
-    hipLaunchKernelGGL(kmeans_refine_q3_kernel<2>, dim3(g3), dim3(256), 0, st, tbl, d, ldx, C32,
-                       k, nbr_idx, nbr_dist, L, c2, q2, Ly.cap2, ss, nstats);
-  }
+  auto q2k = stash ? kmeans_refine_q2_kernel<1, true>
+                   : d <= 128 ? kmeans_refine_q2_kernel<1> : kmeans_refine_q2_kernel<2>;
+  hipLaunchKernelGGL(q2k, dim3(Ly.g2), dim3(256), 0, st, tbl, d, ldx, C32, k, cmax, cerrmax,
+                     pack_rel, c1, q1, Ly.cap1, c2, q2, Ly.cap2, ss, sq);
+  HBMR_RETURN_IF_ERROR(hipGetLastError());
+  auto q3k = d <= 128 ? kmeans_refine_q3_kernel<1> : kmeans_refine_q3_kernel<2>;
+  hipLaunchKernelGGL(q3k, dim3(g3), dim3(256), 0, st, tbl, d, ldx, C32, k, nbr_idx, nbr_dist, L,
+                     c2, q2, Ly.cap2, ss, nstats);
   HBMR_RETURN_IF_ERROR(hipGetLastError());
   hipLaunchKernelGGL(kmeans_refine_stats_kernel, dim3(1), dim3(64), 0, st, ss, stats, nstats);
   return (int)hipGetLastError();
diff --git a/native/kernels/kmeans/bounded.h b/native/kernels/kmeans/bounded.h
--- a/native/kernels/kmeans/bounded.h
+++ b/native/kernels/kmeans/bounded.h
@@ -5,7 +5,14 @@
 namespace {
 
 constexpr int kSweepPer = 8;
-constexpr int kBoundHdr = 512;
+constexpr int kBoundCnt = 3 * kMaxGroup * 4;
+constexpr int kBoundHdr = 2048;
+
+struct StashPub {
+  ushort4* cand[kMaxGroup];
+  float* rlow[kMaxGroup];
+};
+static_assert(kBoundCnt + sizeof(StashPub) <= kBoundHdr, "bound workspace header");
 
 struct ShiftTable {
   const float* ref[kMaxGroup];
@@ -43,16 +50,19 @@
   int nsplit;
   const int32_t* g[kMaxGroup];
   float* gap[kMaxGroup];
+  ushort4* cand[kMaxGroup];
+  float* rlow[kMaxGroup];
   int rid[kMaxGroup];
-  long n[kMaxGroup];
-  long off[kMaxGroup];
+  long off[kMaxGroup + 1];
   long blk[kMaxGroup + 1];
 };
 
+template <bool STASH>
 __global__ __launch_bounds__(256) void kmeans_bound_sweep_kernel(
     const SweepTable tbl, int k, const float* __restrict__ shift,
     const float* __restrict__ smax, int32_t* __restrict__ labels, uint32_t* __restrict__ cnt,
-    uint32_t* __restrict__ idx) {
+    uint32_t* __restrict__ idx, uint32_t* __restrict__ scnt, StashEnt* __restrict__ sq,
+    StashPub* __restrict__ pub) {
   const long b = blockIdx.x;
   int lo = 0, hi = tbl.nsplit;
   while (hi - lo > 1) {
@@ -61,20 +71,30 @@
   }
   const int s = __builtin_amdgcn_readfirstlane(lo);
   const int tid = threadIdx.x, lane = tid & 63, wave = tid >> 6;
-  const long n = tbl.n[s], o = tbl.off[s];
+  if constexpr (STASH) {
+    if (b == 0 && tid < tbl.nsplit) {
+      pub->cand[tid] = tbl.cand[tid];
+      pub->rlow[tid] = tbl.rlow[tid];
+    }
+  }
+  const long o = tbl.off[s], n = tbl.off[s + 1] - o;
   const int32_t* __restrict__ g = tbl.g[s];
   float* __restrict__ gap = tbl.gap[s];
+  const ushort4* __restrict__ cand = STASH ? tbl.cand[s] : nullptr;
+  float* __restrict__ rlow = STASH ? tbl.rlow[s] : nullptr;
   const float* __restrict__ sh = shift + (size_t)tbl.rid[s] * k;
   const float sm = gap ? smax[tbl.rid[s]] : 0.f;
   const long p0 = (b - tbl.blk[s]) * (256 * kSweepPer);
   __shared__ uint32_t wcnt[4][kSweepPer];
-  __shared__ uint32_t base_s;
-  bool list[kSweepPer];
-  uint32_t rank[kSweepPer];
+  __shared__ uint32_t wst[4][kSweepPer];
+  __shared__ uint32_t base_s, sbase_s;
+  bool list[kSweepPer], st[kSweepPer];
+  uint32_t rank[kSweepPer], srank[kSweepPer];
+  StashEnt ent[kSweepPer];
 #pragma unroll
   for (int i = 0; i < kSweepPer; ++i) {
     const long p = p0 + i * 256 + tid;
-    list[i] = false;
+    list[i] = st[i] = false;
     if (p < n) {
       list[i] = true;
       if (gap) {
@@ -85,12 +105,32 @@
           list[i] = false;
           labels[o + p] = c;
           gap[p] = v;
+        } else if (STASH && rlow != nullptr) {
+          const float r = sub_rd_pos(rlow[p], sm);
+          if (r > 0.f) {
+            list[i] = false;
+            st[i] = true;
+            rlow[p] = r;
+            const ushort4 cd = cand[p];
+            labels[o + p] = cd.x;
+            ent[i].row = (uint32_t)p;
+            ent[i].b = cd.x;
+            ent[i].s = cd.y;
+            ent[i].t = cd.z;
+            ent[i].pad = 0;
+            ent[i].rlow = r;
+          }
         }
       }
     }
     const unsigned long long m = __ballot(list[i]);
     rank[i] = lane_rank(m);
     if (lane == 0) wcnt[wave][i] = (uint32_t)__popcll(m);
+    if constexpr (STASH) {
+      const unsigned long long ms = __ballot(st[i]);
+      srank[i] = lane_rank(ms);
+      if (lane == 0) wst[wave][i] = (uint32_t)__popcll(ms);
+    }
   }
   __syncthreads();
   if (tid == 0) {
@@ -105,11 +145,29 @@
       }
     base_s = tot ? atomicAdd(cnt + s, tot) : 0u;
   }
+  if (STASH && tid == 64) {
+    uint32_t tot = 0;
+#pragma unroll
+    for (int w = 0; w < 4; ++w)
+#pragma unroll
+      for (int i = 0; i < kSweepPer; ++i) {
+        const uint32_t c = wst[w][i];
+        wst[w][i] = tot;
+        tot += c;
+      }
+    sbase_s = tot ? atomicAdd(scnt + s, tot) : 0u;
+  }
   __syncthreads();
   uint32_t* out = idx + o + base_s;
 #pragma unroll
   for (int i = 0; i < kSweepPer; ++i)
     if (list[i]) out[wcnt[wave][i] + rank[i]] = (uint32_t)(p0 + i * 256 + tid);
+  if constexpr (STASH) {
+    StashEnt* sout = sq + o + sbase_s;
+#pragma unroll
+    for (int i = 0; i < kSweepPer; ++i)
+      if (st[i]) sout[wst[wave][i] + srank[i]] = ent[i];
+  }
 }
 
 struct GapTable {
@@ -121,13 +179,17 @@
     const TopQ1Table tbl, const GapTable gt, const __bf16* __restrict__ Ct,
     const float* __restrict__ chalf, int ntiles, int32_t* __restrict__ labels, FusedQ1Fin fin,
     const uint32_t* __restrict__ cnt, const uint32_t* __restrict__ idx,
-    unsigned long long* __restrict__ skipped) {
+    unsigned long long* __restrict__ skipped, const uint32_t* __restrict__ scnt,
+    const StashPub* __restrict__ pub, unsigned long long* __restrict__ stashed) {
   extern __shared__ __attribute__((aligned(16))) char smem[];
-  if (blockIdx.x == 0 && threadIdx.x == 0 && skipped != nullptr) {
-    unsigned long long sk = 0;
-    for (int i = 0; i < tbl.nsplit; ++i)
-      sk += (unsigned long long)(tbl.off[i + 1] - tbl.off[i]) - cnt[i];
-    if (sk) atomicAdd(skipped, sk);
+  if (blockIdx.x == 0 && threadIdx.x == 0 && (skipped != nullptr || stashed != nullptr)) {
+    unsigned long long sk = 0, sc = 0;
+    for (int i = 0; i < tbl.nsplit; ++i) {
+      sk += (unsigned long long)(tbl.off[i + 1] - tbl.off[i]) - cnt[i] - scnt[i];
+      sc += scnt[i];
+    }
+    if (sk && skipped != nullptr) atomicAdd(skipped, sk);
+    if (sc && stashed != nullptr) atomicAdd(stashed, sc);
   }
   const long b = hbmr_xcd_remap(blockIdx.x, gridDim.x);
   int lo = 0, hi = tbl.nsplit;
@@ -146,6 +208,10 @@
   fin.sidx = s;
   fin.idx = idx + o;
   fin.gap = gt.gap[s];
+  if (pub != nullptr) {
+    fin.cand = pub->cand[s];
+    fin.rlow = pub->rlow[s];
+  }
   assign_tile_v3<D, F16, true>(tbl.X[s], nl, Ct, chalf, ntiles, labels + o, lb, smem, fin);
 }
 
diff --git a/native/kernels/kmeans/fused.h b/native/kernels/kmeans/fused.h
--- a/native/kernels/kmeans/fused.h
+++ b/native/kernels/kmeans/fused.h
@@ -24,6 +24,8 @@
   unsigned long long* stats;
   const uint32_t* idx;
   float* gap;
+  ushort4* cand;
+  float* rlow;
 
   template <class AM, int PB, bool BND = false>
   __device__ __forceinline__ void operator()(const AM (&am)[PB], int h, long p0, int col, long n,
@@ -83,6 +85,15 @@
           flag[pb] = q.s < k && q1_certify<true>(q, m2, cnorm[q.b], cerr[q.b], k, gam, cm, cem,
                                                  pack_rel, cnorm, cerr, dcc, gp);
           gap[row] = gp;
+          if (rlow != nullptr) {
+            float rl = 0.f;
+            if (flag[pb] && q.t < k && q.t != q.b && q.t != q.s && q.s != q.b)
+              rl = stash_rlow(q, gam, cm, cem, pack_rel);
+            rlow[row] = rl;
+            if (rl > 0.f)
+              cand[row] = make_ushort4((unsigned short)q.b, (unsigned short)q.s,
+                                       (unsigned short)q.t, 0);
+          }
         } else {
           flag[pb] = q.s < k && q1_flagged(q, m2, cnorm[q.b], cerr[q.b], k, gam, cm, cem,
                                            pack_rel, cnorm, cerr, dcc);
diff --git a/native/kernels/kmeans/refine_queue.h b/native/kernels/kmeans/refine_queue.h
--- a/native/kernels/kmeans/refine_queue.h
+++ b/native/kernels/kmeans/refine_queue.h
@@ -137,6 +137,20 @@
   return q1_certify<false>(e, m2, cnb, ceb, k, gam, cm, cem, pack_rel, cnorm, cerr, dcc, unused);
 }
 
+__device__ __forceinline__ float stash_rlow(const ExactQ1& e, double gam, double cm, double cem,
+                                            double pack_rel) {
+  const double inflate = 1.0 + 0x1p-20;
+  const double xn = ((double)e.xn + (double)e.xe) * inflate;
+  const double x2 = (double)e.x2;
+  const double amax = ((double)e.xe + cem) * inflate;
+  const double st = (double)e.sb - (double)e.m3;
+  double et, dl_t;
+  exact_bound(st, cm, xn, x2, amax, gam, pack_rel, et, dl_t);
+  const double r2 = (x2 * (1.0 - 0x1p-22) - 2.0 * (st + et)) * (1.0 - 0x1p-30);
+  if (!(dl_t >= 2.0 * amax) || !(r2 > 0.0)) return 0.f;
+  return fmaxf(0.f, __double2float_rd(sqrt(r2) * (1.0 - 0x1p-30)));
+}
+
 __device__ __forceinline__ void refine_q1_block(
     long n, int sidx, long blk, int d, int k, const float* __restrict__ xnorm,
     const float* __restrict__ xbn2, const float* __restrict__ xerr,
@@ -285,34 +299,86 @@
   return v;
 }
 
-template <int NM>
+struct alignas(16) StashEnt {
+  uint32_t row;
+  unsigned short b, s, t, pad;
+  float rlow;
+};
+static_assert(sizeof(StashEnt) == 16, "stash queue entry layout");
+struct StashQueue {
+  const uint32_t* cnt;
+  const StashEnt* ents;
+  unsigned long long* inval;
+  int nsplit;
+  long off[kMaxGroup];
+  float* rlow[kMaxGroup];
+};
+static_assert(kMaxGroup == HBMR_WAVE, "q2 scans the stash counts in one wave");
+
+template <int NM, bool STASH = false>
 __global__ __launch_bounds__(256) void kmeans_refine_q2_kernel(
     const RefineTable tbl, int d, int ldx, const float* __restrict__ C32, int k,
     const float* __restrict__ cmax, const float* __restrict__ cerrmax, double pack_rel,
     const uint32_t* __restrict__ qcount, const ExactQ1* __restrict__ q1, long cap1,
     uint32_t* __restrict__ q2count, ExactQ2* __restrict__ q2, long cap2,
-    unsigned long long* __restrict__ sstats) {
+    unsigned long long* __restrict__ sstats, const StashQueue sq) {
   constexpr uint32_t kPerBlk = 4 * kQ2Per;
   constexpr uint32_t kBuf = 256;
   const int tid = threadIdx.x, lane = tid & 63, wave = tid >> 6;
   const int grp = lane / kQ2Lanes, sub = lane % kQ2Lanes;
   __shared__ ExactQ2 sbuf[kBuf];
   __shared__ uint32_t sn, sbase;
-  __shared__ unsigned long long cnt[2];
-  if (tid < 2) cnt[tid] = 0;
+  __shared__ unsigned long long cnt[4];
+  __shared__ uint32_t spre[kMaxGroup + 1];
+  if (tid < 4) cnt[tid] = 0;
   if (tid == 0) sn = 0;
+  if constexpr (STASH) {
+    if (tid < HBMR_WAVE) {
+      uint32_t v = tid < sq.nsplit ? sq.cnt[tid] : 0u;
+#pragma unroll
+      for (int o = 1; o < HBMR_WAVE; o <<= 1) {
+        const uint32_t u = __shfl_up(v, o);
+        if (lane >= o) v += u;
+      }
+      spre[tid + 1] = v;
+      if (tid == 0) spre[0] = 0;
+    }
+  }
   __syncthreads();
   const double inflate = 1.0 + 0x1p-20;
   const double gam = (double)(d + 2) * 0x1p-23 * 1.01;
   const double cem = (double)cerrmax[0] * inflate;
   const double cm = (double)cmax[0] * inflate + cem;
   uint32_t c1[kQShards];
-  uint32_t total = 0;
+  uint32_t total1 = 0;
 #pragma unroll
   for (int j = 0; j < kQShards; ++j) {
     c1[j] = qcount[j];
-    total += c1[j];
-  }
+    total1 += c1[j];
+  }
+  uint32_t total = total1;
+  if constexpr (STASH) total += spre[kMaxGroup];
+  auto fetch = [&](uint32_t i) {
+    if (!STASH || i < total1) return q1[shard_slot(c1, cap1, i)];
+    const uint32_t j = i - total1;
+    int lo = 0, hi = kMaxGroup;
+    while (hi - lo > 1) {
+      const int mid = (lo + hi) >> 1;
+      if (spre[mid] <= j) lo = mid; else hi = mid;
+    }
+    const StashEnt se = sq.ents[sq.off[lo] + (j - spre[lo])];
+    const bool ok = se.b < k && se.s < k && se.t < k;
+    ExactQ1 r;
+    r.row = se.row;
+    r.split = (uint32_t)lo;
+    r.b = ok ? se.b : 0;
+    r.s = ok ? se.s : 0;
+    r.t = ok ? se.t : 0;
+    r.sb = r.m3 = r.x2 = r.xn = r.xe = 0.f;
+    r.pad0 = 1.f;
+    r.pad1 = ok ? se.rlow : 0.f;
+    return r;
+  };
   const int shard = blockIdx.x % kQShards;
   const uint32_t stride = gridDim.x * kPerBlk;
   const uint32_t off = wave * kQ2Per + grp;
@@ -330,12 +396,12 @@
   };
   uint32_t bb = blockIdx.x * kPerBlk;
   ExactQ1 e;
-  if (bb < total) e = q1[shard_slot(c1, cap1, min(bb + off, total - 1))];
+  if (bb < total) e = fetch(min(bb + off, total - 1));
   for (; bb < total; bb += stride) {
     const ExactQ1 q = e;
     const bool have = bb + off < total;
     const uint32_t nb = bb + stride;
-    if (nb < total) e = q1[shard_slot(c1, cap1, min(nb + off, total - 1))];
+    if (nb < total) e = fetch(min(nb + off, total - 1));
     const bool t_real = q.t < k;
     const float* xr = tbl.x32[q.split] + (size_t)q.row * ldx;
     float xf[16 * NM], c0[16 * NM], c1r[16 * NM], c2[16 * NM];
@@ -366,7 +432,12 @@
                      (!t_real || w == q.t || beats(f2));
     dw = whi;
     bool certified = !t_real && separated;
-    if (t_real && separated) {
+    const bool stash = STASH && q.pad0 != 0.f;
+    bool drop = false;
+    if (stash) {
+      drop = !(isfinite(whi) && sqrt(whi) * (1.0 + 0x1p-40) < (double)q.pad1);
+      certified = separated && !drop;
+    } else if (t_real && separated) {
       const double xn = ((double)q.xn + (double)q.xe) * inflate;
       const double x2 = (double)q.x2;
       const double amax = ((double)q.xe + cem) * inflate;
@@ -378,6 +449,13 @@
     if (have && sub == 0 && certified && w != q.b) {
       tbl.labels[q.split][q.row] = w;
       atomicAdd(&cnt[0], 1ull);
+    }
+    if constexpr (STASH) {
+      if (have && sub == 0 && drop) sq.rlow[q.split][q.row] = 0.f;
+      const unsigned long long ms = __ballot(have && sub == 0 && stash);
+      const unsigned long long md = __ballot(have && sub == 0 && drop);
+      if (lane == 0 && ms) atomicAdd(&cnt[2], (unsigned long long)__popcll(ms));
+      if (lane == 0 && md) atomicAdd(&cnt[3], (unsigned long long)__popcll(md));
     }
     const bool spill = have && sub == 0 && !certified;
     const unsigned long long m = __ballot(spill);
@@ -401,6 +479,10 @@
   __syncthreads();
   if (sn) flush();
   if (tid < 2 && cnt[tid]) atomicAdd(sstats + 4 * shard + 1 + tid, cnt[tid]);
+  if constexpr (STASH) {
+    if (tid == 2 && cnt[2]) atomicAdd(sstats + 4 * shard, cnt[2]);
+    if (tid == 3 && cnt[3] && sq.inval != nullptr) atomicAdd(sq.inval, cnt[3]);
+  }
 }
 
 template <int NM>
```

Result: slower. 9527 (-6.1%).
